# c5shen/WITCH

Measured on AMD Instinct MI355X. Metric: query-seqs aligned/sec (100k queries x 200-HMM eHMM), higher is better.
Workload: dtype f32; 1 GPU; dna_100k_x200; n_queries=100000, n_hmms=200, query_len=150, model_len_min=898, model_len_max=993, k=10, pairs_reported_rank0=20000000, pairs_multidomain_rank0=968, pairs_long_list_rank0=0, pairs_dense_redo_rank0=3, topk_crc32=3263627139

## Files before the change

witch_amd/csrc/wh_device.h:

```cpp
#pragma once
#include <hip/hip_runtime.h>

#include "wh_common.h"

namespace wh {

template <int CTRL, int ROW_MASK = 0xF, int BANK_MASK = 0xF, bool BOUND = false>
__device__ __forceinline__ float dppf(float old, float src) {
  return __builtin_bit_cast(
      float, __builtin_amdgcn_update_dpp(__builtin_bit_cast(int, old), __builtin_bit_cast(int, src), CTRL,
                                         ROW_MASK, BANK_MASK, BOUND));
}

typedef float v4f_t __attribute__((ext_vector_type(4)));
template <int Q, bool BLK = true>
__device__ __forceinline__ constexpr int fs_piece(int lane, int q4) { return (BLK && Q >= 8) ? lane * (2 * (Q / 4)) + q4 : q4 * kWave + lane; }
__device__ __forceinline__ float4 nt_load4(const float4 *p) {
  v4f_t v = __builtin_nontemporal_load(reinterpret_cast<const v4f_t *>(p));
  return make_float4(v.x, v.y, v.z, v.w);
}
__device__ __forceinline__ void nt_store4(float4 *p, float a, float b, float c, float d) {
  v4f_t v = {a, b, c, d};
  __builtin_nontemporal_store(v, reinterpret_cast<v4f_t *>(p));
}

__device__ __forceinline__ float wave_shr1(float x) { return dppf<0x138, 0xF, 0xF, true>(0.f, x); }

__device__ __forceinline__ float readlane_f(float x, int lane) {
  return __builtin_bit_cast(float, __builtin_amdgcn_readlane(__builtin_bit_cast(int, x), lane));
}

__device__ __forceinline__ float wave_sum(float x) {
  x += dppf<0xB1>(0.f, x);
  x += dppf<0x4E>(0.f, x);
  x += dppf<0x141>(0.f, x);
  x += dppf<0x140>(0.f, x);
  return (readlane_f(x, 0) + readlane_f(x, 16)) + (readlane_f(x, 32) + readlane_f(x, 48));
}

__device__ __forceinline__ float wave_max(float x) {
  x = fmaxf(x, dppf<0xB1>(x, x));
  x = fmaxf(x, dppf<0x4E>(x, x));
  x = fmaxf(x, dppf<0x141>(x, x));
  x = fmaxf(x, dppf<0x140>(x, x));
  return fmaxf(fmaxf(readlane_f(x, 0), readlane_f(x, 16)), fmaxf(readlane_f(x, 32), readlane_f(x, 48)));
}

template <int N>
struct RowsDown {
  unsigned v[N];
  int top;
  __device__ __forceinline__ void load(const float *spec, const int (&off)[N], const int (&shift)[N], int i, int lane) {
    top = i;
#pragma unroll
    for (int n = 0; n < N; n++) {
      const int r = i - lane + shift[n];
      v[n] = r >= 0 ? __builtin_nontemporal_load(reinterpret_cast<const unsigned *>(spec) + off[n] + r) : 0u;
    }
  }
  __device__ __forceinline__ bool spent(int i) const { return top - i >= kWave; }
  __device__ __forceinline__ unsigned u(int n, int i) const { return (unsigned)__builtin_amdgcn_readlane((int)v[n], top - i); }
  __device__ __forceinline__ int s(int n, int i) const { return __builtin_amdgcn_readlane((int)v[n], top - i); }
  __device__ __forceinline__ float f(int n, int i) const { return __builtin_bit_cast(float, __builtin_amdgcn_readlane((int)v[n], top - i)); }
};

struct ScanC { float s[6]; };

__device__ __forceinline__ ScanC scan_prepare(float A) {
  ScanC c;
  c.s[0] = A; A *= dppf<0x111>(1.f, A);
  c.s[1] = A; A *= dppf<0x112>(1.f, A);
  c.s[2] = A; A *= dppf<0x114>(1.f, A);
  c.s[3] = A; A *= dppf<0x118>(1.f, A);
  c.s[4] = A; A *= dppf<0x142, 0xA>(1.f, A);
  c.s[5] = A;
  return c;
}

__device__ __forceinline__ float scan_apply(const ScanC &c, float B) {
#ifndef WH_PLAIN_DPP_SCAN
  asm("s_nop 1\n\tv_fmac_f32_dpp %0, %0, %1 row_shr:1 row_mask:0xf bank_mask:0xf" : "+v"(B) : "v"(c.s[0]));
  asm("s_nop 1\n\tv_fmac_f32_dpp %0, %0, %1 row_shr:2 row_mask:0xf bank_mask:0xf" : "+v"(B) : "v"(c.s[1]));
  asm("s_nop 1\n\tv_fmac_f32_dpp %0, %0, %1 row_shr:4 row_mask:0xf bank_mask:0xf" : "+v"(B) : "v"(c.s[2]));
  asm("s_nop 1\n\tv_fmac_f32_dpp %0, %0, %1 row_shr:8 row_mask:0xf bank_mask:0xf" : "+v"(B) : "v"(c.s[3]));
  asm("s_nop 1\n\tv_fmac_f32_dpp %0, %0, %1 row_bcast:15 row_mask:0xa bank_mask:0xf" : "+v"(B) : "v"(c.s[4]));
  asm("s_nop 1\n\tv_fmac_f32_dpp %0, %0, %1 row_bcast:31 row_mask:0xc bank_mask:0xf" : "+v"(B) : "v"(c.s[5]));
  asm("s_nop 1" : "+v"(B));
  return B;
#else
  B = fmaf(c.s[0], dppf<0x111>(0.f, B), B);
  B = fmaf(c.s[1], dppf<0x112>(0.f, B), B);
  B = fmaf(c.s[2], dppf<0x114>(0.f, B), B);
  B = fmaf(c.s[3], dppf<0x118>(0.f, B), B);
  B = fmaf(c.s[4], dppf<0x142, 0xA>(0.f, B), B);
  B = fmaf(c.s[5], dppf<0x143, 0xC>(0.f, B), B);
  return B;
#endif
}

template <class T>
__device__ __forceinline__ T *uniform_ptr(T *p) {
  const unsigned long long v = (unsigned long long)p;
  const unsigned lo = (unsigned)__builtin_amdgcn_readfirstlane((int)(unsigned)v), hi = (unsigned)__builtin_amdgcn_readfirstlane((int)(unsigned)(v >> 32));
  return (T *)(((unsigned long long)hi << 32) | lo);
}

__device__ __forceinline__ float row_shr1(float x) { return dppf<0x111, 0xF, 0xF, true>(0.f, x); }
__device__ __forceinline__ float row_sum(float x) {
  x += dppf<0xB1>(0.f, x);
  x += dppf<0x4E>(0.f, x);
  x += dppf<0x141>(0.f, x);
  x += dppf<0x140>(0.f, x);
  return x;
}
struct ScanR { float s[4]; };
__device__ __forceinline__ ScanR scan_prepare_row(float A) {
  ScanR c;
  c.s[0] = A; A *= dppf<0x111>(1.f, A);
  c.s[1] = A; A *= dppf<0x112>(1.f, A);
  c.s[2] = A; A *= dppf<0x114>(1.f, A);
  c.s[3] = A;
  return c;
}
__device__ __forceinline__ float scan_apply_row(const ScanR &c, float B) {
  asm("s_nop 1\n\tv_fmac_f32_dpp %0, %0, %1 row_shr:1 row_mask:0xf bank_mask:0xf" : "+v"(B) : "v"(c.s[0]));
  asm("s_nop 1\n\tv_fmac_f32_dpp %0, %0, %1 row_shr:2 row_mask:0xf bank_mask:0xf" : "+v"(B) : "v"(c.s[1]));
  asm("s_nop 1\n\tv_fmac_f32_dpp %0, %0, %1 row_shr:4 row_mask:0xf bank_mask:0xf" : "+v"(B) : "v"(c.s[2]));
  asm("s_nop 1\n\tv_fmac_f32_dpp %0, %0, %1 row_shr:8 row_mask:0xf bank_mask:0xf" : "+v"(B) : "v"(c.s[3]));
  asm("s_nop 1" : "+v"(B));
  return B;
}

template <int Q, bool TREG>
struct TransTab;

template <int Q>
struct TransTab<Q, true> {
  float4 v[FW_NARR][Q / 4];
  __device__ __forceinline__ void load(const float *g, const float * , int lane) {
    const float4 *p = reinterpret_cast<const float4 *>(g);
#pragma unroll
    for (int a = 0; a < FW_NARR; a++)
#pragma unroll
      for (int q4 = 0; q4 < Q / 4; q4++) v[a][q4] = p[(a * (Q / 4) + q4) * kWave + lane];
  }
  __device__ __forceinline__ float4 ld(int a, int q4) const { return v[a][q4]; }
};

template <int Q>
struct TransTab<Q, false> {
  const float4 *p;
  __device__ __forceinline__ void load(const float * , const float *lds, int lane) {
    p = reinterpret_cast<const float4 *>(lds) + lane;
  }
  __device__ __forceinline__ float4 ld(int a, int q4) const { return p[(a * (Q / 4) + q4) * kWave]; }
};

__device__ __forceinline__ float f4get(const float4 &v, int j) {
  return j == 0 ? v.x : j == 1 ? v.y : j == 2 ? v.z : v.w;
}

template <int Q, bool TREG>
__device__ __forceinline__ float lane_product(const TransTab<Q, TREG> &T, int arr) {
  float A = 1.f;
#pragma unroll
  for (int q4 = 0; q4 < Q / 4; q4++) {
    float4 d = T.ld(arr, q4);
    A *= d.x; A *= d.y; A *= d.z; A *= d.w;
  }
  return A;
}

typedef float v4f_t __attribute__((ext_vector_type(4)));
typedef const __attribute__((address_space(3))) v4f_t lds_cv4_t;
struct LdsF4 {
  lds_cv4_t *p;
  __device__ __forceinline__ LdsF4(const float *base) : p((lds_cv4_t *)base) {}
  __device__ __forceinline__ float4 operator[](int i) const { const v4f_t v = p[i]; return make_float4(v.x, v.y, v.z, v.w); }
};

template <int Q>
__device__ __forceinline__ void load_em_fwd(float (&od)[Q], const float *emL, const float *emG, int x, int K,
                                            int lane) {
  if (x < K) {
    const LdsF4 p(emL + (size_t)x * Q * kWave + 4 * lane);
#pragma unroll
    for (int q4 = 0; q4 < Q / 4; q4++) {
      float4 v = p[q4 * kWave];
      od[4 * q4] = v.x; od[4 * q4 + 1] = v.y; od[4 * q4 + 2] = v.z; od[4 * q4 + 3] = v.w;
    }
  } else {
    const float4 *p = reinterpret_cast<const float4 *>(emG + (size_t)x * Q * kWave) + lane;
#pragma unroll
    for (int q4 = 0; q4 < Q / 4; q4++) {
      float4 v = p[q4 * kWave];
      od[4 * q4] = v.x; od[4 * q4 + 1] = v.y; od[4 * q4 + 2] = v.z; od[4 * q4 + 3] = v.w;
    }
  }
}

template <int Q>
__device__ __forceinline__ void load_em_rev(float (&od)[Q], const float *emL, const float *emG, int x, int K,
                                            int lane) {
  if (x < K) {
    const LdsF4 p(emL + (size_t)x * Q * kWave + 4 * (kWave - 1 - lane));
#pragma unroll
    for (int p4 = 0; p4 < Q / 4; p4++) {
      float4 v = p[(Q / 4 - 1 - p4) * kWave];
      od[4 * p4] = v.w; od[4 * p4 + 1] = v.z; od[4 * p4 + 2] = v.y; od[4 * p4 + 3] = v.x;
    }
  } else {
    const float4 *p = reinterpret_cast<const float4 *>(emG + (size_t)x * Q * kWave) + (kWave - 1 - lane);
#pragma unroll
    for (int p4 = 0; p4 < Q / 4; p4++) {
      float4 v = p[(Q / 4 - 1 - p4) * kWave];
      od[4 * p4] = v.w; od[4 * p4 + 1] = v.z; od[4 * p4 + 2] = v.y; od[4 * p4 + 3] = v.x;
    }
  }
}

__device__ __forceinline__ int f32_exponent(float x) { return ((__builtin_bit_cast(int, x) >> 23) & 0xFF) - 127; }
__device__ __forceinline__ float pow2f_int(int e) { return __builtin_bit_cast(float, (e + 127) << 23); }

struct LenCfg { float loop, move, EJ, EC; };

__device__ __forceinline__ LenCfg len_config(int Lcfg, bool multihit) {
  LenCfg c;
  float nj = multihit ? 1.0f : 0.0f;
  c.move = (2.0f + nj) / ((float)Lcfg + 2.0f + nj);
  c.loop = 1.0f - c.move;
  c.EJ = multihit ? 0.5f : 0.0f;
  c.EC = multihit ? 0.5f : 1.0f;
  return c;
}

enum { SP_N = 0, SP_B, SP_E, SP_J, SP_C, SP_S, SP_ML, SP_MH, SP_NARR };

constexpr float kRescaleHi = 1048576.0f;

__device__ __forceinline__ void region_scan_global(float *spec, int SP, int L, int *regs, int lane, int &nenv,
                                                   int &nreg, int &flags) {
  const float rt1 = 0.25f, rt2 = 0.10f;
  float btot = 0.f, etot = 0.f;
  int i0 = -1;
  bool trig = false;
  if (lane == 0) { spec[SP_J * SP] = 0.f; spec[SP_C * SP] = 0.f; }
  for (int j0 = 1; j0 <= L; j0 += kWave) {
    const int jj = j0 + lane;
    const bool valid = jj <= L;
    const float nv = valid ? __builtin_nontemporal_load(spec + SP_N * SP + jj) : 0.f;
    const float bv = valid ? __builtin_nontemporal_load(spec + SP_B * SP + jj - 1) : 0.f;
    const float ev = valid ? __builtin_nontemporal_load(spec + SP_E * SP + jj) : 0.f;
    float jout = 0.f, cout = 0.f;
    const int cnt = L - j0 + 1 < kWave ? L - j0 + 1 : kWave;
    for (int t = 0; t < cnt; t++) {
      const int j = j0 + t;
      const float mocc = 1.0f - readlane_f(nv, t);
      const float bold = btot, eold = etot;
      btot += readlane_f(bv, t);
      etot += readlane_f(ev, t);
      if (lane == t) { jout = btot; cout = etot; }
      if (!trig) {
        if (mocc - (btot - bold) < rt2) i0 = j;
        else if (i0 == -1) i0 = j;
        if (mocc >= rt1) trig = true;
      } else if (mocc - (etot - eold) < rt2) {
        if (nenv < WH_MAX_ENVELOPES) {
          if (lane == 0) { regs[2 * nenv] = i0; regs[2 * nenv + 1] = j; }
          nenv++;
        } else flags |= WH_FLAG_TRUNC;
        nreg++;
        i0 = -1;
        trig = false;
      }
    }
    if (valid) { spec[SP_J * SP + jj] = jout; spec[SP_C * SP + jj] = cout; }
  }
}

template <int Q, bool TREG, bool STORE, bool USEP = false, bool SLIM = false, bool UM = false, bool COUNT = false, bool BLK = false>
__device__ __forceinline__ void forward_sweep(const TransTab<Q, TREG> &T, const ScanC &sc, const float *emL,
                                              const float *emG, int K, const uint8_t *seq, int L, LenCfg cfg,
                                              float *spec, int SP, float *Fs, float keep_scale, int lane,
                                              float &xC_out, int &ef_out, unsigned *um_out = nullptr, int *nstored_out = nullptr, int keep_lanes = 63 << 8) {
  float Mp[Q], Ip[Q], Dp[Q];
#pragma unroll
  for (int q = 0; q < Q; q++) { Mp[q] = 0.f; Ip[q] = 0.f; Dp[q] = 0.f; }
  float xN = 1.0f, xB = cfg.move, xJ = 0.f, xC = 0.f, xE = 0.f;
  int ef = 0;
  unsigned long long um_prev = 0, um_steady = 0;
  int nstored = 0;
  unsigned long long umask = 0;
  if (lane == 0) {
    spec[SP_N * SP] = xN; spec[SP_B * SP] = xB; spec[SP_E * SP] = 0.f; spec[SP_J * SP] = 0.f;
    spec[SP_C * SP] = 0.f; reinterpret_cast<int *>(spec)[SP_S * SP] = 0;
  }
#pragma unroll 1
  for (int i = 1; i <= L; i++) {
    asm volatile("" ::: "memory");
    const int x = seq[i - 1];
    float od[Q];
    load_em_fwd<Q>(od, emL, emG, x, K, lane);
    const float mm1 = wave_shr1(Mp[Q - 1]), im1 = wave_shr1(Ip[Q - 1]), dm1 = wave_shr1(Dp[Q - 1]);
#pragma unroll
    for (int q4 = Q / 4 - 1; q4 >= 0; q4--) {
      const float4 A = T.ld(FW_A, q4), B = T.ld(FW_B, q4), C = T.ld(FW_C, q4), E = T.ld(FW_E, q4);
      const float4 MI = T.ld(FW_MI, q4), II = T.ld(FW_II, q4);
#pragma unroll
      for (int j = 3; j >= 0; j--) {
        const int q = 4 * q4 + j;
        const float pm = q > 0 ? Mp[q > 0 ? q - 1 : 0] : mm1;
        const float pi = q > 0 ? Ip[q > 0 ? q - 1 : 0] : im1;
        const float pd = q > 0 ? Dp[q > 0 ? q - 1 : 0] : dm1;
        const float ni = fmaf(f4get(MI, j), Mp[q], f4get(II, j) * Ip[q]);
        float acc = xB * f4get(E, j);
        acc = fmaf(f4get(A, j), pm, acc);
        acc = fmaf(f4get(B, j), pi, acc);
        acc = fmaf(f4get(C, j), pd, acc);
        Mp[q] = od[q] * acc;
        Ip[q] = ni;
      }
    }
    const float mn1 = wave_shr1(Mp[Q - 1]);
    float dprev = 0.f;
#pragma unroll
    for (int q4 = 0; q4 < Q / 4; q4++) {
      const float4 D1 = T.ld(FW_D1, q4), D2 = T.ld(FW_D2, q4);
#pragma unroll
      for (int j = 0; j < 4; j++) {
        const int q = 4 * q4 + j;
        const float src = q > 0 ? Mp[q > 0 ? q - 1 : 0] : mn1;
        dprev = fmaf(f4get(D2, j), dprev, f4get(D1, j) * src);
        Dp[q] = dprev;
      }
    }
    float carry = wave_shr1(scan_apply(sc, dprev));
    float es = 0.f;
#pragma unroll
    for (int q4 = 0; q4 < Q / 4; q4++) {
      const float4 D2 = T.ld(USEP ? FW_P : FW_D2, q4);
#pragma unroll
      for (int j = 0; j < 4; j++) {
        const int q = 4 * q4 + j;
        if (USEP) {
          Dp[q] = fmaf(f4get(D2, j), carry, Dp[q]);
        } else {
          carry *= f4get(D2, j);
          Dp[q] += carry;
        }
        es += Mp[q] + Dp[q];
      }
    }
    xE = wave_sum(es);
    xN = xN * cfg.loop;
    xC = fmaf(xC, cfg.loop, xE * cfg.EC);
    xJ = fmaf(xJ, cfg.loop, xE * cfg.EJ);
    if (xE > kRescaleHi) {
      const int e = f32_exponent(xE);
      const float r = pow2f_int(-e);
#pragma unroll
      for (int q = 0; q < Q; q++) { Mp[q] *= r; Ip[q] *= r; Dp[q] *= r; }
      xN *= r; xC *= r; xJ *= r; xE *= r;
      ef += e;
    }
    xB = (xJ + xN) * cfg.move;
    if (lane == 0) {
      spec[SP_N * SP + i] = xN;
      if (!(STORE && SLIM)) { spec[SP_B * SP + i] = xB; spec[SP_E * SP + i] = xE; }
      spec[SP_J * SP + i] = xJ; spec[SP_C * SP + i] = xC;
      reinterpret_cast<int *>(spec)[SP_S * SP + i] = ef;
    }
    if (UM && !STORE) {
      if ((i & 7) == 0) {
        float lmax = 0.f;
#pragma unroll
        for (int q = 0; q < Q; q += 2) lmax = fmaxf(fmaxf(fmaxf(fmaxf(lmax, Mp[q]), Mp[q + 1]), Ip[q]), Ip[q + 1]);
        const unsigned long long dom = __ballot(lmax > 0.5f * xE);
        umask |= dom;
        const unsigned long long link = dom & (um_prev | (um_prev << 1));
        if (link) um_steady |= link | (um_prev & (link | (link >> 1)));
        um_prev = dom;
      }
    }
    if (STORE) {
      constexpr int ML = SLIM ? SP_B : SP_ML, MH = SLIM ? SP_E : SP_MH;
      float lmax = 0.f;
#pragma unroll
      for (int q = 0; q < Q; q += 2) lmax = fmaxf(fmaxf(fmaxf(fmaxf(lmax, Mp[q]), Mp[q + 1]), Ip[q]), Ip[q + 1]);
      const unsigned long long dom = __ballot(lmax > 0.5f * xE);
      umask |= dom;
      const int blo = keep_lanes & 255;
      int bhi = (keep_lanes >> 8) & 255;
      if (keep_lanes >> 16) bhi = min(bhi, (keep_lanes >> 16) - 1 + i / Q);
      const bool keep = keep_scale < 0.f || (lmax > keep_scale * xE && lane >= blo && lane <= bhi);
      const unsigned long long mask = __ballot(keep);
      if (COUNT) nstored += __builtin_popcountll(mask);
      if (lane == 0) {
        reinterpret_cast<unsigned *>(spec)[ML * SP + i] = (unsigned)(mask & 0xFFFFFFFFull);
        reinterpret_cast<unsigned *>(spec)[MH * SP + i] = (unsigned)(mask >> 32);
      }
      if (keep) {
        float4 *row = reinterpret_cast<float4 *>(Fs) + (size_t)i * (2 * (Q / 4) * kWave);
#pragma unroll
        for (int q4 = 0; q4 < Q / 4; q4++) {
          nt_store4(row + (BLK ? fs_piece<Q>(lane, q4) : q4 * kWave + lane), Mp[4 * q4], Mp[4 * q4 + 1], Mp[4 * q4 + 2], Mp[4 * q4 + 3]);
          nt_store4(row + (BLK ? fs_piece<Q>(lane, Q / 4 + q4) : (Q / 4 + q4) * kWave + lane), Ip[4 * q4], Ip[4 * q4 + 1], Ip[4 * q4 + 2], Ip[4 * q4 + 3]);
        }
      }
    }
  }
  if (STORE && lane == 0) {
    reinterpret_cast<unsigned *>(spec)[(SLIM ? SP_B : SP_ML) * SP] = (unsigned)(umask & 0xFFFFFFFFull);
    reinterpret_cast<unsigned *>(spec)[(SLIM ? SP_E : SP_MH) * SP] = (unsigned)(umask >> 32);
  }
  if (UM && !STORE && lane == 0) {
    um_out[0] = (unsigned)(umask & 0xFFFFFFFFull); um_out[1] = (unsigned)(umask >> 32);
    um_out[-1] = um_steady ? (unsigned)(__builtin_ctzll(um_steady) | ((63 - __builtin_clzll(um_steady)) << 8) | (1 << 16)) : 0u;
  }
  if (COUNT && nstored_out) *nstored_out = nstored;
  xC_out = xC;
  ef_out = ef;
}

constexpr float kClampHi = 1.1529215e18f;

template <int Q>
__device__ __forceinline__ void mirror_scale(int dn, float (&Mb)[Q], float (&Ib)[Q], float &xJ, float &xC, float &xN) {
  if (dn != 0) {
    const float r = __builtin_bit_cast(float, (127 - dn) << 23);
#pragma unroll
    for (int p = 0; p < Q; p++) { Mb[p] *= r; Ib[p] *= r; }
    xJ *= r; xC *= r; xN *= r;
  }
}

template <int Q>
__device__ __forceinline__ bool clamp_backward(float (&Mb)[Q], float (&Ib)[Q], float &xB, float &xJ, float &xC, float &xN) {
  if (fmaxf(xB, fmaxf(xN, xC)) > kClampHi) {
#pragma unroll
    for (int p = 0; p < Q; p++) { Mb[p] = fminf(Mb[p], kClampHi); Ib[p] = fminf(Ib[p], kClampHi); }
    xB = fminf(xB, kClampHi); xN = fminf(xN, kClampHi); xC = fminf(xC, kClampHi); xJ = fminf(xJ, kClampHi);
    return true;
  }
  return false;
}

template <int Q, bool TREG>
__device__ __forceinline__ float backward_emit(const TransTab<Q, TREG> &T, const float *emL, const float *emG, int x,
                                               int K, int lane, float (&Mb)[Q]) {
  float part = 0.f;
  auto groups = [&](auto em_ld) {
#pragma unroll
    for (int p4 = 0; p4 < Q / 4; p4++) {
      const float4 E = T.ld(BW_E, p4);
      const float4 O = em_ld(Q / 4 - 1 - p4);
      Mb[4 * p4 + 0] *= O.w; part = fmaf(E.x, Mb[4 * p4 + 0], part);
      Mb[4 * p4 + 1] *= O.z; part = fmaf(E.y, Mb[4 * p4 + 1], part);
      Mb[4 * p4 + 2] *= O.y; part = fmaf(E.z, Mb[4 * p4 + 2], part);
      Mb[4 * p4 + 3] *= O.x; part = fmaf(E.w, Mb[4 * p4 + 3], part);
    }
  };
  x = __builtin_amdgcn_readfirstlane(x);
  if (x < K) {
    const LdsF4 ep(emL + (size_t)x * Q * kWave + 4 * (kWave - 1 - lane));
    groups([&](int q4) { return ep[q4 * kWave]; });
  } else {
    const float4 *ep = reinterpret_cast<const float4 *>(emG + (size_t)x * Q * kWave) + (kWave - 1 - lane);
    groups([&](int q4) { return ep[q4 * kWave]; });
  }
  return part;
}

template <int Q>
struct TransTabAt {
  LdsF4 base;
  int slot[4];
  __device__ __forceinline__ TransTabAt(const float *lds) : base(lds) {}
  __device__ __forceinline__ float4 ld(int a, int p4) const { return base[a * (Q / 4) * kWave + slot[p4]]; }
};

template <int Q, bool TREG, bool USEP = false>
__device__ __forceinline__ void backward_cells(const TransTab<Q, TREG> &T, const ScanC &sc, float (&Mb)[Q],
                                               float (&Ib)[Q], float xE) {
  float Dn[Q];
  const float gm1 = wave_shr1(Mb[Q - 1]);
  float dprev = 0.f;
#pragma unroll
  for (int p4 = 0; p4 < Q / 4; p4++) {
    const float4 DM = T.ld(BW_DM, p4), DD = T.ld(BW_DD, p4);
#pragma unroll
    for (int j = 0; j < 4; j++) {
      const int p = 4 * p4 + j;
      const float g = p > 0 ? Mb[p > 0 ? p - 1 : 0] : gm1;
      dprev = fmaf(f4get(DD, j), dprev, fmaf(f4get(DM, j), g, xE));
      Dn[p] = dprev;
    }
  }
  float carry = wave_shr1(scan_apply(sc, dprev));
#pragma unroll
  for (int p4 = 0; p4 < Q / 4; p4++) {
    const float4 DD = T.ld(USEP ? BW_P : BW_DD, p4);
#pragma unroll
    for (int j = 0; j < 4; j++) {
      const int p = 4 * p4 + j;
      if (USEP) {
        Dn[p] = fmaf(f4get(DD, j), carry, Dn[p]);
      } else {
        carry *= f4get(DD, j);
        Dn[p] += carry;
      }
    }
  }
  const float dm1 = wave_shr1(Dn[Q - 1]);
#pragma unroll
  for (int p4 = Q / 4 - 1; p4 >= 0; p4--) {
    const float4 MM = T.ld(BW_MM, p4), IM = T.ld(BW_IM, p4), MI = T.ld(BW_MI, p4), II = T.ld(BW_II, p4);
    const float4 MD = T.ld(BW_MD, p4);
#pragma unroll
    for (int j = 3; j >= 0; j--) {
      const int p = 4 * p4 + j;
      const float g = p > 0 ? Mb[p > 0 ? p - 1 : 0] : gm1;
      const float dn = p > 0 ? Dn[p > 0 ? p - 1 : 0] : dm1;
      float nm = fmaf(f4get(MM, j), g, xE);
      nm = fmaf(f4get(MI, j), Ib[p], nm);
      nm = fmaf(f4get(MD, j), dn, nm);
      const float ni = fmaf(f4get(IM, j), g, f4get(II, j) * Ib[p]);
      Mb[p] = nm;
      Ib[p] = ni;
    }
  }
}

template <class TT>
__device__ __forceinline__ void backward_cells_row(const TT &T, const ScanR &sc, float (&Mb)[16], float (&Ib)[16], float xE) {
  float Dn[16];
  const float gm1 = row_shr1(Mb[15]);
  float dprev = 0.f;
#pragma unroll
  for (int p4 = 0; p4 < 4; p4++) {
    const float4 DM = T.ld(BW_DM, p4), DD = T.ld(BW_DD, p4);
#pragma unroll
    for (int j = 0; j < 4; j++) {
      const int p = 4 * p4 + j;
      const float g = p > 0 ? Mb[p > 0 ? p - 1 : 0] : gm1;
      dprev = fmaf(f4get(DD, j), dprev, fmaf(f4get(DM, j), g, xE));
      Dn[p] = dprev;
    }
  }
  float carry = row_shr1(scan_apply_row(sc, dprev));
#pragma unroll
  for (int p4 = 0; p4 < 4; p4++) {
    const float4 DD = T.ld(BW_DD, p4);
#pragma unroll
    for (int j = 0; j < 4; j++) {
      const int p = 4 * p4 + j;
      carry *= f4get(DD, j);
      Dn[p] += carry;
    }
  }
  const float dm1 = row_shr1(Dn[15]);
#pragma unroll
  for (int p4 = 3; p4 >= 0; p4--) {
    const float4 MM = T.ld(BW_MM, p4), IM = T.ld(BW_IM, p4), MI = T.ld(BW_MI, p4), II = T.ld(BW_II, p4);
    const float4 MD = T.ld(BW_MD, p4);
#pragma unroll
    for (int j = 3; j >= 0; j--) {
      const int p = 4 * p4 + j;
      const float g = p > 0 ? Mb[p > 0 ? p - 1 : 0] : gm1;
      const float dn = p > 0 ? Dn[p > 0 ? p - 1 : 0] : dm1;
      float nm = fmaf(f4get(MM, j), g, xE);
      nm = fmaf(f4get(MI, j), Ib[p], nm);
      nm = fmaf(f4get(MD, j), dn, nm);
      const float ni = fmaf(f4get(IM, j), g, f4get(II, j) * Ib[p]);
      Mb[p] = nm;
      Ib[p] = ni;
    }
  }
}

}
```

witch_amd/csrc/wh_host_score.hip:

```cpp
#include "wh_host.h"

static const int kStagedMaxBatches = 1 << 15;
static const int kStagedQB = 48;

static int resolve_main_cap(int max_M) {
  const size_t per_wave = (kLdsBudget - resolve_lds_header_bytes(0)) / (size_t)resolve_waves_per_cu();
  int lo = 1, hi = 1 << 20;
  while (lo < hi) {
    const int mid = lo + (hi - lo + 1) / 2;
    if (resolve_lds_bytes(mid, max_M) <= per_wave) lo = mid; else hi = mid - 1;
  }
  return lo;
}

static ScoreCall score_call(wh_ehmm *e, const uint8_t *d_residues, const int64_t *d_offsets, int64_t nq, int64_t total_residues, int32_t max_len,
                            int32_t *d_decibits, uint8_t *d_flags, float *d_fwd_bits, wh_pair_detail *d_detail, void *stream) {
  ScoreCall c = {e, (hipStream_t)stream, d_residues, d_offsets, nq, total_residues, max_len, d_decibits, d_flags, d_fwd_bits, d_detail};
  c.Lc = std::max(max_len, 1);
  c.H = (int)e->hmms.size();
  c.npairs_all = nq * (int64_t)c.H;
  const bool fits = resolve_lds_bytes(c.Lc, e->max_M) <= kLdsBudget;
  c.Lmain = fits || e->knobs.no_long_query ? c.Lc : resolve_main_cap(e->max_M);
  c.resolve = !e->knobs.no_resolve && (fits || !e->knobs.no_long_query) && c.npairs_all < 0x7FFFFFFF;
  c.mixed = nq > 0 && total_residues > 0 && (double)max_len > 1.25 * (double)total_residues / (double)nq;
  c.wide_dense = getenv("WH_WIDE_DENSE"); c.wide_no_em_lds = getenv("WH_WIDE_NO_EM_LDS"); c.p2win_force = getenv("WH_P2WIN_FORCE");
  c.res_null2_gather = getenv("WH_RES_NULL2_GATHER"); c.res_no_lds_tables = getenv("WH_RES_NO_LDS_TABLES");
  if (const char *wv = getenv("WH_RES_WAVES")) c.res_waves = std::max(1, atoi(wv));
  c.Ls = main_length_cap(e, c.Lc, false, c.resolve, c.p2win_force);
  return c;
}

struct StagedWaves { int wl, one, both, p2, p4; };
enum class ScoreFamily { PhaseCall, PhaseCallB, TwoQuery, FourEnvelope, PassSync, Staged };
static const char *const kFamilyName[] = {"phase-call", "phase-call(B)", "two-queries-per-wave", "phase-call", "pass-synchronous", "staged"};

struct ScoreClassPlan {
  int Q, list_off, n_list;
  ScoreFamily family;
  LdsPlan b;
  int Klds;
  bool specg;
  int p2win;
  bool use_qorder;
  int QB, n_qblocks, n_items;
  size_t scratch_stride, spec_stride;
  int blocks;
  StagedWaves st;
};

static int cap_waves(const Knobs &kn, int w) { return cap_waves(kn.max_waves, w); }
static size_t score_table_bytes(const wh_ehmm *e, int Q) { return score_table_bytes(e->K, Q); }

static const int G_all = 1, G_most = 4, G_few = 8, G_rare = 32;
static int staged_cand_cap(int G, int per_pair) { return std::min(G * kStagedQB * per_pair, 2048); }
static size_t staged_lds(int Q, int wl, int arrays, int waves, int cand) {
  return lds_bytes(kLdsHeader + (size_t)cand * sizeof(int), (size_t)arrays * Q * kWave * sizeof(float), waves, wl);
}
static bool plan_staged(const wh_ehmm *e, int Q, int Lc, StagedWaves *w) {
  const int K = e->K;
  const size_t tbl = (size_t)Q * kWave * sizeof(float);
  auto fit = [&](int arrays, int from, int cand, int per_cu) { return fit_waves(kLdsHeader + (size_t)cand * sizeof(int), arrays * tbl, from, w->wl, per_cu); };
  w->wl = kScoreSpecArrays * row_stride(Lc) + 32 + kRegsInts + residue_words(Lc);
  w->one = fit(K + FW_NARR, 12, staged_cand_cap(G_few, WH_MAX_ENVELOPES), 1);
  w->both = fit(K + 2 * FW_NARR, 12, staged_cand_cap(G_rare, WH_MAX_ENVELOPES), 1);
  w->p2 = fit(K, 12, staged_cand_cap(G_most, 1), 2);
  w->p4 = fit(K, 10, staged_cand_cap(G_most, WH_MAX_ENVELOPES), 2);
  return w->one >= 4 && w->both >= 4 && w->p2 >= 4 && w->p4 >= 4;
}

static int plan_score_class(const ScoreCall &c, int Q, int list_off, int n_list, ScoreClassPlan *out) {
  const wh_ehmm *e = c.e;
  const Knobs &kn = e->knobs;
  const int Lc = c.Ls;
  const int64_t nq = c.nq;
  const size_t table = score_table_bytes(e, Q);
  ScoreClassPlan p = {};
  p.Q = Q; p.list_off = list_off; p.n_list = n_list;
  ScoreLds l;
  if (!plan_score_lds(plan_knobs(e, c.p2win_force), e->K, Q, Lc, true, &l)) { set_error("query length %d with model class Q=%d does not fit in LDS", c.max_len, Q); return WH_ERANGE; }
  p.b = l.b; p.Klds = l.Klds;
  LdsPlan &b = p.b;
  const bool big = l.big, specg = l.specg, pairk = l.pairk, p2win = l.p2win, p2inpl = l.p2inpl;
  bool quadk = false;
  if ((kn.kernel == 10 || kn.kernel == 11) && !e->st_off && !big && !pairk && !specg && !kn.dbg && (Q == 8 || Q == 12 || Q == 16 || Q == 20 || Q == 24) &&
      plan_staged(e, Q, Lc, &p.st)) {
    p.family = ScoreFamily::Staged;
    b.SP = row_stride(Lc); b.wave_lds = p.st.wl;
    p.QB = kStagedQB; p.n_qblocks = (int)((nq + p.QB - 1) / p.QB); p.n_items = n_list * p.n_qblocks;
    p.scratch_stride = (size_t)(Lc + 1) * 2 * Q * kWave;
    *out = p;
    return WH_OK;
  }
  if (kn.kernel == 12 && !big && !pairk && !specg && Q == 16) {
    const int wlq = kScoreSpecArrays * row_stride(Lc) + 128 + kRegsInts + 4 * 16 + 4 * 16 + 4 * residue_words(Lc);
    const int wq = fit_waves(kLdsHeader, table, cap_waves(kn, 12), wlq);
    if (wq >= 8) { quadk = true; b = {wq, row_stride(Lc), wlq, lds_bytes(kLdsHeader, table, wq, wlq)}; }
  }
  p.family = big ? ScoreFamily::PassSync : pairk ? ScoreFamily::TwoQuery : quadk ? ScoreFamily::FourEnvelope : kn.kernel == 8 ? ScoreFamily::PhaseCallB : ScoreFamily::PhaseCall;
  p.p2win = (specg || big || pairk || quadk) ? 0 : p2win ? 1 : p2inpl ? 2 : 0;
  p.use_qorder = big || c.mixed;
  const int waves = b.waves;
  p.QB = big ? waves * 2 : pairk ? waves * 4 : waves * (kn.item_g > 0 ? kn.item_g : 32);
  const int per_turn = pairk ? 2 : 1;
  const int max_blocks = big ? e->cu_count : e->cu_count * std::max(1, 8 / waves);
  if ((int64_t)n_list * ((nq + p.QB - 1) / p.QB) < 4 * (int64_t)max_blocks) {
    p.QB = waves * per_turn;
    if (!big && !pairk) for (int g_ = 16; g_ > 1; g_ /= 2)
      if ((int64_t)n_list * ((nq + waves * g_ - 1) / (waves * g_)) >= 4 * (int64_t)max_blocks) { p.QB = waves * g_; break; }
  }
  if (quadk) p.QB = std::max(p.QB, waves * 8);
  p.n_qblocks = (int)((nq + p.QB - 1) / p.QB);
  p.n_items = n_list * p.n_qblocks;
  p.scratch_stride = (size_t)(quadk ? 5 : per_turn) * (size_t)(Lc + 1) * 2 * Q * kWave;
  p.spec_stride = specg ? (size_t)8 * b.SP : quadk ? (size_t)(5 * kScoreSpecArrays + 1) * b.SP : 0;
  p.specg = specg || quadk;
  p.blocks = clamp_blocks(std::min(p.n_items, max_blocks), (size_t)waves * (p.scratch_stride + p.spec_stride) * sizeof(float), e->d_scratch, e->max_M, Lc, "scoring");
  if (p.blocks < 0) return WH_ENOMEM;
  *out = p;
  return WH_OK;
}

static ScoreArgs class_args(const ScoreCall &c, const ScoreClassPlan &p, int launches) {
  const wh_ehmm *e = c.e;
  const Knobs &kn = e->knobs;
  ScoreArgs a;
  fill_common(a, c);
  a.tables = (const float *)e->d_tables.p;
  a.hmm_list = (const int32_t *)e->d_lists.p + p.list_off; a.n_list = p.n_list;
  a.counter = e->counter(kSlotLaunch0 + launches);
  a.dbg = kn.dbg;
  a.no_window = kn.no_window ? 1 : 0;
  a.keep_scale = kn.keep_scale;
  a.spill_band = kn.kernel != 9 ? kn.spill_band : 0;
  a.Klds = p.Klds; a.SP = p.b.SP; a.wave_lds = p.b.wave_lds; a.spec_arrays = kScoreSpecArrays;
  a.paths = reinterpret_cast<unsigned long long *>(e->counter(kSlotScorePath));
  a.p2win = p.p2win;
  a.qorder = p.use_qorder ? c.d_qorder : nullptr;
  a.QB = p.QB; a.n_qblocks = p.n_qblocks; a.n_items = p.n_items;
  a.scratch_stride = p.scratch_stride; a.spec_stride = p.spec_stride;
  a.scratch = (float *)e->d_scratch.p;
  if (p.specg) a.spec_scratch = (float *)e->d_spec.p;
  return a;
}

static int print_class_stats(const ScoreCall &c, int Q, const unsigned long long *stats) {
  unsigned long long st[40];
  if (int rc = stats_read(c, stats, st)) return rc;
  const double tot = (double)(st[4] + st[5] + st[6] + st[7] + st[8] + st[9] + st[10] + st[11]);
  fprintf(stderr, "[wh] Q=%d wave cycles: P1 %.1f%%  P2 %.1f%%  regions %.1f%%  P3 %.1f%%  P4 %.1f%%  null2 %.1f%%  swaps+barriers %.1f%%  other %.1f%%  (total %.3g ticks)\n", Q, 100.0 * st[4] / tot,
          100.0 * st[5] / tot, 100.0 * st[6] / tot, 100.0 * st[7] / tot, 100.0 * st[8] / tot, 100.0 * st[9] / tot, 100.0 * st[10] / tot, 100.0 * st[11] / tot, tot);
  if (st[38]) fprintf(stderr, "[wh] Q=%d wave lifetimes %.3g cycles: %.1f%% in the phases above, %.1f%% fetching an item (two barriers)\n", Q, (double)st[38], 100.0 * tot / (double)st[38], 100.0 * (double)st[39] / (double)st[38]);
  if (st[37]) fprintf(stderr, "[wh] Q=%d four-envelope sweeps: %llu envelopes, %.0f wave cycles per envelope (slot 'null2' above)\n", Q, st[37], (double)st[9] / (double)st[37]);
  fprintf(stderr, "[wh] Q=%d envelope Backward sweeps: %llu on a 256-node window, %llu on a 512-node window, %llu windows failed the mass certificate, %llu full width; union of the stored lane blocks: span %.1f blocks (with margin), %.1f blocks set, of %llu envelopes\n", Q, st[0], st[1], st[2], st[3], (double)st[12] / (double)std::max(1ull, st[14]), (double)st[15] / (double)std::max(1ull, st[14]), st[14]);
  fprintf(stderr, "[wh] Q=%d multihit Backward on a window: %llu scans, of them in doubt at a threshold %llu, at the multidomain bound %llu; window loss out of range %llu; mean eps %.3g\n", Q,
          st[35], st[32], st[33], st[36], st[35] ? 1e-9 * (double)st[34] / (double)st[35] : 0.0);
  fprintf(stderr, "[wh] Q=%d |Ld - mass| / Ld  (<3e-7, <1e-6, <3e-6, <1e-5, <2e-5, more): window sweeps %llu %llu %llu %llu %llu %llu; full-width sweeps %llu %llu %llu %llu %llu %llu\n", Q,
          st[16], st[17], st[18], st[19], st[20], st[21], st[22], st[23], st[24], st[25], st[26], st[27]);
  return WH_OK;
}

static int launch_score_class(const ScoreCall &c, const ScoreClassPlan &p, int *launches) {
  wh_ehmm *e = c.e;
  hipStream_t s = c.s;
  const int Q = p.Q, waves = p.b.waves, threads = waves * kWave;
  const bool big = p.family == ScoreFamily::PassSync;
  ScoreArgs a = class_args(c, p, *launches);
  if (a.p2win == 2) {
    a.p2_backup_stride = (size_t)kScoreSpecArrays * a.SP;
    if (e->d_p2bak.ensure((size_t)p.blocks * waves * a.p2_backup_stride * sizeof(float))) return WH_ENOMEM;
    a.p2_backup = (float *)e->d_p2bak.p;
  }
  if (int rc = stats_begin(c, 320, 13, &a.stats)) return rc;
  if (e->knobs.trace) fprintf(stderr, "[wh] score Q=%d kernel=%s specg=%d waves=%d blocks=%d lds=%zu SP=%d wave_lds=%d items=%d Lcap=%d\n", Q,
                              kFamilyName[(int)p.family], (int)p.specg, waves, p.blocks, p.b.lds, a.SP, a.wave_lds, a.n_items, a.Lcap);
  HIPCHK(hipMemsetAsync(a.counter, 0, sizeof(int), s));
  if (class_mark(e, s, Q, big ? 1 : 0)) return WH_EHIP;
  hipError_t err = big ? launch_score_big(Q, a, p.blocks, threads, p.b.lds, s)
                   : p.family == ScoreFamily::TwoQuery ? launch_score9(Q, a, p.blocks, threads, p.b.lds, s)
                   : p.family == ScoreFamily::FourEnvelope ? launch_score7q(Q, a, p.blocks, threads, p.b.lds, s)
                   : p.family == ScoreFamily::PhaseCallB ? launch_score7b(Q, a, p.blocks, threads, p.b.lds, s)
                                                         : launch_score7(Q, a, p.blocks, threads, p.b.lds, s);
  if (err != hipSuccess) { set_error("score kernel launch (Q=%d) failed: %s", Q, hipGetErrorString(err)); return WH_EHIP; }
  (*launches)++;
  return a.stats ? print_class_stats(c, Q, a.stats) : WH_OK;
}

static int print_staged_stats(const ScoreCall &c, int Q, const unsigned long long *stats) {
  unsigned long long st[64];
  if (int rc = stats_read(c, stats, st)) return rc;
  static const char *kind[9] = {"p1", "p2win 256", "p2win 512", "p2full", "p3", "p4win 256", "p4win 512", "p4full", "dense"};
  for (int k = 0; k < 9; k++)
    fprintf(stderr, "[wh] staged Q=%d %-10s sweeps %9llu  shader cycles per sweep %10.0f  real time per sweep %8.1f us  (clock %.2f GHz)  wave lifetimes %.3g cycles, in sweeps %.1f%%\n", Q, kind[k], st[4 * k + 3],
            st[4 * k + 3] ? (double)st[4 * k] / (double)st[4 * k + 3] : 0.0, st[4 * k + 3] ? 0.01 * (double)st[4 * k + 1] / (double)st[4 * k + 3] : 0.0,
            st[4 * k + 1] ? 0.1 * (double)st[4 * k] / (double)st[4 * k + 1] : 0.0, (double)st[4 * k + 2], st[4 * k + 2] ? 100.0 * (double)st[4 * k] / (double)st[4 * k + 2] : 0.0);
  return WH_OK;
}

static int launch_staged_class(const ScoreCall &c, const ScoreClassPlan &p, int *launches) {
  wh_ehmm *e = c.e;
  hipStream_t s = c.s;
  const Knobs &kn = e->knobs;
  const bool split = kn.kernel == 11;
  const int Q = p.Q, Lc = c.Ls, K = e->K, w_one = p.st.one, w_both = p.st.both, w_p2 = p.st.p2, w_p4 = p.st.p4;
  auto lds_of = [&](int arrays, int waves, int cand) { return staged_lds(Q, p.st.wl, arrays, waves, cand); };
  ScoreArgs a = class_args(c, p, *launches);
  StagedArgs g;
  memset(&g, 0, sizeof g);
  g.slab_stride = (size_t)(Lc + 1) * 2 * Q * kWave;
  g.p1stride = (size_t)kScoreSpecArrays * a.SP;
  g.p3stride = g.p1stride;
  int64_t NS = split ? (int64_t)e->cu_count * w_one * 16 : (int64_t)1 << 20;
  size_t free_b = 0, total_b = 0;
  if (split && hipMemGetInfo(&free_b, &total_b) == hipSuccess) {
    const size_t budget = (size_t)((double)(free_b + e->d_st_slabs.cap + e->d_st_p3spec.cap) * 0.45);
    NS = std::min<int64_t>(NS, (int64_t)(budget / ((g.slab_stride + g.p3stride) * sizeof(float))));
  }
  if (kn.st_units > 0) NS = kn.st_units;
  const int64_t total_pairs = (int64_t)a.n_items * a.QB;
  NS = std::min<int64_t>(NS, (int64_t)((double)total_pairs * e->st_upp) + a.QB * WH_MAX_ENVELOPES);
  if (NS < 16) { set_error("staged launches: no HBM for the Forward slabs (Q=%d, L=%d)", Q, Lc); return WH_ENOMEM; }
  const double upp = split ? e->st_upp : 1.0;
  int items_b = (int)std::max<int64_t>(1, (int64_t)((double)NS / upp) / a.QB);
  items_b = std::min(items_b, a.n_items);
  {
    const int nb = (a.n_items + items_b - 1) / items_b;
    items_b = (a.n_items + nb - 1) / nb;
    if (items_b > 2 * e->cu_count) items_b = std::min((items_b + e->cu_count - 1) / e->cu_count * e->cu_count, (int)std::max<int64_t>(1, (int64_t)((double)NS / upp) / a.QB));
  }
  const int NB = items_b * a.QB;
  const int n_batches = (a.n_items + items_b - 1) / items_b;
  if (e->d_st_pairs.ensure(sizeof(StPair) * (size_t)NB) || e->d_st_p1spec.ensure(sizeof(float) * g.p1stride * (size_t)NB) ||
      e->d_st_cnt.ensure(sizeof(int) * 32 * (size_t)kStagedMaxBatches))
    return WH_ENOMEM;
  if (e->last_staged_batches + n_batches > kStagedMaxBatches) { set_error("staged launches: more than %d batches in one call", kStagedMaxBatches); return WH_ERANGE; }
  if (split && (e->d_st_units.ensure(sizeof(StUnit) * (size_t)NS) || e->d_st_p3spec.ensure(sizeof(float) * g.p3stride * (size_t)NS) ||
                e->d_st_slabs.ensure(sizeof(float) * g.slab_stride * (size_t)NS)))
    return WH_ENOMEM;
  g.NB = NB; g.NS = (int)NS;
  if (split) e->st_last_NB = NB;
  g.pairs = (StPair *)e->d_st_pairs.p; g.p1spec = (float *)e->d_st_p1spec.p;
  g.units = (StUnit *)e->d_st_units.p; g.p3spec = (float *)e->d_st_p3spec.p; g.slabs = (float *)e->d_st_slabs.p;
  g.pair_paths = e->path_buf; g.pair_paths16 = e->path_buf16;
  int *cnt0 = (int *)e->d_st_cnt.p + 32 * (size_t)e->last_staged_batches;
  HIPCHK(hipMemsetAsync(cnt0, 0, sizeof(int) * 32 * (size_t)n_batches, s));
  const bool w512 = Q == 16 || Q == 24;
  if (kn.trace) fprintf(stderr, "[wh] staged Q=%d: %d items of %d queries in %d batches of %d pairs, %lld units (%.1f GB of slabs), waves dense %d / both %d / p2win %d / p4win %d\n",
                        Q, a.n_items, a.QB, n_batches, NB, (long long)NS, (double)NS * g.slab_stride * 4e-9, w_one, w_both, w_p2, w_p4);
  if (class_mark(e, s, Q, 4)) return WH_EHIP;
  if (int rc = stats_begin(c, 512, -1, &a.stats)) return rc;
  const int cu = e->cu_count;
  for (int b = 0; b < n_batches; b++) {
    g.a = a;
    g.item0 = b * items_b;
    g.n_items_b = std::min(items_b, a.n_items - g.item0);
    g.cnt = cnt0 + 32 * (size_t)b;
    auto groups = [&](int G) { return (g.n_items_b + G - 1) / G; };
    hipError_t err = hipSuccess;
    auto go = [&](int G, int per_pair) { g.G = G; g.cand_cap = staged_cand_cap(G, per_pair); return err == hipSuccess; };
    if (go(G_all, 1)) err = launch_staged_p1(Q, g, std::min(groups(g.G), cu), w_one * kWave, lds_of(K + FW_NARR, w_one, g.cand_cap), s);
    if (go(G_most, 1)) err = launch_staged_p2win(Q, 4, g, std::min(groups(g.G), 2 * cu), w_p2 * kWave, lds_of(K, w_p2, g.cand_cap), s);
    if (w512 && go(G_few, 1)) err = launch_staged_p2win(Q, 8, g, std::min(groups(g.G), 2 * cu), w_p2 * kWave, lds_of(K, w_p2, g.cand_cap), s);
    if (go(G_few, 1)) err = launch_staged_p2full(Q, g, std::min(groups(g.G), cu), w_one * kWave, lds_of(K + BW_NARR, w_one, g.cand_cap), s);
    if (!split) {
      if (go(G_all, 1)) err = launch_staged_env(Q, g, std::min(groups(g.G), cu), w_both * kWave, lds_of(K + 2 * FW_NARR, w_both, g.cand_cap), s);
      if (err != hipSuccess) { set_error("staged launch (Q=%d, batch %d) failed: %s", Q, b, hipGetErrorString(err)); return WH_EHIP; }
      continue;
    }
    if (go(G_all, WH_MAX_ENVELOPES)) err = launch_staged_p3(Q, g, std::min(groups(g.G), cu), w_one * kWave, lds_of(K + FW_NARR, w_one, g.cand_cap), s);
    if (go(G_most, WH_MAX_ENVELOPES)) err = launch_staged_p4win(Q, 4, g, std::min(groups(g.G), 2 * cu), w_p4 * kWave, lds_of(K, w_p4, g.cand_cap), s);
    if (w512 && go(G_few, WH_MAX_ENVELOPES)) err = launch_staged_p4win(Q, 8, g, std::min(groups(g.G), 2 * cu), w_p4 * kWave, lds_of(K, w_p4, g.cand_cap), s);
    if (go(G_few, WH_MAX_ENVELOPES)) err = launch_staged_p4full(Q, g, std::min(groups(g.G), cu), w_one * kWave, lds_of(K + BW_NARR, w_one, g.cand_cap), s);
    if (go(G_rare, WH_MAX_ENVELOPES)) err = launch_staged_dense(Q, g, std::min(groups(g.G), cu), w_both * kWave, lds_of(K + 2 * FW_NARR, w_both, g.cand_cap), s);
    if (err == hipSuccess) err = launch_staged_assemble(g, s);
    if (err != hipSuccess) { set_error("staged launch (Q=%d, batch %d) failed: %s", Q, b, hipGetErrorString(err)); return WH_EHIP; }
  }
  e->last_staged_batches += n_batches;
  (*launches)++;
  return a.stats ? print_staged_stats(c, Q, a.stats) : WH_OK;
}

static int size_resolver_queue(const ScoreCall &c) {
  wh_ehmm *e = c.e;
  e->last_resolved = 0;
  if (!c.resolve) return WH_OK;
  int64_t cap = std::max<int64_t>(65536, std::max<int64_t>(c.npairs_all / 20, (int64_t)(1.25 * e->rq_rate * (double)c.npairs_all) + 1024)) +
                c.nq * (int64_t)e->generic_front.size();
  cap = std::max<int64_t>(cap, (int64_t)(e->d_rrecs.cap / sizeof(ResolveRec)));
  if (e->knobs.rqueue_cap > 0) cap = e->knobs.rqueue_cap;
  cap = std::min<int64_t>(std::max(cap, e->rq_floor), c.npairs_all);
  if (e->d_rrecs.ensure(sizeof(ResolveRec) * (size_t)cap)) return WH_ENOMEM;
  e->rq_cap = cap;
  HIPCHK(hipMemsetAsync(e->counter(kSlotResolveCount), 0, 2 * sizeof(int), c.s));
  return WH_OK;
}

static int order_queries(ScoreCall &c) {
  wh_ehmm *e = c.e;
  const int64_t nq = c.nq;
  bool any_long = !e->wide_by_w.empty();
  for (auto &kv : e->by_q) any_long = any_long || kv.first >= 20;
  c.d_qorder = nullptr;
  if (!(any_long || c.mixed) || nq <= 4 || nq >= 0x7FFFFFFF) return WH_OK;
  std::vector<int64_t> offs((size_t)nq + 1);
  HIPCHK(hipMemcpyAsync(offs.data(), c.d_offsets, sizeof(int64_t) * offs.size(), hipMemcpyDeviceToHost, c.s));
  HIPCHK(hipStreamSynchronize(c.s));
  std::vector<int32_t> ord((size_t)nq);
  for (int64_t q = 0; q < nq; q++) ord[(size_t)q] = (int32_t)q;
  std::stable_sort(ord.begin(), ord.end(), [&](int32_t x, int32_t y) { return offs[x + 1] - offs[x] > offs[y + 1] - offs[y]; });
  if (e->d_qorder.ensure(sizeof(int32_t) * ord.size())) return WH_ENOMEM;
  HIPCHK(hipMemcpyAsync(e->d_qorder.p, ord.data(), sizeof(int32_t) * ord.size(), hipMemcpyHostToDevice, c.s));
  HIPCHK(hipStreamSynchronize(c.s));
  c.d_qorder = (const int32_t *)e->d_qorder.p;
  return WH_OK;
}

static int score_size_classes(const ScoreCall &c, int *launches) {
  wh_ehmm *e = c.e;
  std::vector<ScoreClassPlan> plans;
  size_t need_scratch = 0, need_spec = 0;
  int list_off = 0;
  for (auto &kv : e->by_q) {
    const int n_list = (int)kv.second.size();
    list_off += n_list;
    if (e->force_wide && e->dev[(size_t)kv.second[0]].wideW > 0) continue;
    ScoreClassPlan p;
    if (int rc = plan_score_class(c, kv.first, list_off - n_list, n_list, &p)) return rc;
    const size_t waves = p.family == ScoreFamily::Staged ? (size_t)p.st.both : (size_t)p.b.waves;
    const size_t blocks = p.family == ScoreFamily::Staged ? (e->knobs.kernel == 11 ? 0 : (size_t)e->cu_count) : (size_t)p.blocks;
    need_scratch = std::max(need_scratch, blocks * waves * p.scratch_stride * sizeof(float));
    if (p.specg) need_spec = std::max(need_spec, blocks * waves * p.spec_stride * sizeof(float));
    plans.push_back(p);
  }
  if (e->d_scratch.ensure(need_scratch) || (need_spec && e->d_spec.ensure(need_spec))) return WH_ENOMEM;
  for (const ScoreClassPlan &p : plans)
    if (int rc = p.family == ScoreFamily::Staged ? launch_staged_class(c, p, launches) : launch_score_class(c, p, launches)) return rc;
  return WH_OK;
}

static int print_wide_stats(const ScoreCall &c, int W, int wq, const unsigned long long *stats) {
  unsigned long long st[24];
  if (int rc = stats_read(c, stats, st)) return rc;
  for (int wv = 0; wv < 2; wv++) {
    const unsigned long long *g = st + 8 + 8 * wv;
    double rt = 0; for (int k = 0; k < 7; k++) rt += (double)g[k];
    if (rt > 0) fprintf(stderr, "[wh] wide P1 row, %s wave: cells %.1f%%  barrier0 %.1f%%  local D %.1f%%  barrier1 %.1f%%  fix-up+sum %.1f%%  barrier2 %.1f%%  specials+tail %.1f%%\n", wv ? "last" : "first",
                        100 * g[0] / rt, 100 * g[1] / rt, 100 * g[2] / rt, 100 * g[3] / rt, 100 * g[4] / rt, 100 * g[5] / rt, 100 * g[6] / rt);
  }
  const double tot = (double)st[5] > 0 ? (double)st[5] : 1.0;
  fprintf(stderr, "[wh] wide %d x %d cells per lane, cycles of the first wave: P1 %.1f%%  P2 %.1f%%  regions %.1f%%  P3 %.1f%%  P4 %.1f%%  (of %.3g)\n", W, wq,
          100.0 * st[0] / tot, 100.0 * st[1] / tot, 100.0 * st[2] / tot, 100.0 * st[3] / tot, 100.0 * st[4] / tot, tot);
  return WH_OK;
}

static size_t wide_score_stride(int Lc, int wq, int W, bool sparse) {
  const size_t st = (size_t)(Lc + 1) * 2 * wq * W * kWave + (sparse ? (size_t)(Lc + 1) * W * 2 + 4 : 0);
  return (st + 3) & ~(size_t)3;
}

static int score_wide_classes(const ScoreCall &c, int *launches, bool *wide_done) {
  wh_ehmm *e = c.e;
  hipStream_t s = c.s;
  const int Lc = c.Ls;
  const size_t wlds0 = wide_lds_bytes(Lc);
  *wide_done = wlds0 <= kLdsBudget;
  if (!*wide_done && e->force_wide) { set_error("WH_FORCE_WIDE: query length %d does not fit the wide kernel's LDS block", c.max_len); return WH_ERANGE; }
  if (!*wide_done) return WH_OK;
  size_t woff = e->generic_front.size();
  for (auto &kv : e->by_q) woff += kv.second.size();
  int wclass = 0;
  for (auto &kv : e->wide_by_w) {
    const int W = kv.first & 15, wq = kv.first >> 4;
    const size_t em_floats = (size_t)e->K * wq * W * kWave;
    const bool em_lds = (wq == kWideQReg || wq == kWideQReg2) && !c.wide_no_em_lds && wide_lds_bytes(Lc, em_floats) <= kLdsBudget;
    const size_t wlds = em_lds ? wide_lds_bytes(Lc, em_floats) : wlds0;
    WideArgs a;
    fill_common(a, c);
    a.tables = (const float *)e->d_tables.p;
    a.hmm_list = (const int32_t *)e->d_lists.p + woff; a.n_list = (int)kv.second.size();
    woff += kv.second.size();
    if (wclass >= kWideScoreClasses) { set_error("too many classes of long models"); return WH_ERANGE; }
    a.counter = e->counter(kSlotWideScore + wclass++);
    a.em_lds = em_lds ? 1 : 0;
    a.SP = row_stride(Lc);
    a.qorder = c.d_qorder;
    a.sparse = c.wide_dense ? 0 : 1;
    a.paths16 = e->path_buf16;
    a.scratch_stride = wide_score_stride(Lc, wq, W, a.sparse != 0);
    const int64_t n_items = c.nq * (int64_t)a.n_list;
    const int per_cu = (W <= 4 && 2 * wlds <= kLdsBudget) ? 2 : 1;
    int blocks = (int)std::min<int64_t>(n_items, (int64_t)e->cu_count * per_cu);
    blocks = clamp_blocks(blocks, a.scratch_stride * sizeof(float), e->d_wscratch, e->max_M, Lc, "wide scoring");
    if (blocks < 0) return WH_ENOMEM;
    if (e->d_wscratch.ensure((size_t)blocks * a.scratch_stride * sizeof(float))) return WH_ENOMEM;
    a.scratch = (float *)e->d_wscratch.p;
    HIPCHK(hipMemsetAsync(a.counter, 0, sizeof(int), s));
    if (e->knobs.trace) fprintf(stderr, "[wh] wide scoring: %lld pairs on %d models, %d waves per pair x %d cells per lane, %d workgroups, lds %zu, slab %zu MB per workgroup\n",
                                (long long)n_items, a.n_list, W, wq, blocks, wlds, a.scratch_stride * 4 >> 20);
    if (class_mark(e, s, wq * W, 3)) return WH_EHIP;
    if (int rc = stats_begin(c, 320, -1, &a.stats)) return rc;
    hipError_t werr = launch_score_wide(wq, a, blocks, W, wlds, s);
    if (werr != hipSuccess) { set_error("wide score kernel launch failed: %s", hipGetErrorString(werr)); return WH_EHIP; }
    if (a.stats) if (int rc = print_wide_stats(c, W, wq, a.stats)) return rc;
    (*launches)++;
  }
  return WH_OK;
}

static int score_front_end(const ScoreCall &c, bool wide_done, int *launches) {
  wh_ehmm *e = c.e;
  if (!c.resolve || c.nq * (int64_t)e->generic.size() >= 0x7FFFFFFF) {
    set_error("models of more than %d nodes need the resolver stage (query length %d, %lld pairs)", kMaxQ * kWave, c.max_len, (long long)c.npairs_all);
    return WH_ERANGE;
  }
  GenericArgs g = front_args(c, c.Ls);
  size_t goff = 0;
  for (auto &kv : e->by_q) goff += kv.second.size();
  const size_t n_gen = wide_done ? e->generic_front.size() : e->generic.size();
  g.hmm_list = (const int32_t *)e->d_lists.p + goff; g.n_list = (int)n_gen;
  const size_t glds = generic_lds_bytes(c.Ls);
  if (glds > kLdsBudget) { set_error("query length %d does not fit the any-size kernel's LDS", c.max_len); return WH_ERANGE; }
  const int64_t n_items = c.nq * (int64_t)n_gen;
  int blocks = 0;
  if (int rc = front_blocks(c, g, n_items, "any-size front end", &blocks)) return rc;
  HIPCHK(hipMemsetAsync(g.counter, 0, sizeof(int), c.s));
  if (e->knobs.trace) fprintf(stderr, "[wh] any-size front end: %lld pairs on %zu models (up to %d nodes), %d wavefronts, slab %zu MB per wave\n",
                              (long long)n_items, n_gen, e->max_M, blocks, g.slab_stride * 8 >> 20);
  if (class_mark(e, c.s, e->max_Q, 2)) return WH_EHIP;
  hipError_t gerr = launch_generic_front(g, blocks, glds, c.s);
  if (gerr != hipSuccess) { set_error("any-size front kernel launch failed: %s", hipGetErrorString(gerr)); return WH_EHIP; }
  (*launches)++;
  return WH_OK;
}

static int read_staged_counters(const ScoreCall &c, bool *over) {
  wh_ehmm *e = c.e;
  e->st_cnt_host.resize((size_t)32 * e->last_staged_batches);
  HIPCHK(hipMemcpyAsync(e->st_cnt_host.data(), e->d_st_cnt.p, sizeof(int) * e->st_cnt_host.size(), hipMemcpyDeviceToHost, c.s));
  HIPCHK(hipStreamSynchronize(c.s));
  int most_units = 0;
  for (int b = 0; b < e->last_staged_batches; b++) {
    *over = *over || e->st_cnt_host[(size_t)32 * b + ST_OVERFLOW] != 0;
    most_units = std::max(most_units, e->st_cnt_host[(size_t)32 * b + ST_N_UNITS]);
  }
  if (!*over && most_units > 0 && e->st_last_NB > 0) e->st_upp = std::max(1.05, 1.25 * (double)most_units / (double)e->st_last_NB);
  if (!*over) return WH_OK;
  if (e->knobs.trace) fprintf(stderr, "[wh] staged launches: a batch ran out of envelope units, the scoring pass is repeated with the fused kernel\n");
  e->st_upp = std::min<double>(WH_MAX_ENVELOPES, e->st_upp * 2.0);
  e->st_off = true;
  return WH_OK;
}

static void prefetch_align_workspace(const ScoreCall &c) {
  wh_ehmm *e = c.e;
  const size_t need = (size_t)8 * (size_t)e->cu_count * (size_t)(c.Ls + 1) * 5 * (size_t)e->by_q.rbegin()->first * kWave * sizeof(float);
  size_t free_b = 0, total_b = 0;
  if (need > e->d_ascratch.cap && hipMemGetInfo(&free_b, &total_b) == hipSuccess && need < free_b / 10) (void)e->d_ascratch.ensure(need);
}

static int score_dev_pass(ScoreCall &c, bool *overflow) {
  wh_ehmm *e = c.e;
  hipStream_t s = c.s;
  HIPCHK(hipSetDevice(e->device));
  if (timer_begin(e, 0, s)) return WH_EHIP;
  e->cls_n = 0;
  e->last_staged_batches = 0;
  int launches = 0;
  bool wide_done = false;
  if (c.nq > 0) {
    if ((int)e->by_q.size() > kMaxLaunches) { set_error("too many model size classes (%zu)", e->by_q.size()); return WH_ERANGE; }
    if (int rc = size_resolver_queue(c)) return rc;
    HIPCHK(hipMemsetAsync(e->counter(kSlotScorePath), 0, kScorePathInts * sizeof(int), s));
    static_assert(2 * kPathRecSlot + 2 == kScorePathInts, "the record's address takes the last of the eight path counters");
    if (e->path_buf16) HIPCHK(hipMemcpyAsync(e->counter(kSlotScorePath) + 2 * kPathRecSlot, &e->path_buf16, sizeof e->path_buf16, hipMemcpyHostToDevice, s));
    if (int rc = order_queries(c)) return rc;
    if (int rc = score_size_classes(c, &launches)) return rc;
    if (!e->wide_by_w.empty()) if (int rc = score_wide_classes(c, &launches, &wide_done)) return rc;
    if (!e->generic_front.empty() || (!wide_done && !e->wide_by_w.empty() && !e->force_wide))
      if (int rc = score_front_end(c, wide_done, &launches)) return rc;
  }
  if (class_mark(e, s, 0, -1)) return WH_EHIP;
  if (timer_end(e, 0, s, launches)) return WH_EHIP;
  if (e->last_staged_batches > 0) {
    bool over = false;
    if (int rc = read_staged_counters(c, &over)) return rc;
    if (over) {
      *overflow = true;
      if (timer_begin(e, 4, s) || timer_end(e, 4, s, 0)) return WH_EHIP;
      return WH_OK;
    }
  }
  if (c.nq > 0 && !e->by_q.empty()) prefetch_align_workspace(c);
  if (timer_begin(e, 4, s)) return WH_EHIP;
  int rlaunches = 0;
  if (c.nq > 0 && !e->knobs.no_resolve && e->d_rrecs.p) {
    if (int rc = resolver_stage(c, overflow, &rlaunches)) return rc;
  }
  if (timer_end(e, 4, s, rlaunches)) return WH_EHIP;
  return WH_OK;
}

extern "C" int wh_score_dev(wh_ehmm *e, const uint8_t *d_residues, const int64_t *d_offsets, int64_t nq,
                            int64_t total_residues, int32_t max_len, int32_t *d_decibits, uint8_t *d_flags,
                            float *d_fwd_bits, wh_pair_detail *d_detail, void *stream) {
  if (!e || !d_residues || !d_offsets || !d_decibits || !d_flags || nq < 0 || max_len < 0) {
    set_error("wh_score_dev: bad argument");
    return WH_EINVAL;
  }
  if (nq * (int64_t)e->hmms.size() >= 0x7FFFFFFF) {
    set_error("wh_score_dev: %lld queries x %zu models is 2^31 pairs or more; score the queries in chunks", (long long)nq, e->hmms.size());
    return WH_ERANGE;
  }
  ScoreCall c = score_call(e, d_residues, d_offsets, nq, total_residues, max_len, d_decibits, d_flags, d_fwd_bits, d_detail, stream);
  if (nq > 0 && !e->generic.empty() &&
      !one_block_fits(((generic_front_doubles(c.Ls, e->max_Q) + 1) & ~(size_t)1) * sizeof(double), e->d_rmx, e->max_M, c.Ls, "any-size front end"))
    return WH_ENOMEM;
  if (nq > 0 && !e->wide_by_w.empty()) {
    if ((int)e->wide_by_w.size() > kWideScoreClasses) { set_error("too many classes of long models (%zu)", e->wide_by_w.size()); return WH_ERANGE; }
    for (auto &kv : e->wide_by_w)
      if (wide_lds_bytes(c.Ls) <= kLdsBudget &&
          !one_block_fits(wide_score_stride(c.Ls, kv.first >> 4, kv.first & 15, !c.wide_dense) * sizeof(float), e->d_wscratch, e->max_M, c.Ls, "wide scoring"))
        return WH_ENOMEM;
  }
  if (c.Ls < c.Lc && !one_block_fits(front_args(c, c.Lc, front_longq(e, c.Lc)).slab_stride * sizeof(double), e->d_rmx, e->max_M, c.Lc, "long-query scoring pass"))
    return WH_ENOMEM;
  e->last_queue_reruns = 0;
  reset_resolver_counts(e);
  e->rq_floor = 0;
  e->st_off = false;
  if (d_detail && nq > 0) HIPCHK(hipMemsetAsync(d_detail, 0, sizeof(wh_pair_detail) * (size_t)nq * e->hmms.size(), c.s));
  bool overflow = false;
  int rc = score_dev_pass(c, &overflow);
  for (int again = 0; rc == WH_OK && overflow; again++) {
    if (again == 2) { set_error("wh_score_dev: the resolver's queue overflowed twice"); rc = WH_ERANGE; break; }
    e->last_queue_reruns++;
    overflow = false;
    rc = score_dev_pass(c, &overflow);
  }
  e->rq_floor = 0;
  e->st_off = false;
  return rc;
}
```

witch_amd/csrc/wh_plan.h:

```cpp
#pragma once
#include <algorithm>
#include <cstddef>
#include <vector>

#include "wh_common.h"

namespace wh {

size_t wide_lds_bytes(int Lcap, size_t em_floats);
size_t generic_lds_bytes(int Lcap);
int score9_block_floats(int SP, int Lcap);

constexpr size_t kLdsBudget = 160 * 1024 - 512;
constexpr size_t kLdsHeader = 16;
constexpr int kScoreSpecArrays = 6;
constexpr int kAlignSpecRows = 14;
constexpr int kMaxPlanLength = 1 << 24;

inline int row_stride(int Lc) { return (Lc + 1 + 3) / 4 * 4; }
inline int residue_words(int Lc) { return (Lc + 3) / 4 + 4; }
inline size_t lds_bytes(size_t header, size_t table, int w, int wave_words) { return header + table + (size_t)w * (size_t)wave_words * sizeof(float); }
inline int fit_waves(size_t header, size_t table, int w, int wave_words, int per_cu = 1) {
  while (w >= 1 && per_cu * lds_bytes(header, table, w, wave_words) > kLdsBudget) w--;
  return w;
}
inline bool plan_long_model(int Q, int K, int wave_words, int *Klds, size_t *lds) {
  *Klds = K;
  size_t table = (size_t)(K + 8) * Q * kWave * sizeof(float);
  if (lds_bytes(kLdsHeader, table, 4, wave_words) > kLdsBudget) { *Klds = 0; table = (size_t)8 * Q * kWave * sizeof(float); }
  *lds = lds_bytes(kLdsHeader, table, 4, wave_words);
  return *lds <= kLdsBudget;
}

struct PlanKnobs { int kernel = 7, max_waves = 0; bool force_specg = false, no_window = false, no_p2win = false, p2win_force = false; };
struct LdsPlan { int waves, SP, wave_lds; size_t lds; };
inline int cap_waves(int max_waves, int w) { return max_waves > 0 ? std::max(1, std::min(w, max_waves)) : w; }
inline size_t score_table_bytes(int K, int Q) { return (size_t)(K + 2 * FW_NARR) * Q * kWave * sizeof(float); }

inline bool plan_block1(int max_waves, int K, int Q, int Lcap, int extra_arrays, LdsPlan *b) {
  const int sp = row_stride(Lcap);
  const int wl = (kScoreSpecArrays + extra_arrays) * sp + 32 + kRegsInts + residue_words(Lcap);
  const int w = fit_waves(kLdsHeader, score_table_bytes(K, Q), cap_waves(max_waves, 12), wl);
  if (w < 1) return false;
  *b = {w, sp, wl, lds_bytes(kLdsHeader, score_table_bytes(K, Q), w, wl)};
  return true;
}

struct ScoreLds { LdsPlan b; bool big, specg, pairk, p2win, p2inpl; int Klds; };
inline bool plan_score_lds(const PlanKnobs &kn, int K, int Q, int Lc, bool with9, ScoreLds *out) {
  const size_t table = score_table_bytes(K, Q);
  ScoreLds r = {};
  LdsPlan &b = r.b;
  r.big = Q > kMaxQFast;
  if (with9 && !r.big && kn.kernel == 9 && !kn.force_specg && (Q == 8 || Q == 12 || Q == 16)) {
    const int wl9 = 2 * score9_block_floats(row_stride(Lc), Lc), w9 = cap_waves(kn.max_waves, 8);
    if (lds_bytes(kLdsHeader, table, w9, wl9) <= kLdsBudget) { r.pairk = true; b = {w9, row_stride(Lc), wl9, lds_bytes(kLdsHeader, table, w9, wl9)}; }
  }
  if (!r.big && !r.pairk) {
    bool ok = plan_block1(kn.max_waves, K, Q, Lc, 0, &b);
    if (ok && b.waves >= 4 && !kn.force_specg && !kn.no_window && !kn.no_p2win && Q >= 8) {
      LdsPlan b2 = {};
      if (plan_block1(kn.max_waves, K, Q, Lc, 3, &b2) && (b2.waves >= b.waves || (kn.p2win_force && b2.waves >= 8))) { r.p2win = true; b = b2; }
      else if (Q >= 20 && kn.kernel != 9) r.p2inpl = true;
    }
    if (!ok || b.waves < 4 || kn.force_specg) {
      r.specg = true;
      b.SP = row_stride(Lc);
      b.wave_lds = 32 + kRegsInts + residue_words(Lc);
      b.waves = fit_waves(kLdsHeader, table, cap_waves(kn.max_waves, Q <= 16 ? 12 : 8), b.wave_lds);
      ok = b.waves >= 1;
      b.lds = lds_bytes(kLdsHeader, table, b.waves, b.wave_lds);
      if (Q >= 20 && (!ok || b.waves < 4)) r.big = true;
      if (Q == 16 && !ok) r.big = true;
    }
    if (!r.big && !ok) return false;
  }
  if (r.big) {
    b.waves = 4; b.SP = row_stride(Lc); b.wave_lds = 32 + kRegsInts + residue_words(Lc);
    if (!plan_long_model(Q, K, b.wave_lds, &r.Klds, &b.lds)) return false;
    r.specg = true;
  }
  *out = r;
  return true;
}

struct AlignLds { int waves, SP, wave_lds, Klds; size_t lds; bool spec_in_hbm, swap; };
inline int plan_align_lds(bool force_specg, int K, int Q, int Lc, AlignLds *out) {
  const size_t table = (size_t)(K + 2 * FW_NARR) * Q * kWave * sizeof(float);
  AlignLds p = {};
  p.Klds = K; p.SP = row_stride(Lc);
  if (Q <= kMaxQFast) {
    p.wave_lds = kAlignSpecRows * p.SP + residue_words(Lc);
    p.waves = std::max(0, fit_waves(0, table, 8, p.wave_lds));
    p.lds = lds_bytes(kLdsHeader, table, p.waves, p.wave_lds);
  }
  p.swap = Q > kMaxQFast;
  if (!p.swap && Q >= 20 && (p.waves < 4 || force_specg) && lds_bytes(kLdsHeader, table, 4, residue_words(Lc)) > kLdsBudget) p.swap = true;
  if (!p.swap && Q == 16 && fit_waves(kLdsHeader, table, 8, residue_words(Lc)) < 1) p.swap = true;
  if (p.swap) {
    p.spec_in_hbm = true; p.wave_lds = residue_words(Lc); p.waves = 4;
    if (!plan_long_model(Q, K, p.wave_lds, &p.Klds, &p.lds)) return 1;
  } else if (p.waves < 4 || force_specg) {
    p.spec_in_hbm = true; p.wave_lds = residue_words(Lc);
    p.waves = fit_waves(kLdsHeader, table, 8, p.wave_lds);
    if (p.waves < 1) return lds_bytes(kLdsHeader, table, 1, residue_words(1)) > kLdsBudget ? 2 : 1;
    p.lds = lds_bytes(kLdsHeader, table, p.waves, p.wave_lds);
  }
  *out = p;
  return 0;
}

struct PlanClasses {
  int K = 4;
  std::vector<int> score_q, align_q;
  bool wide = false;
  bool force_wide = false;
  bool front = false;
};
inline bool score_fits(const PlanKnobs &kn, const PlanClasses &cl, int L, bool as_today) {
  ScoreLds s;
  for (int Q : cl.score_q) if (!plan_score_lds(kn, cl.K, Q, L, false, &s)) return false;
  const bool wide_ok = !cl.wide || wide_lds_bytes(L, 0) <= kLdsBudget;
  if (!wide_ok && (cl.force_wide || !as_today)) return false;
  if ((cl.front || (cl.wide && !wide_ok)) && generic_lds_bytes(L) > kLdsBudget) return false;
  return true;
}
inline bool align_fits(const PlanKnobs &kn, const PlanClasses &cl, int L) {
  AlignLds a;
  for (int Q : cl.align_q) if (plan_align_lds(kn.force_specg, cl.K, Q, L, &a) != 0) return false;
  return true;
}
template <class Fits> int largest_length(Fits fits) {
  if (!fits(1)) return 0;
  int lo = 1, hi = kMaxPlanLength;
  while (lo < hi) {
    const int mid = lo + (hi - lo + 1) / 2;
    if (fits(mid)) lo = mid; else hi = mid - 1;
  }
  return lo;
}
inline int score_main_cap(const PlanKnobs &kn, const PlanClasses &cl, int Lc) {
  if (score_fits(kn, cl, Lc, true)) return Lc;
  const int cap = largest_length([&](int L) { return score_fits(kn, cl, L, false); });
  return cap > 0 ? std::min(cap, Lc) : Lc;
}
inline int align_main_cap(const PlanKnobs &kn, const PlanClasses &cl, int Lc) {
  if (align_fits(kn, cl, Lc)) return Lc;
  const int cap = largest_length([&](int L) { return align_fits(kn, cl, L); });
  return cap > 0 ? std::min(cap, Lc) : Lc;
}
inline int query_len_cap(const PlanKnobs &kn, const PlanClasses &cl) {
  const int s = largest_length([&](int L) { return score_fits(kn, cl, L, false); });
  const int a = largest_length([&](int L) { return align_fits(kn, cl, L); });
  return std::min(s, a);
}

}
```

witch_amd/csrc/wh_score7.hip:

```cpp
#include <hip/hip_runtime.h>

#include "wh_device.h"
#include "wh_launch.h"

#ifndef WH_K7NS
#define WH_K7NS k7
#define WH_K7LAUNCH launch_score7
#endif

namespace wh {
namespace WH_K7NS {


constexpr float kKeepScale7 = 5.9604645e-08f;
constexpr float kMassTol7 = 2e-5f;
constexpr float kWinTol7 = 3e-6f;
__device__ __forceinline__ float spill_tol(bool banded) { return banded ? kWinTol7 : kMassTol7; }
#ifndef WH_K7_MAXQP
#define WH_K7_MAXQP 0
#endif
constexpr int kMaxQP = WH_K7_MAXQP;
#ifdef WH_SLIM_SPEC
constexpr bool kSlim = true;
constexpr int kSpML = SP_B, kSpMH = SP_E, kSpArr = 6;
#else
constexpr bool kSlim = false;
constexpr int kSpML = SP_ML, kSpMH = SP_MH, kSpArr = SP_NARR;
#endif
constexpr bool kMaskedAcc = true;

__device__ __noinline__ static double dlog(double x) { return log(x); }
__device__ __noinline__ static double dexp(double x) { return exp(x); }
__device__ __forceinline__ float flogsum0_v7(float b) {
  const float mx = b > 0.f ? b : 0.f, mn = b > 0.f ? 0.f : b;
  if (mn == -INFINITY || (mx - mn) >= 15.7f) return mx;
  const int idx = (int)((mx - mn) * 1000.0f);
  return mx + (float)dlog(1.0 + dexp((double)-idx / 1000.0));
}

typedef __attribute__((address_space(3))) float lds_f;
typedef __attribute__((address_space(3))) uint8_t lds_u8;
typedef __attribute__((address_space(3))) int lds_i;
typedef __attribute__((address_space(1))) float glb_f;

struct WaveCtx {
  lds_f *emL;
  const glb_f *emG;
  lds_f *fwL, *bwL;
  lds_f *spec;
  glb_f *specg;
  lds_f *n2tab;
  glb_f *Fs;
  int SP, lane;
  int alpha;
  uint32_t degen;
};
#if defined(__HIP_DEVICE_COMPILE__)
static_assert(sizeof(WaveCtx) <= 80, "WaveCtx must stay register-passed (see comment)");
#endif
__device__ __forceinline__ int ctxK(const WaveCtx &c) { return c.alpha & 255; }
__device__ __forceinline__ int ctxKp(const WaveCtx &c) { return (c.alpha >> 8) & 255; }
__device__ __forceinline__ int ctxKlds(const WaveCtx &c) { return (c.alpha >> 16) & 255; }
__device__ __forceinline__ float uniform_f(float x) { return __builtin_bit_cast(float, __builtin_amdgcn_readfirstlane(__builtin_bit_cast(int, x))); }
__device__ __forceinline__ int64_t uniform_i64(int64_t v) {
  const unsigned lo = (unsigned)__builtin_amdgcn_readfirstlane((int)(unsigned)(unsigned long long)v), hi = (unsigned)__builtin_amdgcn_readfirstlane((int)(unsigned)((unsigned long long)v >> 32));
  return (int64_t)(((unsigned long long)hi << 32) | lo);
}
struct P4Out { float mass, domcorr; };
struct RegOut { int nenv, nreg, flags; };

struct FwdOut { float xC; int ef; int nst; };
__device__ __forceinline__ FwdOut uniform_fwd(FwdOut o) { return FwdOut{uniform_f(o.xC), __builtin_amdgcn_readfirstlane(o.ef), __builtin_amdgcn_readfirstlane(o.nst)}; }

constexpr int kUmSlot = 30;
template <int Q, bool STORE, int TH, bool SG>
__device__ __noinline__ FwdOut sweep_forward(const WaveCtx c, lds_u8 *seq3, int L, LenCfg cfg, float keep_scale, int keep_lanes = 63 << 8) {
  const uint8_t *seq = (const uint8_t *)seq3;
  TransTab<Q, false> T;
  T.load(nullptr, (const float *)c.fwL, c.lane);
  const ScanC sc = scan_prepare(lane_product<Q, false>(T, FW_D2));
  FwdOut o;
  constexpr bool UM = !STORE && !SG && Q >= 8;
  o.nst = 0;
  forward_sweep<Q, false, STORE, (Q <= kMaxQP), kSlim, UM, STORE, !SG>(T, sc, (const float *)c.emL, (const float *)c.emG, ctxKlds(c), seq, L, cfg, SG ? (float *)c.specg : (float *)c.spec, c.SP, (float *)c.Fs, keep_scale, c.lane, o.xC, o.ef,
                                                                  reinterpret_cast<unsigned *>((float *)c.n2tab) + kUmSlot, &o.nst, keep_lanes);
  if (SG) __builtin_amdgcn_fence(__ATOMIC_SEQ_CST, "workgroup");
  return o;
}

template <int Q, int TH, bool SG>
__device__ __noinline__ void sweep_backward_decode(const WaveCtx c, lds_u8 *seq3, int L, LenCfg cm, float invZ, int ef_L) {
  const uint8_t *seq = (const uint8_t *)seq3;
  const float *emL = (const float *)c.emL;
  TransTab<Q, false> T;
  T.load(nullptr, (const float *)c.bwL, c.lane);
  const ScanC sc = scan_prepare(lane_product<Q, false>(T, BW_DD));
  const int lane = c.lane, SP = c.SP;
  float *spec = SG ? (float *)c.specg : (float *)c.spec;
  auto ldf = [&](int idx) -> float { return SG ? __builtin_nontemporal_load(spec + idx) : spec[idx]; };
  auto ldi = [&](int idx) -> int { return SG ? __builtin_nontemporal_load(reinterpret_cast<const int *>(spec) + idx) : reinterpret_cast<const int *>(spec)[idx]; };
  float Mb[Q], Ib[Q];
#pragma unroll
  for (int p = 0; p < Q; p++) { Mb[p] = 0.f; Ib[p] = 0.f; }
  float xC = cm.move, xJ = 0.f, xN = 0.f, xB = 0.f;
  int eb = 0;
  RowsDown<7> R;
  const int r_off[7] = {SP_S * SP, SP_S * SP, SP_E * SP, SP_B * SP, SP_N * SP, SP_J * SP, SP_C * SP};
  const int r_sh[7] = {0, -1, 0, 0, -1, -1, -1};
  float wE = 0.f, wB = 0.f, wN = 0.f;
  auto flush = [&](int lo) {
    const int r = R.top - lane;
    if (r >= lo) {
      __builtin_nontemporal_store(wE, spec + SP_E * SP + r);
      __builtin_nontemporal_store(wB, spec + SP_B * SP + r);
      __builtin_nontemporal_store(wN, spec + SP_N * SP + r);
    }
  };
  if (SG) R.load(spec, r_off, r_sh, L, lane);
#pragma unroll 1
  for (int i = L; i >= 0; i--) {
    asm volatile("" ::: "memory");
    if (SG && R.spent(i)) { flush(i + 1); R.load(spec, r_off, r_sh, i, lane); }
    if (i < L) {
      xB = wave_sum(backward_emit<Q, false>(T, emL, (const float *)c.emG, seq[i], ctxKlds(c), lane, Mb));
      xJ = fmaf(xJ, cm.loop, xB * cm.move);
      xC = xC * cm.loop;
      xN = fmaf(xN, cm.loop, xB * cm.move);
    }
    float xE = fmaf(xC, cm.EC, xJ * cm.EJ);
    if (i >= 1) backward_cells<Q, false, (Q <= kMaxQP)>(T, sc, Mb, Ib, xE);
    const float big = fmaxf(xB, xN);
    if (big > kRescaleHi) {
      const int e = f32_exponent(big);
      const float r = pow2f_int(-e);
#pragma unroll
      for (int p = 0; p < Q; p++) { Mb[p] *= r; Ib[p] *= r; }
      xB *= r; xJ *= r; xC *= r; xN *= r; xE *= r;
      eb += e;
    }
    const float s_i = ldexpf(invZ, (SG ? R.s(0, i) : ldi(SP_S * SP + i)) + eb - ef_L);
    const float pe = (SG ? R.f(2, i) : ldf(SP_E * SP + i)) * xE * s_i;
    const float pb = (SG ? R.f(3, i) : ldf(SP_B * SP + i)) * xB * s_i;
    float njc = 0.f;
    if (i >= 1) {
      const float s_p = ldexpf(invZ, (SG ? R.s(1, i) : ldi(SP_S * SP + i - 1)) + eb - ef_L);
      njc = (SG ? R.f(4, i) : ldf(SP_N * SP + i - 1)) * xN;
      njc = fmaf(SG ? R.f(5, i) : ldf(SP_J * SP + i - 1), xJ, njc);
      njc = fmaf(SG ? R.f(6, i) : ldf(SP_C * SP + i - 1), xC, njc);
      njc = njc * cm.loop * s_p;
    }
    if (SG) {
      if (lane == R.top - i) { wE = pe; wB = pb; wN = njc; }
    } else {
      __builtin_amdgcn_wave_barrier();
      if (lane == 0) { spec[SP_E * SP + i] = pe; spec[SP_B * SP + i] = pb; spec[SP_N * SP + i] = njc; }
      __builtin_amdgcn_wave_barrier();
    }
  }
  if (SG) { flush(0); __builtin_amdgcn_fence(__ATOMIC_SEQ_CST, "workgroup"); }
}

template <int Q, int TH, bool SG>
__device__ __noinline__ P4Out sweep_backward_null2(const WaveCtx c, lds_u8 *eseq3, int Ld, LenCfg cu, float invZe, int ef_e, float mass_tol) {
  const uint8_t *eseq = (const uint8_t *)eseq3;
  const float *emL = (const float *)c.emL;
  TransTab<Q, false> T;
  T.load(nullptr, (const float *)c.bwL, c.lane);
  const ScanC sc = scan_prepare(lane_product<Q, false>(T, BW_DD));
  const int lane = c.lane, SP = c.SP;
  const float *spec = SG ? (const float *)c.specg : (const float *)c.spec;
  auto ldf = [&](int idx) -> float { return SG ? __builtin_nontemporal_load(spec + idx) : spec[idx]; };
  auto ldi = [&](int idx) -> int { return SG ? __builtin_nontemporal_load(reinterpret_cast<const int *>(spec) + idx) : reinterpret_cast<const int *>(spec)[idx]; };
  auto ldu = [&](int idx) -> unsigned { return SG ? __builtin_nontemporal_load(reinterpret_cast<const unsigned *>(spec) + idx) : reinterpret_cast<const unsigned *>(spec)[idx]; };
  float Mb[Q], Ib[Q], fM[Q];
#pragma unroll
  for (int p = 0; p < Q; p++) { Mb[p] = 0.f; Ib[p] = 0.f; fM[p] = 0.f; }
  float xC = cu.move, xJ = 0.f, xN = 0.f, xB = 0.f, xfac = 0.f, fIs = 0.f;
  const int src = kWave - 1 - lane;
  int S_next = 0;
  RowsDown<7> R;
  const int r_off[7] = {kSpML * SP, kSpMH * SP, SP_S * SP, SP_S * SP, SP_N * SP, SP_J * SP, SP_C * SP};
  const int r_sh[7] = {0, 0, 0, -1, -1, -1, -1};
  if (SG) R.load(spec, r_off, r_sh, Ld, lane);
#pragma unroll 1
  for (int i = Ld; i >= 1; i--) {
    asm volatile("" ::: "memory");
    if (SG && R.spent(i)) R.load(spec, r_off, r_sh, i, lane);
    auto mask_word = [&]() -> unsigned { return SG ? (src < 32 ? R.u(0, i) : R.u(1, i)) : (src < 32 ? ldu(kSpML * SP + i) : ldu(kSpMH * SP + i)); };
    float4 fm4[Q / 4], fi4[Q / 4];
    auto request_row = [&]() {
      const unsigned mword = mask_word();
      const bool have = (mword >> (src & 31)) & 1u;
      const float4 *row = reinterpret_cast<const float4 *>((const float *)c.Fs) + (size_t)i * (2 * (Q / 4) * kWave);
      if (have) {
#pragma unroll
        for (int p4 = 0; p4 < Q / 4; p4++) {
          fm4[p4] = nt_load4(row + fs_piece<Q, !SG>(src, Q / 4 - 1 - p4));
          fi4[p4] = nt_load4(row + fs_piece<Q, !SG>(src, Q / 4 + Q / 4 - 1 - p4));
        }
      } else {
#pragma unroll
        for (int p4 = 0; p4 < Q / 4; p4++) { fm4[p4] = make_float4(0.f, 0.f, 0.f, 0.f); fi4[p4] = fm4[p4]; }
      }
    };
    if (TH < 768) request_row();
    const int S_i = SG ? R.s(2, i) : ldi(SP_S * SP + i);
    const int dS = S_i - (SG ? R.s(3, i) : ldi(SP_S * SP + i - 1));
    if (i < Ld) {
      mirror_scale<Q>(S_next - S_i, Mb, Ib, xJ, xC, xN);
      xB = wave_sum(backward_emit<Q, false>(T, emL, (const float *)c.emG, eseq[i], ctxKlds(c), lane, Mb));
      xJ = fmaf(xJ, cu.loop, xB * cu.move);
      xC = xC * cu.loop;
      xN = fmaf(xN, cu.loop, xB * cu.move);
    }
    float xE = fmaf(xC, cu.EC, xJ * cu.EJ);
    backward_cells<Q, false, (Q <= kMaxQP)>(T, sc, Mb, Ib, xE);
    clamp_backward<Q>(Mb, Ib, xB, xJ, xC, xN);
    const float s_i = invZe;
    const float s_p = ldexpf(invZe, -dS);
    if (TH >= 768 && kMaskedAcc) {
      asm volatile("" ::: "memory");
      const unsigned mword = mask_word();
      if ((mword >> (src & 31)) & 1u) {
        const float4 *row = reinterpret_cast<const float4 *>((const float *)c.Fs) + (size_t)i * (2 * (Q / 4) * kWave);
        float idot = 0.f;
#pragma unroll
        for (int p4 = 0; p4 < Q / 4; p4++) {
          const float4 fm = nt_load4(row + fs_piece<Q, !SG>(src, Q / 4 - 1 - p4));
          const float4 fi = nt_load4(row + fs_piece<Q, !SG>(src, Q / 4 + Q / 4 - 1 - p4));
          fM[4 * p4 + 0] = fmaf(fm.w * Mb[4 * p4 + 0], s_i, fM[4 * p4 + 0]);
          fM[4 * p4 + 1] = fmaf(fm.z * Mb[4 * p4 + 1], s_i, fM[4 * p4 + 1]);
          fM[4 * p4 + 2] = fmaf(fm.y * Mb[4 * p4 + 2], s_i, fM[4 * p4 + 2]);
          fM[4 * p4 + 3] = fmaf(fm.x * Mb[4 * p4 + 3], s_i, fM[4 * p4 + 3]);
          idot = fmaf(fi.w, Ib[4 * p4 + 0], idot); idot = fmaf(fi.z, Ib[4 * p4 + 1], idot);
          idot = fmaf(fi.y, Ib[4 * p4 + 2], idot); idot = fmaf(fi.x, Ib[4 * p4 + 3], idot);
        }
        fIs = fmaf(idot, s_i, fIs);
      }
    } else {
      if (TH >= 768) { asm volatile("" ::: "memory"); request_row(); }
      float idot = 0.f;
#pragma unroll
      for (int p4 = 0; p4 < Q / 4; p4++) {
        fM[4 * p4 + 0] = fmaf(fm4[p4].w * Mb[4 * p4 + 0], s_i, fM[4 * p4 + 0]);
        fM[4 * p4 + 1] = fmaf(fm4[p4].z * Mb[4 * p4 + 1], s_i, fM[4 * p4 + 1]);
        fM[4 * p4 + 2] = fmaf(fm4[p4].y * Mb[4 * p4 + 2], s_i, fM[4 * p4 + 2]);
        fM[4 * p4 + 3] = fmaf(fm4[p4].x * Mb[4 * p4 + 3], s_i, fM[4 * p4 + 3]);
        idot = fmaf(fi4[p4].w, Ib[4 * p4 + 0], idot); idot = fmaf(fi4[p4].z, Ib[4 * p4 + 1], idot);
        idot = fmaf(fi4[p4].y, Ib[4 * p4 + 2], idot); idot = fmaf(fi4[p4].x, Ib[4 * p4 + 3], idot);
      }
      fIs = fmaf(idot, s_i, fIs);
    }
    float nj = (SG ? R.f(4, i) : ldf(SP_N * SP + i - 1)) * xN;
    nj = fmaf(SG ? R.f(5, i) : ldf(SP_J * SP + i - 1), xJ, nj);
    nj = fmaf(SG ? R.f(6, i) : ldf(SP_C * SP + i - 1), xC, nj);
    S_next = S_i;
    xfac = fmaf(nj * cu.loop, s_p, xfac);
  }
  float sm = 0.f;
#pragma unroll
  for (int p = 0; p < Q; p++) sm += fM[p];
  sm = wave_sum(sm);
  const float si = wave_sum(fIs);
  const float mass = sm + si + xfac;
  P4Out o;
  o.mass = mass; o.domcorr = 0.f;
  if (!(fabsf((float)Ld - mass) <= mass_tol * (float)Ld)) return o;
  const float norm = 1.0f / (float)Ld;
  float mine = 1.0f;
  for (int x = 0; x < ctxK(c); x++) {
    float od[Q];
    load_em_rev<Q>(od, emL, (const float *)c.emG, x, ctxKlds(c), lane);
    float s = 0.f;
#pragma unroll
    for (int p = 0; p < Q; p++) s = fmaf(fM[p], od[p], s);
    s = wave_sum(s);
    if (lane == x) mine = (s + si) * norm + xfac * norm;
  }
  float *n2tab = (float *)c.n2tab;
  __builtin_amdgcn_wave_barrier();
  if (lane < ctxK(c)) n2tab[lane] = mine;
  __builtin_amdgcn_wave_barrier();
  if (lane >= ctxK(c) && lane < ctxKp(c)) {
    const uint32_t m = c.degen;
    float s = 0.f; int n = 0;
    for (int x = 0; x < ctxK(c); x++) if (m & (1u << x)) { s += n2tab[x]; n++; }
    mine = n > 0 ? s / (float)n : 1.0f;
  }
  __builtin_amdgcn_wave_barrier();
  if (lane < ctxKp(c)) n2tab[lane] = logf(mine);
  __builtin_amdgcn_wave_barrier();
  float dc = 0.f;
  for (int t = lane; t < Ld; t += kWave) dc += n2tab[eseq[t]];
  o.domcorr = wave_sum(dc);
  return o;
}

template <int QB, int Q, int TH, bool SG, bool BWG = false>
__device__ __noinline__ P4Out sweep_backward_null2_win(const WaveCtx c, lds_u8 *eseq3, int Ld, LenCfg cu, float invZe, float mass_tol, int m0) {
  static_assert(Q % QB == 0 && QB % 4 == 0, "a window lane must stay inside one forward lane block");
  static_assert(!(SG && BWG), "c.specg cannot be both");
  constexpr int Q4 = Q / 4, B4 = QB / 4;
  const uint8_t *eseq = (const uint8_t *)eseq3;
  const int lane = c.lane, SP = c.SP, Klds = ctxKlds(c);
  const float *spec = SG ? (const float *)c.specg : (const float *)c.spec;
  auto ldf = [&](int idx) -> float { return SG ? __builtin_nontemporal_load(spec + idx) : spec[idx]; };
  auto ldi = [&](int idx) -> int { return SG ? __builtin_nontemporal_load(reinterpret_cast<const int *>(spec) + idx) : reinterpret_cast<const int *>(spec)[idx]; };
  auto ldu = [&](int idx) -> unsigned { return SG ? __builtin_nontemporal_load(reinterpret_cast<const unsigned *>(spec) + idx) : reinterpret_cast<const unsigned *>(spec)[idx]; };
  int fwd[B4], frow[B4];
  TransTab<QB, true> T;
  {
    const float4 *bw4 = BWG ? reinterpret_cast<const float4 *>((const float *)c.specg) : reinterpret_cast<const float4 *>((const float *)c.bwL);
#pragma unroll
    for (int p4 = 0; p4 < B4; p4++) {
      const int m4 = (m0 >> 2) + lane * B4 + p4;
      const int rev = (m4 % Q4) * kWave + m4 / Q4;
      const int jf = 16 * Q - 1 - m4;
      fwd[p4] = (jf % Q4) * kWave + jf / Q4;
      frow[p4] = fs_piece<Q, !SG>(jf / Q4, jf % Q4);
#pragma unroll
      for (int a = 0; a < BW_NARR; a++) T.v[a][p4] = bw4[a * Q4 * kWave + rev];
    }
  }
  const int lanef = (16 * Q - 1 - ((m0 >> 2) + lane * B4)) / Q4;
  const ScanC sc = scan_prepare(lane_product<QB, true>(T, BW_DD));
  const LdsF4 em4L((const float *)c.emL);
  const float4 *em4G = reinterpret_cast<const float4 *>((const float *)c.emG);
  float Mb[QB], Ib[QB], fM[QB];
#pragma unroll
  for (int p = 0; p < QB; p++) { Mb[p] = 0.f; Ib[p] = 0.f; fM[p] = 0.f; }
  float xC = cu.move, xJ = 0.f, xN = 0.f, xB = 0.f, xfac = 0.f, fIs = 0.f;
  int S_next = 0;
  float4 fm_n[B4], fi_n[B4];
  bool have_n = false;
  RowsDown<7> R;
  const int r_off[7] = {kSpML * SP, kSpMH * SP, SP_S * SP, SP_S * SP, SP_N * SP, SP_J * SP, SP_C * SP};
  const int r_sh[7] = {-1, -1, 0, -1, -1, -1, -1};
  if (SG) R.load(spec, r_off, r_sh, Ld, lane);
  auto request_row = [&](int r, bool first) {
    const unsigned mword = SG ? (first ? (lanef < 32 ? ldu(kSpML * SP + r) : ldu(kSpMH * SP + r)) : (lanef < 32 ? R.u(0, r + 1) : R.u(1, r + 1)))
                              : (lanef < 32 ? ldu(kSpML * SP + r) : ldu(kSpMH * SP + r));
    have_n = (mword >> (lanef & 31)) & 1u;
    if (have_n) {
      const float4 *row = reinterpret_cast<const float4 *>((const float *)c.Fs) + (size_t)r * (2 * Q4 * kWave);
#pragma unroll
      for (int p4 = 0; p4 < B4; p4++) { fm_n[p4] = nt_load4(row + frow[p4]); fi_n[p4] = nt_load4(row + (SG ? Q4 * kWave : Q4) + frow[p4]); }
    }
  };
  request_row(Ld, true);
#pragma unroll 1
  for (int i = Ld; i >= 1; i--) {
    asm volatile("" ::: "memory");
    if (SG && R.spent(i)) R.load(spec, r_off, r_sh, i, lane);
    float4 fm_c[B4], fi_c[B4];
#pragma unroll
    for (int p4 = 0; p4 < B4; p4++) { fm_c[p4] = fm_n[p4]; fi_c[p4] = fi_n[p4]; }
    const bool have = have_n;
    if (i > 1) request_row(i - 1, false);
    const int S_i = SG ? R.s(2, i) : ldi(SP_S * SP + i);
    const int dS = S_i - (SG ? R.s(3, i) : ldi(SP_S * SP + i - 1));
    if (i < Ld) {
      mirror_scale<QB>(S_next - S_i, Mb, Ib, xJ, xC, xN);
      const int x = __builtin_amdgcn_readfirstlane((int)eseq[i]);
      float part = 0.f;
      auto emit = [&](auto em_ld) {
#pragma unroll
        for (int p4 = 0; p4 < B4; p4++) {
          const float4 E = T.v[BW_E][p4];
          const float4 O = em_ld(p4);
          Mb[4 * p4 + 0] *= O.w; part = fmaf(E.x, Mb[4 * p4 + 0], part);
          Mb[4 * p4 + 1] *= O.z; part = fmaf(E.y, Mb[4 * p4 + 1], part);
          Mb[4 * p4 + 2] *= O.y; part = fmaf(E.z, Mb[4 * p4 + 2], part);
          Mb[4 * p4 + 3] *= O.x; part = fmaf(E.w, Mb[4 * p4 + 3], part);
        }
      };
      if (x < Klds) emit([&](int p4) { return em4L[x * (Q * 16) + fwd[p4]]; });
      else emit([&](int p4) { return em4G[(size_t)x * (Q * 16) + fwd[p4]]; });
      xB = wave_sum(part);
      xJ = fmaf(xJ, cu.loop, xB * cu.move);
      xC = xC * cu.loop;
      xN = fmaf(xN, cu.loop, xB * cu.move);
    }
    const float xE = fmaf(xC, cu.EC, xJ * cu.EJ);
    backward_cells<QB, true, false>(T, sc, Mb, Ib, xE);
    clamp_backward<QB>(Mb, Ib, xB, xJ, xC, xN);
    const float s_i = invZe;
    const float s_p = ldexpf(invZe, -dS);
    if (have) {
      float idot = 0.f;
#pragma unroll
      for (int p4 = 0; p4 < B4; p4++) {
        const float4 fm = fm_c[p4];
        const float4 fi = fi_c[p4];
        fM[4 * p4 + 0] = fmaf(fm.w * Mb[4 * p4 + 0], s_i, fM[4 * p4 + 0]);
        fM[4 * p4 + 1] = fmaf(fm.z * Mb[4 * p4 + 1], s_i, fM[4 * p4 + 1]);
        fM[4 * p4 + 2] = fmaf(fm.y * Mb[4 * p4 + 2], s_i, fM[4 * p4 + 2]);
        fM[4 * p4 + 3] = fmaf(fm.x * Mb[4 * p4 + 3], s_i, fM[4 * p4 + 3]);
        idot = fmaf(fi.w, Ib[4 * p4 + 0], idot); idot = fmaf(fi.z, Ib[4 * p4 + 1], idot);
        idot = fmaf(fi.y, Ib[4 * p4 + 2], idot); idot = fmaf(fi.x, Ib[4 * p4 + 3], idot);
      }
      fIs = fmaf(idot, s_i, fIs);
    }
    float nj = (SG ? R.f(4, i) : ldf(SP_N * SP + i - 1)) * xN;
    nj = fmaf(SG ? R.f(5, i) : ldf(SP_J * SP + i - 1), xJ, nj);
    nj = fmaf(SG ? R.f(6, i) : ldf(SP_C * SP + i - 1), xC, nj);
    S_next = S_i;
    xfac = fmaf(nj * cu.loop, s_p, xfac);
  }
  float sm = 0.f;
#pragma unroll
  for (int p = 0; p < QB; p++) sm += fM[p];
  sm = wave_sum(sm);
  const float si = wave_sum(fIs);
  const float mass = sm + si + xfac;
  P4Out o;
  o.mass = mass; o.domcorr = 0.f;
  if (!(fabsf((float)Ld - mass) <= mass_tol * (float)Ld)) return o;
  const float norm = 1.0f / (float)Ld;
  float mine = 1.0f;
  for (int x = 0; x < ctxK(c); x++) {
    float s = 0.f;
    auto dot = [&](auto em_ld) {
#pragma unroll
      for (int p4 = 0; p4 < B4; p4++) {
        const float4 O = em_ld(p4);
        s = fmaf(fM[4 * p4 + 0], O.w, s); s = fmaf(fM[4 * p4 + 1], O.z, s);
        s = fmaf(fM[4 * p4 + 2], O.y, s); s = fmaf(fM[4 * p4 + 3], O.x, s);
      }
    };
    if (x < Klds) dot([&](int p4) { return em4L[x * (Q * 16) + fwd[p4]]; });
    else dot([&](int p4) { return em4G[(size_t)x * (Q * 16) + fwd[p4]]; });
    s = wave_sum(s);
    if (lane == x) mine = (s + si) * norm + xfac * norm;
  }
  float *n2tab = (float *)c.n2tab;
  __builtin_amdgcn_wave_barrier();
  if (lane < ctxK(c)) n2tab[lane] = mine;
  __builtin_amdgcn_wave_barrier();
  if (lane >= ctxK(c) && lane < ctxKp(c)) {
    const uint32_t m = c.degen;
    float s = 0.f; int n = 0;
    for (int x = 0; x < ctxK(c); x++) if (m & (1u << x)) { s += n2tab[x]; n++; }
    mine = n > 0 ? s / (float)n : 1.0f;
  }
  __builtin_amdgcn_wave_barrier();
  if (lane < ctxKp(c)) n2tab[lane] = logf(mine);
  __builtin_amdgcn_wave_barrier();
  float dc = 0.f;
  for (int t = lane; t < Ld; t += kWave) dc += n2tab[eseq[t]];
  o.domcorr = wave_sum(dc);
  return o;
}

enum { QS_ACTIVE = 0, QS_LD, QS_M0, QS_INVZ, QS_LOOP, QS_MOVE, QS_SEQ, QS_PAD, QS_MASS, QS_DOMCORR, QS_INTS = 16 };
template <int Q, int TH>
__device__ __noinline__ void sweep_backward_null2_quad(const WaveCtx c, lds_i *slots3, lds_u8 *seqs3, lds_f *n2, int slab_stride, int spec_stride, float mass_tol) {
  static_assert(Q % 4 == 0, "float4 pieces");
  constexpr int Q4 = Q / 4;
  const int lane = c.lane, SP = c.SP, Klds = ctxKlds(c);
  const int t = lane >> 4, r = lane & 15;
  lds_i *slot = slots3 + t * QS_INTS;
  const bool active = slot[QS_ACTIVE] != 0;
  const int Ld = active ? min(max(slot[QS_LD], 0), SP - 1) : 0;
  const int m0 = active ? min(max(slot[QS_M0], 0), 16 * (Q - 4) * 4) & ~15 : 0;
  const float invZe = __builtin_bit_cast(float, slot[QS_INVZ]);
  LenCfg cu;
  cu.loop = __builtin_bit_cast(float, slot[QS_LOOP]); cu.move = __builtin_bit_cast(float, slot[QS_MOVE]); cu.EJ = 0.0f; cu.EC = 1.0f;
  lds_u8 *eseq = seqs3 + (active ? slot[QS_SEQ] : 0);
  typedef __attribute__((address_space(1))) unsigned glb_u;
  typedef __attribute__((address_space(1))) v4f_t glb_v4;
  typedef __attribute__((address_space(1))) char glb_c;
  const glb_c *FsU = (const glb_c *)uniform_ptr((const glb_f *)c.Fs);
  const glb_c *specU = (const glb_c *)uniform_ptr((const glb_f *)c.specg);
  constexpr int kRowBytes = 32 * Q4 * kWave;
  const unsigned qspec = 4u * (unsigned)(t * __builtin_amdgcn_readfirstlane(spec_stride) + Ld);
  const unsigned qslab = 4u * (unsigned)(t * __builtin_amdgcn_readfirstlane(slab_stride)) + (unsigned)Ld * kRowBytes;
  auto ldu = [&](int arr_word, int back) -> unsigned {
    return __builtin_nontemporal_load((const glb_u *)(uniform_ptr(specU + 4 * ((long)__builtin_amdgcn_readfirstlane(arr_word) - (long)__builtin_amdgcn_readfirstlane(back))) + qspec));
  };
  auto ldf_ = [&](int arr_word, int back) -> float { return __builtin_bit_cast(float, ldu(arr_word, back)); };
  const unsigned qmask = qspec + 4u * (unsigned)(((kWave - 1 - ((m0 >> 4) + r)) < 32 ? kSpML : kSpMH) * SP);
  static_assert(Q == 16, "the quarter-wave sweep is written for 16 cells per lane");
  const int lr = (m0 >> 4) + r, lanef = kWave - 1 - lr;
  struct TabRow {
    LdsF4 base; int lr;
    __device__ __forceinline__ TabRow(const float *lds, int lr_) : base(lds), lr(lr_) {}
    __device__ __forceinline__ float4 ld(int a, int p4) const { return base[(a * 4 + p4) * kWave + lr]; }
  } T((const float *)c.bwL, lr);
  float A = 1.f;
#pragma unroll
  for (int p4 = 0; p4 < 4; p4++) { const float4 d = T.ld(BW_DD, p4); A *= d.x; A *= d.y; A *= d.z; A *= d.w; }
  const ScanR sc = scan_prepare_row(A);
  const LdsF4 em4L((const float *)c.emL);
  const float4 *em4G = reinterpret_cast<const float4 *>((const float *)c.emG);
  float Mb[16], Ib[16], fM[16];
#pragma unroll
  for (int p = 0; p < 16; p++) { Mb[p] = 0.f; Ib[p] = 0.f; fM[p] = 0.f; }
  float xC = cu.move, xJ = 0.f, xN = 0.f, xB = 0.f, xfac = 0.f, fIs = 0.f;
  auto mask_word = [&](int back) -> unsigned {
    return __builtin_nontemporal_load((const glb_u *)(uniform_ptr(specU - 4 * (long)__builtin_amdgcn_readfirstlane(back)) + qmask));
  };
  float4 fm[4], fi[4];
  const unsigned foff = qslab + 128u * (unsigned)lanef;
  auto ld4 = [&](const glb_c *rowp, unsigned off) -> float4 {
    const v4f_t v = __builtin_nontemporal_load((const glb_v4 *)(rowp + off));
    return make_float4(v.x, v.y, v.z, v.w);
  };
  auto request_row = [&](int back) {
#pragma unroll
    for (int p4 = 0; p4 < 4; p4++) {
      const glb_c *rowp = uniform_ptr(FsU - (long)__builtin_amdgcn_readfirstlane(back) * kRowBytes + 16 * (3 - p4));
      fm[p4] = ld4(rowp, foff);
      fi[p4] = ld4(uniform_ptr(rowp + 64), foff);
    }
  };
  int Lmax = Ld;
  Lmax = max(Lmax, __shfl_xor(Lmax, 16));
  Lmax = max(Lmax, __shfl_xor(Lmax, 32));
  int S_i, S_p;
  float n_p, j_p, c_p;
  unsigned w_i;
  request_row(0);
  w_i = mask_word(0);
  S_i = (int)ldu(SP_S * SP, 0);
  S_p = (int)ldu(SP_S * SP, 1);
  n_p = ldf_(SP_N * SP, 1);
  j_p = ldf_(SP_J * SP, 1);
  c_p = ldf_(SP_C * SP, 1);
#pragma unroll 1
  for (int j = 0; j < Lmax; j++) {
    asm volatile("" ::: "memory");
    const int i = Ld - j;
    if (i >= 1) {
      if (j > 0) {
        const int x = eseq[i];
        float part = 0.f;
        auto emit = [&](auto em_ld) {
#pragma unroll
          for (int p4 = 0; p4 < 4; p4++) {
            const float4 E = T.ld(BW_E, p4);
            const float4 O = em_ld(p4);
            Mb[4 * p4 + 0] *= O.w; part = fmaf(E.x, Mb[4 * p4 + 0], part);
            Mb[4 * p4 + 1] *= O.z; part = fmaf(E.y, Mb[4 * p4 + 1], part);
            Mb[4 * p4 + 2] *= O.y; part = fmaf(E.z, Mb[4 * p4 + 2], part);
            Mb[4 * p4 + 3] *= O.x; part = fmaf(E.w, Mb[4 * p4 + 3], part);
          }
        };
        if (x < Klds) emit([&](int p4) { return em4L[x * (Q * 16) + (3 - p4) * kWave + lanef]; });
        else emit([&](int p4) { return em4G[(size_t)x * (Q * 16) + (3 - p4) * kWave + lanef]; });
        xB = row_sum(part);
        xJ = fmaf(xJ, cu.loop, xB * cu.move);
        xC = xC * cu.loop;
        xN = fmaf(xN, cu.loop, xB * cu.move);
      }
      const float xE = fmaf(xC, cu.EC, xJ * cu.EJ);
      backward_cells_row(T, sc, Mb, Ib, xE);
      clamp_backward<16>(Mb, Ib, xB, xJ, xC, xN);
      const float s_i = invZe;
      const float s_p = ldexpf(invZe, S_p - S_i);
      if ((w_i >> (lanef & 31)) & 1u) {
        float idot = 0.f;
#pragma unroll
        for (int p4 = 0; p4 < 4; p4++) {
          const float4 fm_ = fm[p4], fi_ = fi[p4];
          fM[4 * p4 + 0] = fmaf(fm_.w * Mb[4 * p4 + 0], s_i, fM[4 * p4 + 0]);
          fM[4 * p4 + 1] = fmaf(fm_.z * Mb[4 * p4 + 1], s_i, fM[4 * p4 + 1]);
          fM[4 * p4 + 2] = fmaf(fm_.y * Mb[4 * p4 + 2], s_i, fM[4 * p4 + 2]);
          fM[4 * p4 + 3] = fmaf(fm_.x * Mb[4 * p4 + 3], s_i, fM[4 * p4 + 3]);
          idot = fmaf(fi_.w, Ib[4 * p4 + 0], idot); idot = fmaf(fi_.z, Ib[4 * p4 + 1], idot);
          idot = fmaf(fi_.y, Ib[4 * p4 + 2], idot); idot = fmaf(fi_.x, Ib[4 * p4 + 3], idot);
        }
        fIs = fmaf(idot, s_i, fIs);
      }
      float nj = n_p * xN;
      nj = fmaf(j_p, xJ, nj);
      nj = fmaf(c_p, xC, nj);
      xfac = fmaf(nj * cu.loop, s_p, xfac);
      mirror_scale<16>(S_i - S_p, Mb, Ib, xJ, xC, xN);
    }
    if (j + 1 < Lmax) {
      request_row(j + 1);
      w_i = mask_word(j + 1);
      S_i = (int)ldu(SP_S * SP, j + 1);
      S_p = (int)ldu(SP_S * SP, j + 2);
      n_p = ldf_(SP_N * SP, j + 2);
      j_p = ldf_(SP_J * SP, j + 2);
      c_p = ldf_(SP_C * SP, j + 2);
    }
  }
  float sm = 0.f;
#pragma unroll
  for (int p = 0; p < 16; p++) sm += fM[p];
  sm = row_sum(sm);
  const float si = row_sum(fIs);
  const float mass = sm + si + xfac;
  const bool ok = active && fabsf((float)Ld - mass) <= mass_tol * (float)Ld;
  lds_f *n2tab = n2 + 32 * t;
  const int K = ctxK(c), Kp = ctxKp(c);
  const float norm = 1.0f / (float)(Ld > 0 ? Ld : 1);
  for (int x = 0; x < K; x++) {
    float s_ = 0.f;
    auto dot = [&](auto em_ld) {
#pragma unroll
      for (int p4 = 0; p4 < 4; p4++) {
        const float4 O = em_ld(p4);
        s_ = fmaf(fM[4 * p4 + 0], O.w, s_); s_ = fmaf(fM[4 * p4 + 1], O.z, s_);
        s_ = fmaf(fM[4 * p4 + 2], O.y, s_); s_ = fmaf(fM[4 * p4 + 3], O.x, s_);
      }
    };
    if (x < Klds) dot([&](int p4) { return em4L[x * (Q * 16) + (3 - p4) * kWave + lanef]; });
    else dot([&](int p4) { return em4G[(size_t)x * (Q * 16) + (3 - p4) * kWave + lanef]; });
    s_ = row_sum(s_);
    if (r == 0) n2tab[x] = (s_ + si) * norm + xfac * norm;
  }
  __builtin_amdgcn_wave_barrier();
  const uint32_t mdeg = (uint32_t)__shfl((int)c.degen, min(K + r, kWave - 1));
  if (K + r < Kp) {
    float s_ = 0.f; int n = 0;
    for (int x = 0; x < K; x++) if (mdeg & (1u << x)) { s_ += n2tab[x]; n++; }
    n2tab[K + r] = n > 0 ? s_ / (float)n : 1.0f;
  }
  __builtin_amdgcn_wave_barrier();
  for (int d = r; d < Kp; d += 16) n2tab[d] = logf(n2tab[d]);
  __builtin_amdgcn_wave_barrier();
  float dc = 0.f;
  for (int u = r; u < Ld; u += 16) dc += n2tab[eseq[u]];
  const float domcorr = row_sum(dc);
  if (r == 0) {
    slot[QS_MASS] = __builtin_bit_cast(int, mass);
    slot[QS_DOMCORR] = __builtin_bit_cast(int, ok ? domcorr : 0.f);
  }
  __builtin_amdgcn_wave_barrier();
}

struct WinDec { float eps; };
template <int QB, int Q, int TH, bool INPL = false, bool BWG = false, bool TMPG = false>
__device__ __noinline__ WinDec sweep_backward_decode_win(const WaveCtx c, lds_u8 *seq3, int L, LenCfg cm, float invZ, int ef_L, int m0) {
  static_assert(Q % QB == 0 && QB % 4 == 0, "a window lane must stay inside one forward lane block");
  static_assert(!(BWG && TMPG) && !(INPL && TMPG), "c.specg serves one purpose per call");
  constexpr int Q4 = Q / 4, B4 = QB / 4;
  const uint8_t *seq = (const uint8_t *)seq3;
  const int lane = c.lane, SP = c.SP, Klds = ctxKlds(c);
  const float *spec = (const float *)c.spec;
  float *tmp = (float *)c.spec + kSpArr * SP;
  float *tE = INPL ? (float *)c.spec + SP_E * SP : tmp, *tB = INPL ? (float *)c.spec + SP_B * SP : tmp + SP, *tN = INPL ? (float *)c.spec + SP_N * SP : tmp + 2 * SP;
  glb_f *gE = c.specg, *gB = c.specg + SP, *gN = c.specg + 2 * SP;
  const int *speci = reinterpret_cast<const int *>(spec);
  int fwd[B4];
  TransTab<QB, true> T;
  {
    const float4 *bw4 = BWG ? reinterpret_cast<const float4 *>((const float *)c.specg) : reinterpret_cast<const float4 *>((const float *)c.bwL);
#pragma unroll
    for (int p4 = 0; p4 < B4; p4++) {
      const int m4 = (m0 >> 2) + lane * B4 + p4;
      const int rev = (m4 % Q4) * kWave + m4 / Q4;
      const int jf = 16 * Q - 1 - m4;
      fwd[p4] = (jf % Q4) * kWave + jf / Q4;
#pragma unroll
      for (int a = 0; a < BW_NARR; a++) T.v[a][p4] = bw4[a * Q4 * kWave + rev];
    }
  }
  const ScanC sc = scan_prepare(lane_product<QB, true>(T, BW_DD));
  const LdsF4 em4L((const float *)c.emL);
  const float4 *em4G = reinterpret_cast<const float4 *>((const float *)c.emG);
  float Mb[QB], Ib[QB];
#pragma unroll
  for (int p = 0; p < QB; p++) { Mb[p] = 0.f; Ib[p] = 0.f; }
  float xC = cm.move, xJ = 0.f, xN = 0.f, xB = 0.f;
  int eb = 0;
  float ratio = 0.f;
#pragma unroll 1
  for (int i = L; i >= 0; i--) {
    asm volatile("" ::: "memory");
    if (i < L) {
      const int x = __builtin_amdgcn_readfirstlane((int)seq[i]);
      float part = 0.f;
      auto emit = [&](auto em_ld) {
#pragma unroll
        for (int p4 = 0; p4 < B4; p4++) {
          const float4 E = T.v[BW_E][p4];
          const float4 O = em_ld(p4);
          Mb[4 * p4 + 0] *= O.w; part = fmaf(E.x, Mb[4 * p4 + 0], part);
          Mb[4 * p4 + 1] *= O.z; part = fmaf(E.y, Mb[4 * p4 + 1], part);
          Mb[4 * p4 + 2] *= O.y; part = fmaf(E.z, Mb[4 * p4 + 2], part);
          Mb[4 * p4 + 3] *= O.x; part = fmaf(E.w, Mb[4 * p4 + 3], part);
        }
      };
      if (x < Klds) emit([&](int p4) { return em4L[x * (Q * 16) + fwd[p4]]; });
      else emit([&](int p4) { return em4G[(size_t)x * (Q * 16) + fwd[p4]]; });
      xB = wave_sum(part);
      xJ = fmaf(xJ, cm.loop, xB * cm.move);
      xC = xC * cm.loop;
      xN = fmaf(xN, cm.loop, xB * cm.move);
    }
    float xE = fmaf(xC, cm.EC, xJ * cm.EJ);
    if (i >= 1) backward_cells<QB, true, false>(T, sc, Mb, Ib, xE);
    const float big = fmaxf(xB, xN);
    if (big > kRescaleHi) {
      const int e = f32_exponent(big);
      const float r = pow2f_int(-e);
#pragma unroll
      for (int p = 0; p < QB; p++) { Mb[p] *= r; Ib[p] *= r; }
      xB *= r; xJ *= r; xC *= r; xN *= r; xE *= r;
      eb += e;
    }
    const float s_i = ldexpf(invZ, speci[SP_S * SP + i] + eb - ef_L);
    const float pe = spec[SP_E * SP + i] * xE * s_i;
    const float pb = spec[SP_B * SP + i] * xB * s_i;
    float njc = 0.f;
    if (i >= 1) {
      const float s_p = ldexpf(invZ, speci[SP_S * SP + i - 1] + eb - ef_L);
      njc = spec[SP_N * SP + i - 1] * xN;
      njc = fmaf(spec[SP_J * SP + i - 1], xJ, njc);
      njc = fmaf(spec[SP_C * SP + i - 1], xC, njc);
      njc = njc * cm.loop * s_p;
    } else {
      ratio = spec[SP_N * SP] * xN * s_i;
    }
    __builtin_amdgcn_wave_barrier();
    if (TMPG) { if (lane == 0) { gE[i] = pe; gB[i] = pb; gN[i] = njc; } }
    else if (lane == 0) { tE[i] = pe; tB[i] = pb; tN[i] = njc; }
    __builtin_amdgcn_wave_barrier();
  }
  WinDec o;
  o.eps = 1.0f - ratio;
  return o;
}

template <int TH, bool INPL = false, bool TMPG = false>
__device__ __noinline__ RegOut region_scan_cert(lds_f *spec3, int SP, int L, lds_i *regs3, int lane, float eps, glb_f *tmpg = nullptr) {
  float *tmp = TMPG ? (float *)tmpg : (float *)spec3 + kSpArr * SP;
  float *tE = INPL ? (float *)spec3 + SP_E * SP : tmp, *tB = INPL ? (float *)spec3 + SP_B * SP : tmp + SP, *tN = INPL ? (float *)spec3 + SP_N * SP : tmp + 2 * SP;
  if (TMPG) __builtin_amdgcn_fence(__ATOMIC_SEQ_CST, "workgroup");
  int *regs = (int *)regs3;
  const float rt1 = 0.25f, rt2 = 0.10f, rt3 = 0.20f;
  const float slack = 2e-5f;
  const float e1 = eps + slack, e2 = 2.0f * eps + slack;
  int nenv = 0, nreg = 0, flags = 0, doubt = 0, doubt_md = 0;
  float btot = 0.f, etot = 0.f;
  int i0 = -1;
  bool trig = false;
  auto ldt = [&](const float *p_) -> float { return TMPG ? __builtin_nontemporal_load(p_) : *p_; };
  auto stt = [&](float *p_, float v_) { if (TMPG) __builtin_nontemporal_store(v_, p_); else *p_ = v_; };
  const float pb0 = ldt(tB);
  __builtin_amdgcn_wave_barrier();
  if (lane == 0) { stt(tE, 0.f); stt(tN, 0.f); }
  for (int j0 = 1; j0 <= L; j0 += kWave) {
    const int jj = j0 + lane;
    const bool valid = jj <= L;
    const float nv = valid ? ldt(tN + jj) : 0.f;
    const float bv = valid ? (jj - 1 == 0 ? pb0 : ldt(tB + jj - 1)) : 0.f;
    const float ev = valid ? ldt(tE + jj) : 0.f;
    float jout = 0.f, cout = 0.f;
    const int cnt = L - j0 + 1 < kWave ? L - j0 + 1 : kWave;
    for (int t = 0; t < cnt; t++) {
      const int j = j0 + t;
      const float mocc = 1.0f - readlane_f(nv, t);
      const float bold = btot, eold = etot;
      btot += readlane_f(bv, t);
      etot += readlane_f(ev, t);
      if (lane == t) { jout = btot; cout = etot; }
      if (!trig) {
        const float d = mocc - (btot - bold);
        if (d >= rt2 - slack && d < rt2 + e2) doubt = 1;
        if (d < rt2) i0 = j;
        else if (i0 == -1) i0 = j;
        if (mocc >= rt1 - slack && mocc < rt1 + e1) doubt = 1;
        if (mocc >= rt1) trig = true;
      } else {
        const float d = mocc - (etot - eold);
        if (d >= rt2 - slack && d < rt2 + e2) doubt = 1;
        if (d < rt2) {
          if (nenv < WH_MAX_ENVELOPES) {
            if (lane == 0) { regs[2 * nenv] = i0; regs[2 * nenv + 1] = j; }
            nenv++;
          } else flags |= WH_FLAG_TRUNC;
          nreg++;
          i0 = -1;
          trig = false;
        }
      }
    }
    if (valid) { stt(tN + jj, jout); stt(tE + jj, cout); }
  }
  __builtin_amdgcn_wave_barrier();
  if (TMPG) __builtin_amdgcn_fence(__ATOMIC_SEQ_CST, "workgroup");
  int multi_mask = 0;
  for (int e = 0; e < nenv; e++) {
    const int ri = regs[2 * e], rj = regs[2 * e + 1];
    float mx = -1.0f;
    const float e0 = ldt(tE + ri - 1), bj = ldt(tN + rj);
    for (int z = ri + lane; z <= rj; z += kWave) {
      const float u = ldt(tE + z) - e0, v = bj - ldt(tN + z - 1);
      mx = fmaxf(mx, fminf(u, v));
    }
    mx = wave_max(mx);
    const float up = mx + (float)(rj - ri + 1) * eps + slack;
    if (mx >= rt3) { flags |= WH_FLAG_MULTI; multi_mask |= 1 << e; if (mx < rt3 + slack) doubt_md = 1; }
    else if (up >= rt3) doubt_md = 1;
  }
  RegOut o;
  o.nenv = nenv; o.nreg = nreg; o.flags = flags | (multi_mask << 8) | (doubt << 24) | (doubt_md << 25);
  return o;
}

template <int TH, bool SG>
__device__ __noinline__ RegOut region_scan(lds_f *spec3, glb_f *specg, int SP, int L, lds_i *regs3, int lane) {
  float *spec = SG ? (float *)specg : (float *)spec3;
  auto ldf = [&](int idx) -> float { return SG ? __builtin_nontemporal_load(spec + idx) : spec[idx]; };
  int *regs = (int *)regs3;
  const float rt3 = 0.20f;
  int nenv = 0, nreg = 0, flags = 0;
  region_scan_global(spec, SP, L, regs, lane, nenv, nreg, flags);
  __builtin_amdgcn_wave_barrier();
  if (SG) __builtin_amdgcn_fence(__ATOMIC_SEQ_CST, "workgroup");
  int multi_mask = 0;
  for (int e = 0; e < nenv; e++) {
    const int ri = regs[2 * e], rj = regs[2 * e + 1];
    float mx = -1.0f;
    const float e0 = ldf(SP_C * SP + ri - 1), bj = ldf(SP_J * SP + rj);
    for (int z = ri + lane; z <= rj; z += kWave) {
      const float u = ldf(SP_C * SP + z) - e0, v = bj - ldf(SP_J * SP + z - 1);
      mx = fmaxf(mx, fminf(u, v));
    }
    mx = wave_max(mx);
    if (mx >= rt3) { flags |= WH_FLAG_MULTI; multi_mask |= 1 << e; }
  }
  RegOut o;
  o.nenv = nenv; o.nreg = nreg; o.flags = flags | (multi_mask << 8);
  return o;
}

struct EnvCounters { unsigned n_w256, n_w512, n_wfail, n_full; unsigned long long spill; };
constexpr int kBandEvShift = 48;
__device__ __forceinline__ unsigned take_band_events(EnvCounters &ec) {
  const unsigned ev = (unsigned)(ec.spill >> kBandEvShift);
  ec.spill &= (1ull << kBandEvShift) - 1;
  return ev;
}
__device__ __forceinline__ int band_path_bits(unsigned ev) {
  const unsigned n0 = ev & 0xFF, nfail = ev >> 8;
  return (nfail ? WH_PATH_BAND_FAIL : 0) | (n0 > nfail ? WH_PATH_BAND_KEPT : 0);
}
__device__ __forceinline__ unsigned long long mask_in_band(unsigned long long um, int band) {
  const int blo = band & 255, bhi = (band >> 8) & 255;
  const unsigned long long bm = (bhi >= 63 ? ~0ull : ((1ull << (bhi + 1)) - 1)) & ~((1ull << blo) - 1);
  return (um & bm) ? (um & bm) : um;
}
template <int Q, int TH, bool SG>
__device__ __forceinline__ P4Out envelope_backward(const ScoreArgs &a, const WaveCtx &c, const uint8_t *eseq, int Ld, LenCfg cu, const FwdOut &f3,
                                                   bool dense, bool skip_window, EnvCounters &ec, int lane, int band) {
  const int SP = c.SP;
  const bool banded = band != (63 << 8);
  const float tol = dense ? INFINITY : spill_tol(banded);
  P4Out p4;
  bool have4 = false;
  if constexpr (Q >= 8) {
    if (!dense && !a.no_window && !skip_window) {
      const unsigned *su = reinterpret_cast<const unsigned *>(SG ? (const float *)c.specg : (const float *)c.spec);
      unsigned long long um = ((unsigned long long)su[kSpMH * SP] << 32) | su[kSpML * SP];
      um = mask_in_band(um, band);
      if (um != 0) {
        int lo = __builtin_ctzll(um), hi = 63 - __builtin_clzll(um);
        lo = lo > 1 ? lo - 2 : 0; hi = hi < 63 ? hi + 1 : 63;
        const int nodes = (hi - lo + 1) * Q;
        if (a.stats && lane == 0) { atomicAdd(a.stats + 12, (unsigned long long)(hi - lo + 1)); atomicAdd(a.stats + 14, 1ull); atomicAdd(a.stats + 15, (unsigned long long)__builtin_popcountll(um)); }
        if (nodes <= 4 * kWave) {
          const int m0 = min((63 - hi) * Q, kWave * (Q - 4));
          p4 = sweep_backward_null2_win<4, Q, TH, SG>(c, (lds_u8 *)eseq, Ld, cu, 1.0f / (f3.xC * cu.move), kWinTol7, m0);
          have4 = fabsf((float)Ld - p4.mass) <= kWinTol7 * (float)Ld;
          if (have4) ec.n_w256++; else ec.n_wfail++;
          if (a.stats && lane == 0) {
            atomicAdd(a.stats + (have4 ? 0 : 2), 1ull);
            const float dev = fabsf((float)Ld - p4.mass) / (float)Ld;
            atomicAdd(a.stats + (dev < 3e-7f ? 16 : dev < 1e-6f ? 17 : dev < 3e-6f ? 18 : dev < 1e-5f ? 19 : dev < 2e-5f ? 20 : 21), 1ull);
          }
        } else if (Q % 8 == 0 && Q > 8 && nodes <= 8 * kWave) {
          const int m0 = min((63 - hi) * Q, kWave * (Q - 8));
          p4 = sweep_backward_null2_win<(Q % 8 == 0 ? 8 : 4), Q, TH, SG>(c, (lds_u8 *)eseq, Ld, cu, 1.0f / (f3.xC * cu.move), kWinTol7, m0);
          have4 = fabsf((float)Ld - p4.mass) <= kWinTol7 * (float)Ld;
          if (have4) ec.n_w512++; else ec.n_wfail++;
          if (a.stats && lane == 0) atomicAdd(a.stats + (have4 ? 1 : 2), 1ull);
        }
      }
    }
  }
  if (!have4) {
    p4 = sweep_backward_null2<Q, TH, SG>(c, (lds_u8 *)eseq, Ld, cu, 1.0f / (f3.xC * cu.move), f3.ef, tol);
    ec.n_full++;
    if (a.stats && lane == 0) {
      atomicAdd(a.stats + 3, 1ull);
      const float dev = fabsf((float)Ld - p4.mass) / (float)Ld;
      atomicAdd(a.stats + (dev < 3e-7f ? 22 : dev < 1e-6f ? 23 : dev < 3e-6f ? 24 : dev < 1e-5f ? 25 : dev < 2e-5f ? 26 : 27), 1ull);
    }
  }
  return p4;
}

__device__ __forceinline__ void assemble_score(int L, int Ld_tot, float seqbias_sum, float sum_score, float sb2, float fwdsc, float nullsc,
                                               wh_pair_detail *dp, int &flags, int &decibits) {
  const double LOG2 = 0.69314718055994529;
  const float lomega = (float)log(1.0 / 256.0);
  const float seqbias = flogsum0_v7(lomega + seqbias_sum);
  float pre_score = (float)(((double)fwdsc - (double)nullsc) / LOG2);
  float seq_score = (float)(((double)fwdsc - (double)(nullsc + seqbias)) / LOG2);
  sb2 = flogsum0_v7(lomega + sb2);
  sum_score += (float)((double)(L - Ld_tot) * dlog((double)((float)L / (float)(L + 3))));
  const float pre2 = (float)(((double)sum_score - (double)nullsc) / LOG2);
  sum_score = (float)(((double)sum_score - (double)(nullsc + sb2)) / LOG2);
  if (Ld_tot > 0 && sum_score > seq_score) { seq_score = sum_score; pre_score = pre2; flags |= WH_FLAG_OVERRIDE; }
  decibits = (int)rint((double)seq_score * 10.0);
  flags |= WH_FLAG_REPORTED;
  if (dp) { dp->seq_score = seq_score; dp->pre_score = pre_score; dp->seqbias_nats = seqbias; }
}

#define WH_TICK7(slot) do { if (a.stats) { const long long t_now = __builtin_readcyclecounter(); if (lane == 0) atomicAdd(a.stats + (slot), (unsigned long long)(t_now - t_last)); t_last = t_now; } } while (0)
constexpr int kAllLanes = 63 << 8;
struct P1Mask { unsigned long long um; unsigned steady; };
template <int Q>
__device__ __forceinline__ int spill_band(const ScoreArgs &a, P1Mask pm) {
  unsigned long long um1 = pm.um;
  const bool steady = pm.steady && !(a.spill_band & 2);
  if (steady) um1 = (1ull << (pm.steady & 255)) | (1ull << ((pm.steady >> 8) & 255));
  if (Q < 8 || um1 == 0 || !a.spill_band) return kAllLanes;
  int below = (80 + Q - 1) / Q, above = (48 + Q - 1) / Q;
  if (a.spill_band >= 1000) { below = (a.spill_band / 1000 + Q - 1) / Q; above = (a.spill_band % 1000 + Q - 1) / Q; }
  const int lo = __builtin_ctzll(um1) - below, hi = 63 - __builtin_clzll(um1) + above;
  int band = (lo > 0 ? lo : 0) | ((hi < 63 ? hi : 63) << 8);
  if (steady && !(a.spill_band & 4)) band |= (__builtin_ctzll(um1) + 1 + (32 + Q - 1) / Q) << 16;
  return band;
}
__device__ __forceinline__ P1Mask p1_mask(const WaveCtx &c) {
  const unsigned *su = reinterpret_cast<const unsigned *>((const float *)c.n2tab) + kUmSlot;
  return P1Mask{((unsigned long long)su[1] << 32) | su[0], su[-1]};
}
template <int Q, int TH, bool SG>
__device__ __forceinline__ float envelope_attempts(const ScoreArgs &a, WaveCtx &c, const uint8_t *eseq, int Ld, LenCfg cu, int band, int first,
                                                   EnvCounters &ec, int lane, int &flags, long long &t_last, float &envsc) {
  const double LOG2 = 0.69314718055994529;
  float domcorr = 0.f;
#pragma unroll 1
  for (int attempt = first; attempt < 3; attempt++) {
    const float keep_scale = attempt < 2 ? (a.keep_scale > 0.f ? a.keep_scale : kKeepScale7) : -1.0f;
    const FwdOut f3 = uniform_fwd(sweep_forward<Q, true, TH, SG>(c, (lds_u8 *)eseq, Ld, cu, keep_scale, attempt == 0 ? band : kAllLanes));
    ec.spill += (unsigned long long)f3.nst * (8 * Q) + (attempt == 0 ? (f3.xC > 0.f ? 1ull << kBandEvShift : 0ull) : attempt == 1 && band != kAllLanes ? 1ull << (kBandEvShift + 8) : 0ull);
    __builtin_amdgcn_fence(__ATOMIC_SEQ_CST, "workgroup");
    envsc = uniform_f((float)((double)f3.ef * LOG2 + dlog((double)(f3.xC * cu.move))));
    domcorr = 0.f;
    if (!(f3.xC > 0.f)) break;
    WH_TICK7(7);
    const P4Out p4 = envelope_backward<Q, TH, SG>(a, c, eseq, Ld, cu, f3, attempt == 2, false, ec, lane, attempt == 0 ? band : kAllLanes);
    domcorr = uniform_f(p4.domcorr);
    WH_TICK7(8);
    if (attempt < 2 && !(fabsf((float)Ld - p4.mass) <= spill_tol(attempt == 0) * (float)Ld)) continue;
    if (attempt == 2) flags |= WH_FLAG_EXACT;
    break;
  }
  return domcorr;
}

template <int Q, int TH, bool SG>
__device__ __forceinline__ void score_envelopes(const ScoreArgs &a, WaveCtx &c, uint8_t *seq, int *regs, int L, int lane, int h, int64_t qi, int nenv, int nreg,
                                                int multi_mask, float fwdsc, float nullsc, float fwd_bits_out, wh_pair_detail *dp, int &flags, int &decibits,
                                                EnvCounters &ec, long long &t_last, P1Mask um1) {
  const int band = spill_band<Q>(a, SG ? P1Mask{0ull, 0u} : um1);
  {
  const LenCfg cu = len_config(L, false);
  float seqbias_sum = 0.f, sum_score = 0.f, sb2 = 0.f;
  int Ld_tot = 0;
  const bool queue_pair = multi_mask != 0 && a.rrecs != nullptr;
  float *envres = reinterpret_cast<float *>(regs + 3 * WH_MAX_ENVELOPES);
  for (int e = 0; e < nenv; e++) {
    if (queue_pair && ((multi_mask >> e) & 1)) { if (lane == 0) { envres[e] = 0.f; envres[WH_MAX_ENVELOPES + e] = 0.f; } continue; }
    const int ri = regs[2 * e], rj = regs[2 * e + 1];
    const int Ld = rj - ri + 1;
    const uint8_t *eseq = seq + (ri - 1);
    float envsc = -INFINITY;
    const float domcorr = envelope_attempts<Q, TH, SG>(a, c, eseq, Ld, cu, band, band != kAllLanes ? 0 : 1, ec, lane, flags, t_last, envsc);
    seqbias_sum += domcorr;
    if (envsc - domcorr > 0.0f) { sum_score += envsc; Ld_tot += Ld; sb2 += domcorr; }
    if (dp) { dp->env_i[e] = ri; dp->env_j[e] = rj; dp->envsc[e] = envsc; dp->domcorr[e] = domcorr; }
    if (queue_pair && lane == 0) { envres[e] = envsc; envres[WH_MAX_ENVELOPES + e] = domcorr; }
  }
  if (queue_pair) {
    __builtin_amdgcn_wave_barrier();
    int slot = 0;
    if (lane == 0) slot = atomicAdd(a.rcount, 1);
    slot = __shfl(slot, 0);
    if (slot < a.rcap && lane == 0) {
      ResolveRec *rr = a.rrecs + slot;
      rr->q = qi; rr->h = h; rr->fwdsc = fwdsc; rr->fwd_bits = fwd_bits_out; rr->nreg = nreg; rr->nenv = nenv;
      rr->multi_mask = multi_mask; rr->flags = flags;
      for (int e = 0; e < nenv; e++) { rr->ri[e] = regs[2 * e]; rr->rj[e] = regs[2 * e + 1]; rr->envsc[e] = envres[e]; rr->domcorr[e] = envres[WH_MAX_ENVELOPES + e]; }
    }
  } else assemble_score(L, Ld_tot, seqbias_sum, sum_score, sb2, fwdsc, nullsc, dp, flags, decibits);
  }
}

struct FrontState {
  float eps_prev, eps_prev2;
  unsigned n_pairs_h;
  unsigned n_p2w, n_p2rej;
};
template <int Q, int TH, bool SG, bool TMPG>
__device__ __forceinline__ RegOut score_regions(const ScoreArgs &a, const WaveCtx &c, uint8_t *seq, int *regs, int L, int lane, LenCfg cm, const FwdOut &f1,
                                                FrontState &fs, long long &t_last, glb_f *tmpg = nullptr) {
  const int SP = c.SP;
  bool saved = false;
  RegOut ro;
  bool have_ro = false;
  if constexpr (Q >= 8 && !SG) {
    const bool try_win = fminf(fs.eps_prev, fs.eps_prev2) * (float)L < 0.17f || (fs.n_pairs_h & 15) == 0;
    fs.n_pairs_h++;
    if ((a.p2win == 1 || TMPG) && !a.no_window && try_win) {
      const unsigned *su = reinterpret_cast<const unsigned *>((const float *)c.n2tab) + kUmSlot;
      const unsigned long long um = ((unsigned long long)su[1] << 32) | su[0];
      if (um != 0) {
        int lo = __builtin_ctzll(um), hi = 63 - __builtin_clzll(um);
        lo = lo > 1 ? lo - 2 : 0; hi = hi < 63 ? hi + 1 : 63;
        const int nodes = (hi - lo + 1) * Q;
        WinDec wd;
        wd.eps = 1.0f;
        if (TMPG && nodes <= (Q % 8 == 0 && Q > 8 ? 8 : 4) * kWave) {
          const float *spec = (const float *)c.spec;
          for (int arr = 0; arr < kSpArr; arr++)
            for (int u = lane; u <= L; u += kWave) __builtin_nontemporal_store(spec[arr * SP + u], tmpg + arr * SP + u);
          saved = true;
        }
        if (nodes <= 4 * kWave) wd = sweep_backward_decode_win<4, Q, TH, TMPG, false, false>(c, (lds_u8 *)seq, L, cm, 1.0f / (f1.xC * cm.move), f1.ef, min((63 - hi) * Q, kWave * (Q - 4)));
        else if (Q % 8 == 0 && Q > 8 && nodes <= 8 * kWave) wd = sweep_backward_decode_win<(Q % 8 == 0 ? 8 : 4), Q, TH, TMPG, false, false>(c, (lds_u8 *)seq, L, cm, 1.0f / (f1.xC * cm.move), f1.ef, min((63 - hi) * Q, kWave * (Q - 8)));
        if (nodes <= (Q % 8 == 0 && Q > 8 ? 8 : 4) * kWave) { fs.eps_prev2 = fs.eps_prev; fs.eps_prev = fabsf(wd.eps); }
        if (wd.eps > -1e-4f && wd.eps < 0.01f) {
          ro = region_scan_cert<TH, TMPG, false>(c.spec, SP, L, (lds_i *)regs, lane, fmaxf(wd.eps, 0.f));
          have_ro = ((ro.flags >> 24) & 3) == 0;
          if (a.stats && lane == 0) {
            if ((ro.flags >> 24) & 1) atomicAdd(a.stats + 32, 1ull);
            if ((ro.flags >> 25) & 1) atomicAdd(a.stats + 33, 1ull);
            atomicAdd(a.stats + 34, (unsigned long long)(wd.eps * 1e9f));
            atomicAdd(a.stats + 35, 1ull);
          }
          ro.flags &= 0xFFFFFF;
        } else if (a.stats && lane == 0) atomicAdd(a.stats + 36, 1ull);
        if (have_ro) fs.n_p2w++; else fs.n_p2rej++;
      }
    }
  }
  if (!have_ro) {
    if (TMPG && saved) {
      __builtin_amdgcn_fence(__ATOMIC_SEQ_CST, "workgroup");
      float *spec = (float *)c.spec;
      __builtin_amdgcn_wave_barrier();
      for (int arr = 0; arr < kSpArr; arr++)
        for (int u = lane; u <= L; u += kWave) spec[arr * SP + u] = __builtin_nontemporal_load(tmpg + arr * SP + u);
      __builtin_amdgcn_wave_barrier();
    }
    sweep_backward_decode<Q, TH, SG>(c, (lds_u8 *)seq, L, cm, 1.0f / (f1.xC * cm.move), f1.ef);
    WH_TICK7(5);
    ro = region_scan<TH, SG>(c.spec, c.specg, SP, L, (lds_i *)regs, lane);
  } else WH_TICK7(5);
  return ro;
}

__device__ __forceinline__ int *path_words(int *regs) { return regs + 2 * WH_MAX_ENVELOPES; }
__device__ __forceinline__ void path_snapshot(int *regs, const EnvCounters &ec, const FrontState &fs) {
  int *pw = path_words(regs);
  pw[0] = (int)ec.n_w256; pw[1] = (int)ec.n_w512; pw[2] = (int)ec.n_wfail; pw[3] = (int)ec.n_full; pw[4] = (int)fs.n_p2w;
}
__device__ __forceinline__ int path_bits(const int *regs, const EnvCounters &ec, const FrontState &fs, bool p2_ran, int flags, bool queued, unsigned band_ev) {
  const int *pw = regs + 2 * WH_MAX_ENVELOPES;
  int path = p2_ran ? ((int)fs.n_p2w != pw[4] ? WH_PATH_P2_WIN : WH_PATH_P2_FULL) : 0;
  if ((int)ec.n_w256 != pw[0]) path |= WH_PATH_P4_W256;
  if ((int)ec.n_w512 != pw[1]) path |= WH_PATH_P4_W512;
  if ((int)ec.n_wfail != pw[2]) path |= WH_PATH_P4_WFAIL;
  if ((int)ec.n_full != pw[3]) path |= WH_PATH_P4_FULL;
  if (flags & WH_FLAG_EXACT) path |= WH_PATH_DENSE;
  if (queued) path |= WH_PATH_MULTI;
  return path | band_path_bits(band_ev);
}

#ifndef WH_SWEEPS_ONLY

template <int Q, int TH, bool SG>
__global__ __launch_bounds__(TH) void score_kernel7(ScoreArgs a) {
  extern __shared__ __attribute__((aligned(16))) float smem_raw[];
  volatile int *s_item_p = reinterpret_cast<volatile int *>(smem_raw);
  float *smem = smem_raw + 4;
  const int lane = threadIdx.x & 63, wave = __builtin_amdgcn_readfirstlane((int)(threadIdx.x >> 6)), nwaves = blockDim.x >> 6;
  constexpr int TBL = Q * kWave;
  float *emL = smem;
  float *trL = smem + (size_t)a.K * TBL;
  constexpr int NARR = FW_NARR + (Q <= kMaxQP ? 1 : 0);
  float *wbase = trL + 2 * NARR * TBL + (size_t)wave * a.wave_lds;
  const int SP = a.SP;
  WaveCtx c;
  c.emL = (lds_f *)emL; c.fwL = (lds_f *)trL; c.bwL = (lds_f *)(trL + NARR * TBL);
  const int spArrAll = kSpArr + (a.p2win == 1 ? 3 : 0);
  c.spec = (lds_f *)wbase; c.n2tab = (lds_f *)(wbase + (SG ? 0 : spArrAll * SP));
  c.specg = SG ? (glb_f *)(a.spec_scratch + ((size_t)blockIdx.x * nwaves + wave) * a.spec_stride) : nullptr;
  c.degen = 0;
  for (int t = 0; t < 32; t++) if (t == lane) c.degen = a.degen[t];
  c.Fs = (glb_f *)(a.scratch + ((size_t)blockIdx.x * nwaves + wave) * a.scratch_stride);
  c.SP = SP; c.alpha = a.K | (a.Kp << 8) | (a.K << 16); c.lane = lane;
  int *regs = reinterpret_cast<int *>(wbase + (SG ? 0 : spArrAll * SP) + 32);
  uint8_t *seq = reinterpret_cast<uint8_t *>(regs + kRegsInts);
  const double LOG2 = 0.69314718055994529;
  int cur_h = -1;
  const DevHMM *hm = nullptr;
  EnvCounters ec = {0, 0, 0, 0, 0};
  FrontState fs = {0.f, 0.f, 0u, 0u, 0u};

  for (;;) {
    __syncthreads();
    if (threadIdx.x == 0) { *s_item_p = atomicAdd(a.counter, 1); s_item_p[1] = 0; }
    __syncthreads();
    const int item = __builtin_amdgcn_readfirstlane(*s_item_p);
    if (item >= a.n_items) break;
    const int h = __builtin_amdgcn_readfirstlane(a.hmm_list[item / a.n_qblocks]);
    const int64_t q_lo = (int64_t)(item % a.n_qblocks) * a.QB;
    const int64_t q_hi = q_lo + a.QB < a.nq ? q_lo + a.QB : a.nq;
    if (h != cur_h) {
      hm = a.hmms + h;
      const float4 *src = reinterpret_cast<const float4 *>(a.tables + hm->em_off);
      float4 *dst = reinterpret_cast<float4 *>(emL);
      for (int t = threadIdx.x; t < a.K * TBL / 4; t += blockDim.x) dst[t] = src[t];
      const float4 *s1 = reinterpret_cast<const float4 *>(a.tables + hm->fw_off);
      const float4 *s2 = reinterpret_cast<const float4 *>(a.tables + hm->bw_off);
      float4 *d1 = reinterpret_cast<float4 *>(trL);
      for (int t = threadIdx.x; t < NARR * TBL / 4; t += blockDim.x) { d1[t] = s1[t]; d1[NARR * TBL / 4 + t] = s2[t]; }
      cur_h = h;
      fs.eps_prev = 0.f; fs.eps_prev2 = 0.f; fs.n_pairs_h = 0;
      __syncthreads();
    }
    c.emG = (const glb_f *)(a.tables + hm->em_off);

    for (;;) {
      int k_ = 0;
      if (lane == 0) k_ = atomicAdd(const_cast<int *>(s_item_p) + 1, 1);
      const int64_t qpos = q_lo + __builtin_amdgcn_readfirstlane(k_);
      if (qpos >= q_hi) break;
      const int64_t qi = a.qorder ? uniform_i64(a.qorder[qpos]) : qpos;
      const int64_t off = uniform_i64(a.offsets[qi]);
      const int L = __builtin_amdgcn_readfirstlane((int)(a.offsets[qi + 1] - off));
      const size_t out = (size_t)qi * a.H + h;
      int flags = 0, decibits = 0;
      float fwd_bits_out = -INFINITY;
      if (lane == 0) path_snapshot(regs, ec, fs);
      wh_pair_detail *dp = (a.detail && lane == 0) ? a.detail + out : nullptr;
      if (dp) {
        dp->fwd_bits = -INFINITY; dp->seq_score = 0.f; dp->pre_score = 0.f; dp->seqbias_nats = 0.f;
        dp->nregions = 0; dp->nenv = 0;
      }
      if (L > 0 && L <= a.Lcap) {
        for (int t = lane; t < L; t += kWave) {
          int r = a.residues[off + t];
          seq[t] = (uint8_t)(r < a.Kp ? r : a.Kp - 1);
        }
        __builtin_amdgcn_wave_barrier();
        long long t_last = a.stats ? __builtin_readcyclecounter() : 0;
        const LenCfg cm = len_config(L, true);
        const FwdOut f1 = uniform_fwd(sweep_forward<Q, false, TH, SG>(c, (lds_u8 *)seq, L, cm, 0.f));
        const double fwd_nats = (double)f1.ef * LOG2 + dlog((double)(f1.xC * cm.move));
        const float fwdsc = uniform_f((float)fwd_nats);
        const float p1 = (float)L / (float)(L + 1);
        const float nullsc = uniform_f((float)((double)(float)L * dlog((double)p1) + dlog(1.0 - (double)p1)));
        fwd_bits_out = uniform_f((float)((fwd_nats - (double)nullsc) / LOG2));
        if (dp) dp->fwd_bits = fwd_bits_out;
        if (f1.xC > 0.f && isfinite(fwdsc)) {
          WH_TICK7(4);
          RegOut ro;
          if constexpr (!SG && Q >= 20) {
            if (a.p2win == 2) ro = score_regions<Q, TH, false, true>(a, c, seq, regs, L, lane, cm, f1, fs, t_last, (glb_f *)(a.p2_backup + ((size_t)blockIdx.x * nwaves + wave) * a.p2_backup_stride));
            else ro = score_regions<Q, TH, SG, false>(a, c, seq, regs, L, lane, cm, f1, fs, t_last);
          } else ro = score_regions<Q, TH, SG, false>(a, c, seq, regs, L, lane, cm, f1, fs, t_last);
          const int nenv = ro.nenv, nreg = ro.nreg, multi_mask = ro.flags >> 8;
          flags |= ro.flags & 0xFF;
          if (dp) { dp->nregions = nreg; dp->nenv = nenv; }
          if (nenv > 0) {
            WH_TICK7(6);
            score_envelopes<Q, TH, SG>(a, c, seq, regs, L, lane, h, qi, nenv, nreg, multi_mask, fwdsc, nullsc, fwd_bits_out, dp, flags, decibits, ec, t_last, p1_mask(c));
          }
        }
      }
      if (lane == 0) {
        a.decibits[out] = decibits;
        a.flags[out] = (uint8_t)flags;
        if (a.fwd_bits) a.fwd_bits[out] = fwd_bits_out;
      }
      const unsigned band_ev = take_band_events(ec);
      if (uint16_t *rec = path_record(a)) {
        if (lane == 0) rec[out] = (uint16_t)path_bits(regs, ec, fs, isfinite(fwd_bits_out), flags, (flags & WH_FLAG_MULTI) && a.rrecs != nullptr, band_ev);
      }
    }
  }
  if (a.paths && lane == 0) {
    if (ec.n_w256) atomicAdd(a.paths + 0, (unsigned long long)ec.n_w256);
    if (ec.n_w512) atomicAdd(a.paths + 1, (unsigned long long)ec.n_w512);
    if (ec.n_wfail) atomicAdd(a.paths + 2, (unsigned long long)ec.n_wfail);
    if (ec.n_full) atomicAdd(a.paths + 3, (unsigned long long)ec.n_full);
    if (ec.spill) atomicAdd(a.paths + 6, ec.spill);
    if (fs.n_p2w) atomicAdd(a.paths + 4, (unsigned long long)fs.n_p2w);
    if (fs.n_p2rej) atomicAdd(a.paths + 5, (unsigned long long)fs.n_p2rej);
  }
}

enum { QR_QLO = 0, QR_QHI, QR_L, QR_NREG, QR_FLAGS, QR_FWDSC, QR_NULLSC, QR_FWDBITS, QR_ENVSC, QR_RI, QR_RJ, QR_XC3, QR_EF3, QR_BAND, QR_INTS = 16 };
template <int Q, int TH>
__global__ __launch_bounds__(TH) void score_kernel7q(ScoreArgs a) {
  extern __shared__ __attribute__((aligned(16))) float smem_raw[];
  volatile int *s_item_p = reinterpret_cast<volatile int *>(smem_raw);
  float *smem = smem_raw + 4;
  const int lane = threadIdx.x & 63, wave = threadIdx.x >> 6, nwaves = blockDim.x >> 6;
  constexpr int TBL = Q * kWave;
  float *emL = smem;
  float *trL = smem + (size_t)a.K * TBL;
  float *wbase = trL + 2 * FW_NARR * TBL + (size_t)wave * a.wave_lds;
  const int SP = a.SP;
  const int seqw = (a.Lcap + 3) / 4 + 4;
  WaveCtx c;
  c.emL = (lds_f *)emL; c.fwL = (lds_f *)trL; c.bwL = (lds_f *)(trL + FW_NARR * TBL);
  c.spec = (lds_f *)wbase; c.n2tab = (lds_f *)(wbase + kSpArr * SP);
  const size_t wid = (size_t)blockIdx.x * nwaves + wave;
  glb_f *specg0 = (glb_f *)(a.spec_scratch + wid * a.spec_stride) + SP;
  const int spec_stride1 = kSpArr * SP;
  glb_f *tmpg = specg0 + 4 * spec_stride1;
  c.specg = nullptr;
  c.degen = 0;
  for (int t = 0; t < 32; t++) if (t == lane) c.degen = a.degen[t];
  const int slab1 = (int)(a.scratch_stride / 5);
  glb_f *Fs0 = (glb_f *)(a.scratch + wid * a.scratch_stride) + slab1;
  glb_f *FsW = Fs0 - slab1;
  c.Fs = FsW;
  c.SP = SP; c.alpha = a.K | (a.Kp << 8) | (a.K << 16); c.lane = lane;
  int *regs = reinterpret_cast<int *>(wbase + kSpArr * SP + 128);
  int *qslots = regs + kRegsInts;
  int *qrecs = qslots + 4 * QS_INTS;
  uint8_t *seqs = reinterpret_cast<uint8_t *>(qrecs + 4 * QR_INTS);
  const double LOG2 = 0.69314718055994529;
  int cur_h = -1;
  const DevHMM *hm = nullptr;
  EnvCounters ec = {0, 0, 0, 0, 0};
  FrontState fs = {0.f, 0.f, 0u, 0u, 0u};
  const long long t_kernel0 = a.stats ? (long long)__builtin_readcyclecounter() : 0;

  for (;;) {
    const long long t_bar0 = a.stats ? (long long)__builtin_readcyclecounter() : 0;
    __syncthreads();
    if (threadIdx.x == 0) { *s_item_p = atomicAdd(a.counter, 1); s_item_p[1] = 0; }
    __syncthreads();
    const int item = *s_item_p;
    if (a.stats && lane == 0) atomicAdd(a.stats + 39, (unsigned long long)((long long)__builtin_readcyclecounter() - t_bar0));
    if (item >= a.n_items) break;
    const int h = a.hmm_list[item / a.n_qblocks];
    const int64_t q_lo = (int64_t)(item % a.n_qblocks) * a.QB;
    const int64_t q_hi = q_lo + a.QB < a.nq ? q_lo + a.QB : a.nq;
    if (h != cur_h) {
      hm = a.hmms + h;
      const float4 *src = reinterpret_cast<const float4 *>(a.tables + hm->em_off);
      float4 *dst = reinterpret_cast<float4 *>(emL);
      for (int t = threadIdx.x; t < a.K * TBL / 4; t += blockDim.x) dst[t] = src[t];
      const float4 *s1 = reinterpret_cast<const float4 *>(a.tables + hm->fw_off);
      const float4 *s2 = reinterpret_cast<const float4 *>(a.tables + hm->bw_off);
      float4 *d1 = reinterpret_cast<float4 *>(trL);
      for (int t = threadIdx.x; t < FW_NARR * TBL / 4; t += blockDim.x) { d1[t] = s1[t]; d1[FW_NARR * TBL / 4 + t] = s2[t]; }
      cur_h = h;
      fs.eps_prev = 0.f; fs.eps_prev2 = 0.f; fs.n_pairs_h = 0;
      __syncthreads();
    }
    c.emG = (const glb_f *)(a.tables + hm->em_off);

    for (;;) {
      int k_ = 0;
      if (lane == 0) k_ = atomicAdd(const_cast<int *>(s_item_p) + 1, 4);
      const int64_t base = q_lo + __builtin_amdgcn_readfirstlane(k_);
      if (base >= q_hi) break;
      int waiting = 0;
      if (lane < 4) qslots[lane * QS_INTS + QS_ACTIVE] = 0;
      __builtin_amdgcn_wave_barrier();
      for (int t = 0; t < 4; t++) {
        const int64_t qpos = base + t;
        if (qpos >= q_hi) break;
        const int64_t qi = a.qorder ? a.qorder[qpos] : qpos;
        const int64_t off = a.offsets[qi];
        const int L = (int)(a.offsets[qi + 1] - off);
        const size_t out = (size_t)qi * a.H + h;
        uint8_t *seq = seqs + t * seqw * 4;
        int flags = 0, decibits = 0;
        float fwd_bits_out = -INFINITY;
        bool deferred = false;
        wh_pair_detail *dp = (a.detail && lane == 0) ? a.detail + out : nullptr;
        if (dp) {
          dp->fwd_bits = -INFINITY; dp->seq_score = 0.f; dp->pre_score = 0.f; dp->seqbias_nats = 0.f;
          dp->nregions = 0; dp->nenv = 0;
        }
        if (L > 0 && L <= a.Lcap) {
          for (int u = lane; u < L; u += kWave) {
            int r = a.residues[off + u];
            seq[u] = (uint8_t)(r < a.Kp ? r : a.Kp - 1);
          }
          __builtin_amdgcn_wave_barrier();
          long long t_last = a.stats ? __builtin_readcyclecounter() : 0;
          const LenCfg cm = len_config(L, true);
          const FwdOut f1 = sweep_forward<Q, false, TH, false>(c, (lds_u8 *)seq, L, cm, 0.f);
          const double fwd_nats = (double)f1.ef * LOG2 + dlog((double)(f1.xC * cm.move));
          const float fwdsc = (float)fwd_nats;
          const float p1 = (float)L / (float)(L + 1);
          const float nullsc = (float)((double)(float)L * dlog((double)p1) + dlog(1.0 - (double)p1));
          fwd_bits_out = (float)((fwd_nats - (double)nullsc) / LOG2);
          if (dp) dp->fwd_bits = fwd_bits_out;
          if (f1.xC > 0.f && isfinite(fwdsc)) {
            WH_TICK7(4);
            const RegOut ro = score_regions<Q, TH, false, true>(a, c, seq, regs, L, lane, cm, f1, fs, t_last, tmpg);
            const int nenv = ro.nenv, nreg = ro.nreg, multi_mask = ro.flags >> 8;
            flags |= ro.flags & 0xFF;
            if (dp) { dp->nregions = nreg; dp->nenv = nenv; }
            if (nenv == 1 && multi_mask == 0 && !a.no_window) {
              WH_TICK7(6);
              const int ri = regs[0], rj = regs[1];
              const int Ld = rj - ri + 1;
              const uint8_t *eseq = seq + (ri - 1);
              const LenCfg cu = len_config(L, false);
              c.Fs = Fs0 + (size_t)t * slab1;
              const float keep_scale = a.keep_scale > 0.f ? a.keep_scale : kKeepScale7;
              const int band = spill_band<Q>(a, p1_mask(c));
              const FwdOut f3 = sweep_forward<Q, true, TH, false>(c, (lds_u8 *)eseq, Ld, cu, keep_scale, band);
              ec.spill += (unsigned long long)f3.nst * (8 * Q);
              __builtin_amdgcn_fence(__ATOMIC_SEQ_CST, "workgroup");
              const float envsc = (float)((double)f3.ef * LOG2 + dlog((double)(f3.xC * cu.move)));
              WH_TICK7(7);
              float domcorr = 0.f;
              bool done = !(f3.xC > 0.f);
              if (!done) {
                const unsigned *su = reinterpret_cast<const unsigned *>((const float *)c.spec);
                const unsigned long long um = mask_in_band(((unsigned long long)su[kSpMH * SP] << 32) | su[kSpML * SP], band);
                int m0 = -1;
                if (um != 0) {
                  int lo = __builtin_ctzll(um), hi = 63 - __builtin_clzll(um);
                  lo = lo > 1 ? lo - 2 : 0; hi = hi < 63 ? hi + 1 : 63;
                  if ((hi - lo + 1) * Q <= 4 * kWave) m0 = min((63 - hi) * Q, kWave * (Q - 4));
                }
                if (m0 >= 0) {
                  glb_f *dst = specg0 + (size_t)t * spec_stride1;
                  const float *spec = (const float *)c.spec;
                  for (int arr = 0; arr < kSpArr; arr++)
                    for (int u = lane; u <= Ld; u += kWave) __builtin_nontemporal_store(spec[arr * SP + u], dst + arr * SP + u);
                  if (lane == 0) {
                    int *sl = qslots + t * QS_INTS;
                    sl[QS_ACTIVE] = 1; sl[QS_LD] = Ld; sl[QS_M0] = m0;
                    sl[QS_INVZ] = __builtin_bit_cast(int, 1.0f / (f3.xC * cu.move));
                    sl[QS_LOOP] = __builtin_bit_cast(int, cu.loop); sl[QS_MOVE] = __builtin_bit_cast(int, cu.move);
                    sl[QS_SEQ] = t * seqw * 4 + (ri - 1);
                    int *qr = qrecs + t * QR_INTS;
                    qr[QR_QLO] = (int)(unsigned)(qi & 0xFFFFFFFF); qr[QR_QHI] = (int)(qi >> 32);
                    qr[QR_L] = L; qr[QR_NREG] = nreg; qr[QR_FLAGS] = flags;
                    qr[QR_FWDSC] = __builtin_bit_cast(int, fwdsc); qr[QR_NULLSC] = __builtin_bit_cast(int, nullsc);
                    qr[QR_FWDBITS] = __builtin_bit_cast(int, fwd_bits_out); qr[QR_ENVSC] = __builtin_bit_cast(int, envsc);
                    qr[QR_RI] = ri; qr[QR_RJ] = rj; qr[QR_XC3] = __builtin_bit_cast(int, f3.xC); qr[QR_EF3] = f3.ef; qr[QR_BAND] = band;
                  }
                  waiting |= 1 << t;
                  deferred = true;
                  WH_TICK7(10);
                } else {
                  const bool banded = band != kAllLanes;
                  const P4Out p4 = envelope_backward<Q, TH, false>(a, c, eseq, Ld, cu, f3, false, false, ec, lane, band);
                  domcorr = p4.domcorr;
                  if (!(fabsf((float)Ld - p4.mass) <= spill_tol(banded) * (float)Ld)) {
                    float envsc2;
                    domcorr = envelope_attempts<Q, TH, false>(a, c, eseq, Ld, cu, band, banded ? 1 : 2, ec, lane, flags, t_last, envsc2);
                  }
                  done = true;
                }
              }
              if (done) {
                WH_TICK7(8);
                float sum_score = 0.f, sb2 = 0.f; int Ld_tot = 0;
                if (envsc - domcorr > 0.0f) { sum_score = envsc; Ld_tot = Ld; sb2 = domcorr; }
                if (dp) { dp->env_i[0] = ri; dp->env_j[0] = rj; dp->envsc[0] = envsc; dp->domcorr[0] = domcorr; }
                assemble_score(L, Ld_tot, domcorr, sum_score, sb2, fwdsc, nullsc, dp, flags, decibits);
              }
              c.Fs = FsW;
            } else if (nenv > 0) {
              WH_TICK7(6);
              score_envelopes<Q, TH, false>(a, c, seq, regs, L, lane, h, qi, nenv, nreg, multi_mask, fwdsc, nullsc, fwd_bits_out, dp, flags, decibits, ec, t_last, p1_mask(c));
            }
          }
        }
        if (lane == 0) {
          if (!deferred) { a.decibits[out] = decibits; a.flags[out] = (uint8_t)flags; }
          if (a.fwd_bits) a.fwd_bits[out] = fwd_bits_out;
        }
      }
      if (waiting) {
        long long t_last = a.stats ? __builtin_readcyclecounter() : 0;
        __builtin_amdgcn_wave_barrier();
        __builtin_amdgcn_fence(__ATOMIC_SEQ_CST, "workgroup");
        WaveCtx cq = c;
        cq.specg = specg0;
        cq.Fs = Fs0;
        WH_TICK7(10);
        sweep_backward_null2_quad<Q, TH>(cq, (lds_i *)qslots, (lds_u8 *)seqs, (lds_f *)(wbase + kSpArr * SP), slab1, spec_stride1, kWinTol7);
        WH_TICK7(9);
        if (a.stats && lane == 0) atomicAdd(a.stats + 37, (unsigned long long)__builtin_popcount(waiting));
        for (int t = 0; t < 4; t++) {
          if (!((waiting >> t) & 1)) continue;
          const int *qr = qrecs + t * QR_INTS;
          const int *sl = qslots + t * QS_INTS;
          const int64_t qi = ((int64_t)qr[QR_QHI] << 32) | (unsigned)qr[QR_QLO];
          const size_t out = (size_t)qi * a.H + h;
          const int L = qr[QR_L], Ld = sl[QS_LD], ri = qr[QR_RI], rj = qr[QR_RJ];
          int flags = qr[QR_FLAGS], decibits = 0;
          const float fwdsc = __builtin_bit_cast(float, qr[QR_FWDSC]), nullsc = __builtin_bit_cast(float, qr[QR_NULLSC]);
          const float envsc = __builtin_bit_cast(float, qr[QR_ENVSC]);
          const float mass = __builtin_bit_cast(float, sl[QS_MASS]);
          float domcorr = __builtin_bit_cast(float, sl[QS_DOMCORR]);
          wh_pair_detail *dp = (a.detail && lane == 0) ? a.detail + out : nullptr;
          if (fabsf((float)Ld - mass) <= kWinTol7 * (float)Ld) ec.n_w256++;
          else {
            ec.n_wfail++;
            uint8_t *seq = seqs + t * seqw * 4;
            const uint8_t *eseq = seq + (ri - 1);
            const LenCfg cu = len_config(L, false);
            float *spec = (float *)c.spec;
            const glb_f *src = specg0 + (size_t)t * spec_stride1;
            __builtin_amdgcn_wave_barrier();
            for (int arr = 0; arr < kSpArr; arr++)
              for (int u = lane; u <= Ld; u += kWave) spec[arr * SP + u] = __builtin_nontemporal_load(src + arr * SP + u);
            __builtin_amdgcn_wave_barrier();
            c.Fs = Fs0 + (size_t)t * slab1;
            FwdOut f3; f3.xC = __builtin_bit_cast(float, qr[QR_XC3]); f3.ef = qr[QR_EF3];
            const int band = qr[QR_BAND];
            const bool banded = band != kAllLanes;
            const P4Out p4 = envelope_backward<Q, TH, false>(a, c, eseq, Ld, cu, f3, false, true, ec, lane, band);
            domcorr = p4.domcorr;
            if (!(fabsf((float)Ld - p4.mass) <= spill_tol(banded) * (float)Ld)) {
              float envsc2;
              domcorr = envelope_attempts<Q, TH, false>(a, c, eseq, Ld, cu, band, banded ? 1 : 2, ec, lane, flags, t_last, envsc2);
            }
            c.Fs = FsW;
          }
          float sum_score = 0.f, sb2 = 0.f; int Ld_tot = 0;
          if (envsc - domcorr > 0.0f) { sum_score = envsc; Ld_tot = Ld; sb2 = domcorr; }
          if (dp) { dp->env_i[0] = ri; dp->env_j[0] = rj; dp->envsc[0] = envsc; dp->domcorr[0] = domcorr; }
          assemble_score(L, Ld_tot, domcorr, sum_score, sb2, fwdsc, nullsc, dp, flags, decibits);
          if (lane == 0) { a.decibits[out] = decibits; a.flags[out] = (uint8_t)flags; }
        }
        WH_TICK7(11);
      }
    }
  }
  (void)take_band_events(ec);
  if (a.paths && lane == 0) {
    if (ec.n_w256) atomicAdd(a.paths + 0, (unsigned long long)ec.n_w256);
    if (ec.n_w512) atomicAdd(a.paths + 1, (unsigned long long)ec.n_w512);
    if (ec.n_wfail) atomicAdd(a.paths + 2, (unsigned long long)ec.n_wfail);
    if (ec.n_full) atomicAdd(a.paths + 3, (unsigned long long)ec.n_full);
    if (ec.spill) atomicAdd(a.paths + 6, ec.spill);
    if (fs.n_p2w) atomicAdd(a.paths + 4, (unsigned long long)fs.n_p2w);
    if (fs.n_p2rej) atomicAdd(a.paths + 5, (unsigned long long)fs.n_p2rej);
  }
  if (a.stats && lane == 0) atomicAdd(a.stats + 38, (unsigned long long)(__builtin_readcyclecounter() - t_kernel0));
}

template <int Q, int TH>
static hipError_t launch7q(const ScoreArgs &a, int blocks, int threads, size_t lds, hipStream_t s) {
  hipError_t err = hipFuncSetAttribute(reinterpret_cast<const void *>(&score_kernel7q<Q, TH>), hipFuncAttributeMaxDynamicSharedMemorySize, (int)lds);
  if (err != hipSuccess) return err;
  hipLaunchKernelGGL((score_kernel7q<Q, TH>), dim3(blocks), dim3(threads), lds, s, a);
  return hipGetLastError();
}

template <int Q, int TH, bool SG>
static hipError_t launch7sg(const ScoreArgs &a, int blocks, int threads, size_t lds, hipStream_t s) {
  hipError_t err = hipFuncSetAttribute(reinterpret_cast<const void *>(&score_kernel7<Q, TH, SG>),
                                       hipFuncAttributeMaxDynamicSharedMemorySize, (int)lds);
  if (err != hipSuccess) return err;
  hipLaunchKernelGGL((score_kernel7<Q, TH, SG>), dim3(blocks), dim3(threads), lds, s, a);
  return hipGetLastError();
}

template <int Q, int TH>
static hipError_t launch7(const ScoreArgs &a, int blocks, int threads, size_t lds, hipStream_t s) {
  if (a.spec_scratch) return launch7sg<Q, TH, true>(a, blocks, threads, lds, s);
  return launch7sg<Q, TH, false>(a, blocks, threads, lds, s);
}

template <int TH>
static hipError_t launch7_q(int Q, const ScoreArgs &a, int blocks, int threads, size_t lds, hipStream_t s) {
  switch (Q) {
    case 4:  return launch7<4, TH>(a, blocks, threads, lds, s);
    case 8:  return launch7<8, TH>(a, blocks, threads, lds, s);
    case 12: return launch7<12, TH>(a, blocks, threads, lds, s);
    case 16: return launch7<16, TH>(a, blocks, threads, lds, s);
    case 20: return launch7<20, TH>(a, blocks, threads, lds, s);
    case 24: return launch7<24, TH>(a, blocks, threads, lds, s);
    default: return hipErrorInvalidValue;
  }
}

#endif
}

#if !defined(WH_SWEEPS_ONLY) && !defined(WH_K7B)
hipError_t launch_score7q(int Q, const ScoreArgs &a, int blocks, int threads, size_t lds, hipStream_t s) {
  using namespace WH_K7NS;
  if (a.spec_arrays != kSpArr || !a.spec_scratch || threads > 768) return hipErrorInvalidValue;
  if (Q == 16) return launch7q<16, 768>(a, blocks, threads, lds, s);
  return hipErrorInvalidValue;
}
#endif
#ifndef WH_SWEEPS_ONLY
hipError_t WH_K7LAUNCH(int Q, const ScoreArgs &a, int blocks, int threads, size_t lds, hipStream_t s) {
  using namespace WH_K7NS;
  if (!a.spec_scratch && a.spec_arrays != kSpArr) return hipErrorInvalidValue;
  if (threads <= 512) return launch7_q<512>(Q, a, blocks, threads, lds, s);
  if (threads <= 768) return launch7_q<768>(Q, a, blocks, threads, lds, s);
  return hipErrorInvalidValue;
}
#endif

}
```

Baseline: 22970 queries/s.

## Store per-row spec records interleaved and drop J state in unihit stored sweeps

Adds a row-major (array-of-structs) layout for the per-row special-state scratch, packing the six per-row words (B, E, S, N, J, C) together so the backward and decode passes touch one record per row instead of six strided arrays. It also adds a unihit specialisation for the stored forward sweep that skips the J-state update, its store and its load in the backward pass. The layout is chosen at compile time and tagged into spec_arrays so the host and kernel agree. This adds template complexity and a new layout-mismatch failure mode, and round-trips through the global spill buffer now translate between the two layouts.

```diff
diff --git a/witch_amd/csrc/wh_device.h b/witch_amd/csrc/wh_device.h
--- a/witch_amd/csrc/wh_device.h
+++ b/witch_amd/csrc/wh_device.h
@@ -238,19 +238,43 @@
 
 constexpr float kRescaleHi = 1048576.0f;
 
+enum { SPEC_SOA = 0, SPEC_ROWS = 1 };
+template <int LAYOUT>
+struct SpecAt {
+  int SP;
+  __device__ __forceinline__ int operator()(int field, int row) const {
+    if (LAYOUT == SPEC_ROWS) {
+      return 6 * row + (field == SP_B ? 0 : field == SP_E ? 1 : field == SP_S ? 2 : field == SP_N ? 3 : field == SP_J ? 4 : 5);
+    }
+    return field * SP + row;
+  }
+  __device__ __forceinline__ int row0(int field) const { return LAYOUT == SPEC_ROWS ? (*this)(field, 0) : field * SP; }
+  __device__ __forceinline__ int operator()(int field, int row, int back) const {
+    if (LAYOUT == SPEC_ROWS) return (*this)(field, row - back);
+    return field * SP + row - back;
+  }
+  template <class T>
+  __device__ __forceinline__ T *ptr(T *spec, int field, int row, int back = 0) const {
+    if (LAYOUT == SPEC_ROWS) return spec + (*this)(field, row - back);
+    return back ? spec + field * SP + row - back : spec + field * SP + row;
+  }
+};
+
+template <int LAYOUT = SPEC_SOA>
 __device__ __forceinline__ void region_scan_global(float *spec, int SP, int L, int *regs, int lane, int &nenv,
                                                    int &nreg, int &flags) {
+  const SpecAt<LAYOUT> at{SP};
   const float rt1 = 0.25f, rt2 = 0.10f;
   float btot = 0.f, etot = 0.f;
   int i0 = -1;
   bool trig = false;
-  if (lane == 0) { spec[SP_J * SP] = 0.f; spec[SP_C * SP] = 0.f; }
+  if (lane == 0) { spec[at.row0(SP_J)] = 0.f; spec[at.row0(SP_C)] = 0.f; }
   for (int j0 = 1; j0 <= L; j0 += kWave) {
     const int jj = j0 + lane;
     const bool valid = jj <= L;
-    const float nv = valid ? __builtin_nontemporal_load(spec + SP_N * SP + jj) : 0.f;
-    const float bv = valid ? __builtin_nontemporal_load(spec + SP_B * SP + jj - 1) : 0.f;
-    const float ev = valid ? __builtin_nontemporal_load(spec + SP_E * SP + jj) : 0.f;
+    const float nv = valid ? __builtin_nontemporal_load(at.ptr(spec, SP_N, jj)) : 0.f;
+    const float bv = valid ? __builtin_nontemporal_load(at.ptr(spec, SP_B, jj, 1)) : 0.f;
+    const float ev = valid ? __builtin_nontemporal_load(at.ptr(spec, SP_E, jj)) : 0.f;
     float jout = 0.f, cout = 0.f;
     const int cnt = L - j0 + 1 < kWave ? L - j0 + 1 : kWave;
     for (int t = 0; t < cnt; t++) {
@@ -274,15 +298,17 @@
         trig = false;
       }
     }
-    if (valid) { spec[SP_J * SP + jj] = jout; spec[SP_C * SP + jj] = cout; }
-  }
-}
-
-template <int Q, bool TREG, bool STORE, bool USEP = false, bool SLIM = false, bool UM = false, bool COUNT = false, bool BLK = false>
+    if (valid) { spec[at(SP_J, jj)] = jout; spec[at(SP_C, jj)] = cout; }
+  }
+}
+
+template <int Q, bool TREG, bool STORE, bool USEP = false, bool SLIM = false, bool UM = false, bool COUNT = false, bool BLK = false, bool UNI = false, int LAYOUT = SPEC_SOA>
 __device__ __forceinline__ void forward_sweep(const TransTab<Q, TREG> &T, const ScanC &sc, const float *emL,
                                               const float *emG, int K, const uint8_t *seq, int L, LenCfg cfg,
                                               float *spec, int SP, float *Fs, float keep_scale, int lane,
                                               float &xC_out, int &ef_out, unsigned *um_out = nullptr, int *nstored_out = nullptr, int keep_lanes = 63 << 8) {
+  static_assert(LAYOUT == SPEC_SOA || !STORE || SLIM, "a record has six words: the mask words of a stored sweep share the B / E slots");
+  const SpecAt<LAYOUT> at{SP};
   float Mp[Q], Ip[Q], Dp[Q];
 #pragma unroll
   for (int q = 0; q < Q; q++) { Mp[q] = 0.f; Ip[q] = 0.f; Dp[q] = 0.f; }
@@ -292,8 +318,8 @@
   int nstored = 0;
   unsigned long long umask = 0;
   if (lane == 0) {
-    spec[SP_N * SP] = xN; spec[SP_B * SP] = xB; spec[SP_E * SP] = 0.f; spec[SP_J * SP] = 0.f;
-    spec[SP_C * SP] = 0.f; reinterpret_cast<int *>(spec)[SP_S * SP] = 0;
+    spec[at.row0(SP_N)] = xN; spec[at.row0(SP_B)] = xB; spec[at.row0(SP_E)] = 0.f; spec[at.row0(SP_J)] = 0.f;
+    spec[at.row0(SP_C)] = 0.f; reinterpret_cast<int *>(spec)[at.row0(SP_S)] = 0;
   }
 #pragma unroll 1
   for (int i = 1; i <= L; i++) {
@@ -353,22 +379,29 @@
     }
     xE = wave_sum(es);
     xN = xN * cfg.loop;
-    xC = fmaf(xC, cfg.loop, xE * cfg.EC);
-    xJ = fmaf(xJ, cfg.loop, xE * cfg.EJ);
+    if (UNI) {
+      xC = fmaf(xC, cfg.loop, xE);
+    } else {
+      xC = fmaf(xC, cfg.loop, xE * cfg.EC);
+      xJ = fmaf(xJ, cfg.loop, xE * cfg.EJ);
+    }
     if (xE > kRescaleHi) {
       const int e = f32_exponent(xE);
       const float r = pow2f_int(-e);
 #pragma unroll
       for (int q = 0; q < Q; q++) { Mp[q] *= r; Ip[q] *= r; Dp[q] *= r; }
-      xN *= r; xC *= r; xJ *= r; xE *= r;
+      xN *= r; xC *= r;
+      if (!UNI) xJ *= r;
+      xE *= r;
       ef += e;
     }
-    xB = (xJ + xN) * cfg.move;
+    xB = UNI ? xN * cfg.move : (xJ + xN) * cfg.move;
     if (lane == 0) {
-      spec[SP_N * SP + i] = xN;
-      if (!(STORE && SLIM)) { spec[SP_B * SP + i] = xB; spec[SP_E * SP + i] = xE; }
-      spec[SP_J * SP + i] = xJ; spec[SP_C * SP + i] = xC;
-      reinterpret_cast<int *>(spec)[SP_S * SP + i] = ef;
+      spec[at(SP_N, i)] = xN;
+      if (!(STORE && SLIM)) { spec[at(SP_B, i)] = xB; spec[at(SP_E, i)] = xE; }
+      if (!UNI) spec[at(SP_J, i)] = xJ;
+      spec[at(SP_C, i)] = xC;
+      reinterpret_cast<int *>(spec)[at(SP_S, i)] = ef;
     }
     if (UM && !STORE) {
       if ((i & 7) == 0) {
@@ -396,8 +429,8 @@
       const unsigned long long mask = __ballot(keep);
       if (COUNT) nstored += __builtin_popcountll(mask);
       if (lane == 0) {
-        reinterpret_cast<unsigned *>(spec)[ML * SP + i] = (unsigned)(mask & 0xFFFFFFFFull);
-        reinterpret_cast<unsigned *>(spec)[MH * SP + i] = (unsigned)(mask >> 32);
+        reinterpret_cast<unsigned *>(spec)[at(ML, i)] = (unsigned)(mask & 0xFFFFFFFFull);
+        reinterpret_cast<unsigned *>(spec)[at(MH, i)] = (unsigned)(mask >> 32);
       }
       if (keep) {
         float4 *row = reinterpret_cast<float4 *>(Fs) + (size_t)i * (2 * (Q / 4) * kWave);
@@ -410,8 +443,8 @@
     }
   }
   if (STORE && lane == 0) {
-    reinterpret_cast<unsigned *>(spec)[(SLIM ? SP_B : SP_ML) * SP] = (unsigned)(umask & 0xFFFFFFFFull);
-    reinterpret_cast<unsigned *>(spec)[(SLIM ? SP_E : SP_MH) * SP] = (unsigned)(umask >> 32);
+    reinterpret_cast<unsigned *>(spec)[at.row0(SLIM ? SP_B : SP_ML)] = (unsigned)(umask & 0xFFFFFFFFull);
+    reinterpret_cast<unsigned *>(spec)[at.row0(SLIM ? SP_E : SP_MH)] = (unsigned)(umask >> 32);
   }
   if (UM && !STORE && lane == 0) {
     um_out[0] = (unsigned)(umask & 0xFFFFFFFFull); um_out[1] = (unsigned)(umask >> 32);
@@ -432,6 +465,26 @@
     for (int p = 0; p < Q; p++) { Mb[p] *= r; Ib[p] *= r; }
     xJ *= r; xC *= r; xN *= r;
   }
+}
+
+template <int Q>
+__device__ __forceinline__ void mirror_scale(int dn, float (&Mb)[Q], float (&Ib)[Q], float &xC, float &xN) {
+  if (dn != 0) {
+    const float r = __builtin_bit_cast(float, (127 - dn) << 23);
+#pragma unroll
+    for (int p = 0; p < Q; p++) { Mb[p] *= r; Ib[p] *= r; }
+    xC *= r; xN *= r;
+  }
+}
+template <int Q>
+__device__ __forceinline__ bool clamp_backward(float (&Mb)[Q], float (&Ib)[Q], float &xB, float &xC, float &xN) {
+  if (fmaxf(xB, fmaxf(xN, xC)) > kClampHi) {
+#pragma unroll
+    for (int p = 0; p < Q; p++) { Mb[p] = fminf(Mb[p], kClampHi); Ib[p] = fminf(Ib[p], kClampHi); }
+    xB = fminf(xB, kClampHi); xN = fminf(xN, kClampHi); xC = fminf(xC, kClampHi);
+    return true;
+  }
+  return false;
 }
 
 template <int Q>
diff --git a/witch_amd/csrc/wh_host_score.hip b/witch_amd/csrc/wh_host_score.hip
--- a/witch_amd/csrc/wh_host_score.hip
+++ b/witch_amd/csrc/wh_host_score.hip
@@ -133,6 +133,7 @@
   a.keep_scale = kn.keep_scale;
   a.spill_band = kn.kernel != 9 ? kn.spill_band : 0;
   a.Klds = p.Klds; a.SP = p.b.SP; a.wave_lds = p.b.wave_lds; a.spec_arrays = kScoreSpecArrays;
+  if (p.family == ScoreFamily::PhaseCall || p.family == ScoreFamily::FourEnvelope) a.spec_arrays |= kScoreSpecLayout << 8;
   a.paths = reinterpret_cast<unsigned long long *>(e->counter(kSlotScorePath));
   a.p2win = p.p2win;
   a.qorder = p.use_qorder ? c.d_qorder : nullptr;
diff --git a/witch_amd/csrc/wh_plan.h b/witch_amd/csrc/wh_plan.h
--- a/witch_amd/csrc/wh_plan.h
+++ b/witch_amd/csrc/wh_plan.h
@@ -14,6 +14,10 @@
 constexpr size_t kLdsBudget = 160 * 1024 - 512;
 constexpr size_t kLdsHeader = 16;
 constexpr int kScoreSpecArrays = 6;
+#ifndef WH_K7_LAYOUT
+#define WH_K7_LAYOUT 1
+#endif
+constexpr int kScoreSpecLayout = WH_K7_LAYOUT;
 constexpr int kAlignSpecRows = 14;
 constexpr int kMaxPlanLength = 1 << 24;
 
diff --git a/witch_amd/csrc/wh_score7.hip b/witch_amd/csrc/wh_score7.hip
--- a/witch_amd/csrc/wh_score7.hip
+++ b/witch_amd/csrc/wh_score7.hip
@@ -28,6 +28,22 @@
 constexpr int kSpML = SP_ML, kSpMH = SP_MH, kSpArr = SP_NARR;
 #endif
 constexpr bool kMaskedAcc = true;
+#if defined(WH_SWEEPS_ONLY) || !defined(WH_SLIM_SPEC)
+#define WH_K7_NEW_DEFAULT 0
+#else
+#define WH_K7_NEW_DEFAULT 1
+#endif
+#ifndef WH_SPEC_ROWS
+#define WH_SPEC_ROWS WH_K7_NEW_DEFAULT
+#endif
+#ifndef WH_UNI
+#define WH_UNI WH_K7_NEW_DEFAULT
+#endif
+constexpr int kLayout = WH_SPEC_ROWS ? SPEC_ROWS : SPEC_SOA;
+constexpr bool kUni = WH_UNI != 0;
+static_assert(kLayout == SPEC_SOA || kSlim, "a row record has six words (WH_SLIM_SPEC)");
+template <bool SG> using SpecOf = SpecAt<SG ? (int)SPEC_SOA : kLayout>;
+constexpr int kSpecTag = kSpArr | (kLayout << 8);
 
 __device__ __noinline__ static double dlog(double x) { return log(x); }
 __device__ __noinline__ static double dexp(double x) { return exp(x); }
@@ -66,6 +82,7 @@
   const unsigned lo = (unsigned)__builtin_amdgcn_readfirstlane((int)(unsigned)(unsigned long long)v), hi = (unsigned)__builtin_amdgcn_readfirstlane((int)(unsigned)((unsigned long long)v >> 32));
   return (int64_t)(((unsigned long long)hi << 32) | lo);
 }
+__device__ __forceinline__ void touch_len_config(const LenCfg &cfg) { asm volatile("" :: "v"(cfg.EJ), "v"(cfg.EC)); }
 struct P4Out { float mass, domcorr; };
 struct RegOut { int nenv, nreg, flags; };
 
@@ -81,8 +98,9 @@
   const ScanC sc = scan_prepare(lane_product<Q, false>(T, FW_D2));
   FwdOut o;
   constexpr bool UM = !STORE && !SG && Q >= 8;
+  if (STORE && kUni && !SG) touch_len_config(cfg);
   o.nst = 0;
-  forward_sweep<Q, false, STORE, (Q <= kMaxQP), kSlim, UM, STORE, !SG>(T, sc, (const float *)c.emL, (const float *)c.emG, ctxKlds(c), seq, L, cfg, SG ? (float *)c.specg : (float *)c.spec, c.SP, (float *)c.Fs, keep_scale, c.lane, o.xC, o.ef,
+  forward_sweep<Q, false, STORE, (Q <= kMaxQP), kSlim, UM, STORE, !SG, (STORE && kUni && !SG), (SG ? (int)SPEC_SOA : kLayout)>(T, sc, (const float *)c.emL, (const float *)c.emG, ctxKlds(c), seq, L, cfg, SG ? (float *)c.specg : (float *)c.spec, c.SP, (float *)c.Fs, keep_scale, c.lane, o.xC, o.ef,
                                                                   reinterpret_cast<unsigned *>((float *)c.n2tab) + kUmSlot, &o.nst, keep_lanes);
   if (SG) __builtin_amdgcn_fence(__ATOMIC_SEQ_CST, "workgroup");
   return o;
@@ -96,6 +114,7 @@
   T.load(nullptr, (const float *)c.bwL, c.lane);
   const ScanC sc = scan_prepare(lane_product<Q, false>(T, BW_DD));
   const int lane = c.lane, SP = c.SP;
+  const SpecOf<SG> at{SP};
   float *spec = SG ? (float *)c.specg : (float *)c.spec;
   auto ldf = [&](int idx) -> float { return SG ? __builtin_nontemporal_load(spec + idx) : spec[idx]; };
   auto ldi = [&](int idx) -> int { return SG ? __builtin_nontemporal_load(reinterpret_cast<const int *>(spec) + idx) : reinterpret_cast<const int *>(spec)[idx]; };
@@ -138,22 +157,22 @@
       xB *= r; xJ *= r; xC *= r; xN *= r; xE *= r;
       eb += e;
     }
-    const float s_i = ldexpf(invZ, (SG ? R.s(0, i) : ldi(SP_S * SP + i)) + eb - ef_L);
-    const float pe = (SG ? R.f(2, i) : ldf(SP_E * SP + i)) * xE * s_i;
-    const float pb = (SG ? R.f(3, i) : ldf(SP_B * SP + i)) * xB * s_i;
+    const float s_i = ldexpf(invZ, (SG ? R.s(0, i) : ldi(at(SP_S, i))) + eb - ef_L);
+    const float pe = (SG ? R.f(2, i) : ldf(at(SP_E, i))) * xE * s_i;
+    const float pb = (SG ? R.f(3, i) : ldf(at(SP_B, i))) * xB * s_i;
     float njc = 0.f;
     if (i >= 1) {
-      const float s_p = ldexpf(invZ, (SG ? R.s(1, i) : ldi(SP_S * SP + i - 1)) + eb - ef_L);
-      njc = (SG ? R.f(4, i) : ldf(SP_N * SP + i - 1)) * xN;
-      njc = fmaf(SG ? R.f(5, i) : ldf(SP_J * SP + i - 1), xJ, njc);
-      njc = fmaf(SG ? R.f(6, i) : ldf(SP_C * SP + i - 1), xC, njc);
+      const float s_p = ldexpf(invZ, (SG ? R.s(1, i) : ldi(at(SP_S, i, 1))) + eb - ef_L);
+      njc = (SG ? R.f(4, i) : ldf(at(SP_N, i, 1))) * xN;
+      njc = fmaf(SG ? R.f(5, i) : ldf(at(SP_J, i, 1)), xJ, njc);
+      njc = fmaf(SG ? R.f(6, i) : ldf(at(SP_C, i, 1)), xC, njc);
       njc = njc * cm.loop * s_p;
     }
     if (SG) {
       if (lane == R.top - i) { wE = pe; wB = pb; wN = njc; }
     } else {
       __builtin_amdgcn_wave_barrier();
-      if (lane == 0) { spec[SP_E * SP + i] = pe; spec[SP_B * SP + i] = pb; spec[SP_N * SP + i] = njc; }
+      if (lane == 0) { spec[at(SP_E, i)] = pe; spec[at(SP_B, i)] = pb; spec[at(SP_N, i)] = njc; }
       __builtin_amdgcn_wave_barrier();
     }
   }
@@ -168,6 +187,8 @@
   T.load(nullptr, (const float *)c.bwL, c.lane);
   const ScanC sc = scan_prepare(lane_product<Q, false>(T, BW_DD));
   const int lane = c.lane, SP = c.SP;
+  const SpecOf<SG> at{SP};
+  constexpr bool NOJ = kUni && !SG;
   const float *spec = SG ? (const float *)c.specg : (const float *)c.spec;
   auto ldf = [&](int idx) -> float { return SG ? __builtin_nontemporal_load(spec + idx) : spec[idx]; };
   auto ldi = [&](int idx) -> int { return SG ? __builtin_nontemporal_load(reinterpret_cast<const int *>(spec) + idx) : reinterpret_cast<const int *>(spec)[idx]; };
@@ -186,7 +207,7 @@
   for (int i = Ld; i >= 1; i--) {
     asm volatile("" ::: "memory");
     if (SG && R.spent(i)) R.load(spec, r_off, r_sh, i, lane);
-    auto mask_word = [&]() -> unsigned { return SG ? (src < 32 ? R.u(0, i) : R.u(1, i)) : (src < 32 ? ldu(kSpML * SP + i) : ldu(kSpMH * SP + i)); };
+    auto mask_word = [&]() -> unsigned { return SG ? (src < 32 ? R.u(0, i) : R.u(1, i)) : (src < 32 ? ldu(at(kSpML, i)) : ldu(at(kSpMH, i))); };
     float4 fm4[Q / 4], fi4[Q / 4];
     auto request_row = [&]() {
       const unsigned mword = mask_word();
@@ -204,8 +225,8 @@
       }
     };
     if (TH < 768) request_row();
-    const int S_i = SG ? R.s(2, i) : ldi(SP_S * SP + i);
-    const int dS = S_i - (SG ? R.s(3, i) : ldi(SP_S * SP + i - 1));
+    const int S_i = SG ? R.s(2, i) : ldi(at(SP_S, i));
+    const int dS = S_i - (SG ? R.s(3, i) : ldi(at(SP_S, i, 1)));
     if (i < Ld) {
       mirror_scale<Q>(S_next - S_i, Mb, Ib, xJ, xC, xN);
       xB = wave_sum(backward_emit<Q, false>(T, emL, (const float *)c.emG, eseq[i], ctxKlds(c), lane, Mb));
@@ -251,9 +272,9 @@
       }
       fIs = fmaf(idot, s_i, fIs);
     }
-    float nj = (SG ? R.f(4, i) : ldf(SP_N * SP + i - 1)) * xN;
-    nj = fmaf(SG ? R.f(5, i) : ldf(SP_J * SP + i - 1), xJ, nj);
-    nj = fmaf(SG ? R.f(6, i) : ldf(SP_C * SP + i - 1), xC, nj);
+    float nj = (SG ? R.f(4, i) : ldf(at(SP_N, i, 1))) * xN;
+    nj = fmaf(SG ? R.f(5, i) : NOJ ? 0.f : ldf(at(SP_J, i, 1)), xJ, nj);
+    nj = fmaf(SG ? R.f(6, i) : ldf(at(SP_C, i, 1)), xC, nj);
     S_next = S_i;
     xfac = fmaf(nj * cu.loop, s_p, xfac);
   }
@@ -303,6 +324,10 @@
   constexpr int Q4 = Q / 4, B4 = QB / 4;
   const uint8_t *eseq = (const uint8_t *)eseq3;
   const int lane = c.lane, SP = c.SP, Klds = ctxKlds(c);
+  const SpecOf<SG> at{SP};
+  constexpr bool UNI = kUni && !SG;
+  if (UNI) touch_len_config(cu);
+  constexpr bool CARRY = !SG && kLayout == SPEC_ROWS;
   const float *spec = SG ? (const float *)c.specg : (const float *)c.spec;
   auto ldf = [&](int idx) -> float { return SG ? __builtin_nontemporal_load(spec + idx) : spec[idx]; };
   auto ldi = [&](int idx) -> int { return SG ? __builtin_nontemporal_load(reinterpret_cast<const int *>(spec) + idx) : reinterpret_cast<const int *>(spec)[idx]; };
@@ -339,7 +364,7 @@
   if (SG) R.load(spec, r_off, r_sh, Ld, lane);
   auto request_row = [&](int r, bool first) {
     const unsigned mword = SG ? (first ? (lanef < 32 ? ldu(kSpML * SP + r) : ldu(kSpMH * SP + r)) : (lanef < 32 ? R.u(0, r + 1) : R.u(1, r + 1)))
-                              : (lanef < 32 ? ldu(kSpML * SP + r) : ldu(kSpMH * SP + r));
+                              : (lanef < 32 ? ldu(at(kSpML, r)) : ldu(at(kSpMH, r)));
     have_n = (mword >> (lanef & 31)) & 1u;
     if (have_n) {
       const float4 *row = reinterpret_cast<const float4 *>((const float *)c.Fs) + (size_t)r * (2 * Q4 * kWave);
@@ -348,6 +373,7 @@
     }
   };
   request_row(Ld, true);
+  int S_row = CARRY ? ldi(at(SP_S, Ld)) : 0;
 #pragma unroll 1
   for (int i = Ld; i >= 1; i--) {
     asm volatile("" ::: "memory");
@@ -357,10 +383,16 @@
     for (int p4 = 0; p4 < B4; p4++) { fm_c[p4] = fm_n[p4]; fi_c[p4] = fi_n[p4]; }
     const bool have = have_n;
     if (i > 1) request_row(i - 1, false);
-    const int S_i = SG ? R.s(2, i) : ldi(SP_S * SP + i);
-    const int dS = S_i - (SG ? R.s(3, i) : ldi(SP_S * SP + i - 1));
+    int S_p = 0;
+    float N_p = 0.f, J_p = 0.f, C_p = 0.f;
+    if (CARRY) {
+      S_p = ldi(at(SP_S, i, 1)); N_p = ldf(at(SP_N, i, 1)); C_p = ldf(at(SP_C, i, 1));
+      if (!UNI) J_p = ldf(at(SP_J, i, 1));
+    }
+    const int S_i = CARRY ? S_row : SG ? R.s(2, i) : ldi(at(SP_S, i));
+    const int dS = S_i - (CARRY ? S_p : SG ? R.s(3, i) : ldi(at(SP_S, i, 1)));
     if (i < Ld) {
-      mirror_scale<QB>(S_next - S_i, Mb, Ib, xJ, xC, xN);
+      if (UNI) mirror_scale<QB>(S_next - S_i, Mb, Ib, xC, xN); else mirror_scale<QB>(S_next - S_i, Mb, Ib, xJ, xC, xN);
       const int x = __builtin_amdgcn_readfirstlane((int)eseq[i]);
       float part = 0.f;
       auto emit = [&](auto em_ld) {
@@ -377,13 +409,13 @@
       if (x < Klds) emit([&](int p4) { return em4L[x * (Q * 16) + fwd[p4]]; });
       else emit([&](int p4) { return em4G[(size_t)x * (Q * 16) + fwd[p4]]; });
       xB = wave_sum(part);
-      xJ = fmaf(xJ, cu.loop, xB * cu.move);
+      if (!UNI) xJ = fmaf(xJ, cu.loop, xB * cu.move);
       xC = xC * cu.loop;
       xN = fmaf(xN, cu.loop, xB * cu.move);
     }
-    const float xE = fmaf(xC, cu.EC, xJ * cu.EJ);
+    const float xE = UNI ? xC : fmaf(xC, cu.EC, xJ * cu.EJ);
     backward_cells<QB, true, false>(T, sc, Mb, Ib, xE);
-    clamp_backward<QB>(Mb, Ib, xB, xJ, xC, xN);
+    if (UNI) clamp_backward<QB>(Mb, Ib, xB, xC, xN); else clamp_backward<QB>(Mb, Ib, xB, xJ, xC, xN);
     const float s_i = invZe;
     const float s_p = ldexpf(invZe, -dS);
     if (have) {
@@ -401,10 +433,11 @@
       }
       fIs = fmaf(idot, s_i, fIs);
     }
-    float nj = (SG ? R.f(4, i) : ldf(SP_N * SP + i - 1)) * xN;
-    nj = fmaf(SG ? R.f(5, i) : ldf(SP_J * SP + i - 1), xJ, nj);
-    nj = fmaf(SG ? R.f(6, i) : ldf(SP_C * SP + i - 1), xC, nj);
+    float nj = (CARRY ? N_p : SG ? R.f(4, i) : ldf(at(SP_N, i, 1))) * xN;
+    if (!UNI) nj = fmaf(CARRY ? J_p : SG ? R.f(5, i) : ldf(at(SP_J, i, 1)), xJ, nj);
+    nj = fmaf(CARRY ? C_p : SG ? R.f(6, i) : ldf(at(SP_C, i, 1)), xC, nj);
     S_next = S_i;
+    if (CARRY) S_row = S_p;
     xfac = fmaf(nj * cu.loop, s_p, xfac);
   }
   float sm = 0.f;
@@ -549,13 +582,13 @@
         if (x < Klds) emit([&](int p4) { return em4L[x * (Q * 16) + (3 - p4) * kWave + lanef]; });
         else emit([&](int p4) { return em4G[(size_t)x * (Q * 16) + (3 - p4) * kWave + lanef]; });
         xB = row_sum(part);
-        xJ = fmaf(xJ, cu.loop, xB * cu.move);
+        if (!kUni) xJ = fmaf(xJ, cu.loop, xB * cu.move);
         xC = xC * cu.loop;
         xN = fmaf(xN, cu.loop, xB * cu.move);
       }
-      const float xE = fmaf(xC, cu.EC, xJ * cu.EJ);
+      const float xE = kUni ? xC : fmaf(xC, cu.EC, xJ * cu.EJ);
       backward_cells_row(T, sc, Mb, Ib, xE);
-      clamp_backward<16>(Mb, Ib, xB, xJ, xC, xN);
+      if (kUni) clamp_backward<16>(Mb, Ib, xB, xC, xN); else clamp_backward<16>(Mb, Ib, xB, xJ, xC, xN);
       const float s_i = invZe;
       const float s_p = ldexpf(invZe, S_p - S_i);
       if ((w_i >> (lanef & 31)) & 1u) {
@@ -573,10 +606,10 @@
         fIs = fmaf(idot, s_i, fIs);
       }
       float nj = n_p * xN;
-      nj = fmaf(j_p, xJ, nj);
+      if (!kUni) nj = fmaf(j_p, xJ, nj);
       nj = fmaf(c_p, xC, nj);
       xfac = fmaf(nj * cu.loop, s_p, xfac);
-      mirror_scale<16>(S_i - S_p, Mb, Ib, xJ, xC, xN);
+      if (kUni) mirror_scale<16>(S_i - S_p, Mb, Ib, xC, xN); else mirror_scale<16>(S_i - S_p, Mb, Ib, xJ, xC, xN);
     }
     if (j + 1 < Lmax) {
       request_row(j + 1);
@@ -641,9 +674,11 @@
   constexpr int Q4 = Q / 4, B4 = QB / 4;
   const uint8_t *seq = (const uint8_t *)seq3;
   const int lane = c.lane, SP = c.SP, Klds = ctxKlds(c);
+  const SpecAt<kLayout> at{SP};
+  constexpr bool CARRY = kLayout == SPEC_ROWS;
   const float *spec = (const float *)c.spec;
   float *tmp = (float *)c.spec + kSpArr * SP;
-  float *tE = INPL ? (float *)c.spec + SP_E * SP : tmp, *tB = INPL ? (float *)c.spec + SP_B * SP : tmp + SP, *tN = INPL ? (float *)c.spec + SP_N * SP : tmp + 2 * SP;
+  float *specw = (float *)c.spec;
   glb_f *gE = c.specg, *gB = c.specg + SP, *gN = c.specg + 2 * SP;
   const int *speci = reinterpret_cast<const int *>(spec);
   int fwd[B4];
@@ -669,9 +704,22 @@
   float xC = cm.move, xJ = 0.f, xN = 0.f, xB = 0.f;
   int eb = 0;
   float ratio = 0.f;
+  int S_row = 0;
+  float E_row = 0.f, B_row = 0.f;
+  if (CARRY) { S_row = speci[at(SP_S, L)]; E_row = spec[at(SP_E, L)]; B_row = spec[at(SP_B, L)]; }
 #pragma unroll 1
   for (int i = L; i >= 0; i--) {
     asm volatile("" ::: "memory");
+    const int S_i = CARRY ? S_row : 0;
+    const float E_i = CARRY ? E_row : 0.f, B_i = CARRY ? B_row : 0.f;
+    int S_p = 0;
+    float N_p = 0.f, J_p = 0.f, C_p = 0.f;
+    if (CARRY) {
+      const int ip = i >= 1 ? i - 1 : 0;
+      S_p = speci[at(SP_S, ip)]; N_p = spec[at(SP_N, ip)]; J_p = spec[at(SP_J, ip)]; C_p = spec[at(SP_C, ip)];
+      E_row = spec[at(SP_E, ip)]; B_row = spec[at(SP_B, ip)];
+      S_row = S_p;
+    }
     if (i < L) {
       const int x = __builtin_amdgcn_readfirstlane((int)seq[i]);
       float part = 0.f;
@@ -704,22 +752,25 @@
       xB *= r; xJ *= r; xC *= r; xN *= r; xE *= r;
       eb += e;
     }
-    const float s_i = ldexpf(invZ, speci[SP_S * SP + i] + eb - ef_L);
-    const float pe = spec[SP_E * SP + i] * xE * s_i;
-    const float pb = spec[SP_B * SP + i] * xB * s_i;
+    const float s_i = ldexpf(invZ, (CARRY ? S_i : speci[at(SP_S, i)]) + eb - ef_L);
+    const float pe = (CARRY ? E_i : spec[at(SP_E, i)]) * xE * s_i;
+    const float pb = (CARRY ? B_i : spec[at(SP_B, i)]) * xB * s_i;
     float njc = 0.f;
     if (i >= 1) {
-      const float s_p = ldexpf(invZ, speci[SP_S * SP + i - 1] + eb - ef_L);
-      njc = spec[SP_N * SP + i - 1] * xN;
-      njc = fmaf(spec[SP_J * SP + i - 1], xJ, njc);
-      njc = fmaf(spec[SP_C * SP + i - 1], xC, njc);
+      const float s_p = ldexpf(invZ, (CARRY ? S_p : speci[at(SP_S, i, 1)]) + eb - ef_L);
+      njc = (CARRY ? N_p : spec[at(SP_N, i, 1)]) * xN;
+      njc = fmaf(CARRY ? J_p : spec[at(SP_J, i, 1)], xJ, njc);
+      njc = fmaf(CARRY ? C_p : spec[at(SP_C, i, 1)], xC, njc);
       njc = njc * cm.loop * s_p;
     } else {
-      ratio = spec[SP_N * SP] * xN * s_i;
+      ratio = (CARRY ? N_p : spec[at(SP_N, 0)]) * xN * s_i;
     }
     __builtin_amdgcn_wave_barrier();
     if (TMPG) { if (lane == 0) { gE[i] = pe; gB[i] = pb; gN[i] = njc; } }
-    else if (lane == 0) { tE[i] = pe; tB[i] = pb; tN[i] = njc; }
+    else if (lane == 0) {
+      if (INPL) { specw[at(SP_E, i)] = pe; specw[at(SP_B, i)] = pb; specw[at(SP_N, i)] = njc; }
+      else { tmp[i] = pe; tmp[SP + i] = pb; tmp[2 * SP + i] = njc; }
+    }
     __builtin_amdgcn_wave_barrier();
   }
   WinDec o;
@@ -730,7 +781,13 @@
 template <int TH, bool INPL = false, bool TMPG = false>
 __device__ __noinline__ RegOut region_scan_cert(lds_f *spec3, int SP, int L, lds_i *regs3, int lane, float eps, glb_f *tmpg = nullptr) {
   float *tmp = TMPG ? (float *)tmpg : (float *)spec3 + kSpArr * SP;
-  float *tE = INPL ? (float *)spec3 + SP_E * SP : tmp, *tB = INPL ? (float *)spec3 + SP_B * SP : tmp + SP, *tN = INPL ? (float *)spec3 + SP_N * SP : tmp + 2 * SP;
+  const SpecAt<kLayout> at{SP};
+  struct Col {
+    float *base; int field; SpecAt<kLayout> at;
+    __device__ __forceinline__ float *operator+(int row) const { return INPL ? base + at(field, row) : base + row; }
+    __device__ __forceinline__ operator float *() const { return *this + 0; }
+  };
+  const Col tE{INPL ? (float *)spec3 : tmp, SP_E, at}, tB{INPL ? (float *)spec3 : tmp + SP, SP_B, at}, tN{INPL ? (float *)spec3 : tmp + 2 * SP, SP_N, at};
   if (TMPG) __builtin_amdgcn_fence(__ATOMIC_SEQ_CST, "workgroup");
   int *regs = (int *)regs3;
   const float rt1 = 0.25f, rt2 = 0.10f, rt3 = 0.20f;
@@ -749,7 +806,7 @@
     const int jj = j0 + lane;
     const bool valid = jj <= L;
     const float nv = valid ? ldt(tN + jj) : 0.f;
-    const float bv = valid ? (jj - 1 == 0 ? pb0 : ldt(tB + jj - 1)) : 0.f;
+    const float bv = valid ? (jj - 1 == 0 ? pb0 : ldt(tB + (jj - 1))) : 0.f;
     const float ev = valid ? ldt(tE + jj) : 0.f;
     float jout = 0.f, cout = 0.f;
     const int cnt = L - j0 + 1 < kWave ? L - j0 + 1 : kWave;
@@ -789,9 +846,9 @@
   for (int e = 0; e < nenv; e++) {
     const int ri = regs[2 * e], rj = regs[2 * e + 1];
     float mx = -1.0f;
-    const float e0 = ldt(tE + ri - 1), bj = ldt(tN + rj);
+    const float e0 = ldt(tE + (ri - 1)), bj = ldt(tN + rj);
     for (int z = ri + lane; z <= rj; z += kWave) {
-      const float u = ldt(tE + z) - e0, v = bj - ldt(tN + z - 1);
+      const float u = ldt(tE + z) - e0, v = bj - ldt(tN + (z - 1));
       mx = fmaxf(mx, fminf(u, v));
     }
     mx = wave_max(mx);
@@ -811,16 +868,17 @@
   int *regs = (int *)regs3;
   const float rt3 = 0.20f;
   int nenv = 0, nreg = 0, flags = 0;
-  region_scan_global(spec, SP, L, regs, lane, nenv, nreg, flags);
+  const SpecOf<SG> at{SP};
+  region_scan_global<(SG ? (int)SPEC_SOA : kLayout)>(spec, SP, L, regs, lane, nenv, nreg, flags);
   __builtin_amdgcn_wave_barrier();
   if (SG) __builtin_amdgcn_fence(__ATOMIC_SEQ_CST, "workgroup");
   int multi_mask = 0;
   for (int e = 0; e < nenv; e++) {
     const int ri = regs[2 * e], rj = regs[2 * e + 1];
     float mx = -1.0f;
-    const float e0 = ldf(SP_C * SP + ri - 1), bj = ldf(SP_J * SP + rj);
+    const float e0 = ldf(at(SP_C, ri, 1)), bj = ldf(at(SP_J, rj));
     for (int z = ri + lane; z <= rj; z += kWave) {
-      const float u = ldf(SP_C * SP + z) - e0, v = bj - ldf(SP_J * SP + z - 1);
+      const float u = ldf(at(SP_C, z)) - e0, v = bj - ldf(at(SP_J, z, 1));
       mx = fmaxf(mx, fminf(u, v));
     }
     mx = wave_max(mx);
@@ -858,7 +916,8 @@
   if constexpr (Q >= 8) {
     if (!dense && !a.no_window && !skip_window) {
       const unsigned *su = reinterpret_cast<const unsigned *>(SG ? (const float *)c.specg : (const float *)c.spec);
-      unsigned long long um = ((unsigned long long)su[kSpMH * SP] << 32) | su[kSpML * SP];
+      const SpecOf<SG> at{SP};
+      unsigned long long um = ((unsigned long long)su[at.row0(kSpMH)] << 32) | su[at.row0(kSpML)];
       um = mask_in_band(um, band);
       if (um != 0) {
         int lo = __builtin_ctzll(um), hi = 63 - __builtin_clzll(um);
@@ -1023,8 +1082,12 @@
         wd.eps = 1.0f;
         if (TMPG && nodes <= (Q % 8 == 0 && Q > 8 ? 8 : 4) * kWave) {
           const float *spec = (const float *)c.spec;
-          for (int arr = 0; arr < kSpArr; arr++)
-            for (int u = lane; u <= L; u += kWave) __builtin_nontemporal_store(spec[arr * SP + u], tmpg + arr * SP + u);
+          if (kLayout == SPEC_ROWS) {
+            for (int u = lane; u < kSpArr * (L + 1); u += kWave) __builtin_nontemporal_store(spec[u], tmpg + u);
+          } else {
+            for (int arr = 0; arr < kSpArr; arr++)
+              for (int u = lane; u <= L; u += kWave) __builtin_nontemporal_store(spec[arr * SP + u], tmpg + arr * SP + u);
+          }
           saved = true;
         }
         if (nodes <= 4 * kWave) wd = sweep_backward_decode_win<4, Q, TH, TMPG, false, false>(c, (lds_u8 *)seq, L, cm, 1.0f / (f1.xC * cm.move), f1.ef, min((63 - hi) * Q, kWave * (Q - 4)));
@@ -1050,8 +1113,12 @@
       __builtin_amdgcn_fence(__ATOMIC_SEQ_CST, "workgroup");
       float *spec = (float *)c.spec;
       __builtin_amdgcn_wave_barrier();
-      for (int arr = 0; arr < kSpArr; arr++)
-        for (int u = lane; u <= L; u += kWave) spec[arr * SP + u] = __builtin_nontemporal_load(tmpg + arr * SP + u);
+      if (kLayout == SPEC_ROWS) {
+        for (int u = lane; u < kSpArr * (L + 1); u += kWave) spec[u] = __builtin_nontemporal_load(tmpg + u);
+      } else {
+        for (int arr = 0; arr < kSpArr; arr++)
+          for (int u = lane; u <= L; u += kWave) spec[arr * SP + u] = __builtin_nontemporal_load(tmpg + arr * SP + u);
+      }
       __builtin_amdgcn_wave_barrier();
     }
     sweep_backward_decode<Q, TH, SG>(c, (lds_u8 *)seq, L, cm, 1.0f / (f1.xC * cm.move), f1.ef);
@@ -1331,7 +1398,8 @@
               bool done = !(f3.xC > 0.f);
               if (!done) {
                 const unsigned *su = reinterpret_cast<const unsigned *>((const float *)c.spec);
-                const unsigned long long um = mask_in_band(((unsigned long long)su[kSpMH * SP] << 32) | su[kSpML * SP], band);
+                const SpecAt<kLayout> at{SP};
+                const unsigned long long um = mask_in_band(((unsigned long long)su[at.row0(kSpMH)] << 32) | su[at.row0(kSpML)], band);
                 int m0 = -1;
                 if (um != 0) {
                   int lo = __builtin_ctzll(um), hi = 63 - __builtin_clzll(um);
@@ -1342,7 +1410,7 @@
                   glb_f *dst = specg0 + (size_t)t * spec_stride1;
                   const float *spec = (const float *)c.spec;
                   for (int arr = 0; arr < kSpArr; arr++)
-                    for (int u = lane; u <= Ld; u += kWave) __builtin_nontemporal_store(spec[arr * SP + u], dst + arr * SP + u);
+                    for (int u = lane; u <= Ld; u += kWave) __builtin_nontemporal_store(spec[at(arr, u)], dst + arr * SP + u);
                   if (lane == 0) {
                     int *sl = qslots + t * QS_INTS;
                     sl[QS_ACTIVE] = 1; sl[QS_LD] = Ld; sl[QS_M0] = m0;
@@ -1422,8 +1490,9 @@
             float *spec = (float *)c.spec;
             const glb_f *src = specg0 + (size_t)t * spec_stride1;
             __builtin_amdgcn_wave_barrier();
+            const SpecAt<kLayout> at{SP};
             for (int arr = 0; arr < kSpArr; arr++)
-              for (int u = lane; u <= Ld; u += kWave) spec[arr * SP + u] = __builtin_nontemporal_load(src + arr * SP + u);
+              for (int u = lane; u <= Ld; u += kWave) spec[at(arr, u)] = __builtin_nontemporal_load(src + arr * SP + u);
             __builtin_amdgcn_wave_barrier();
             c.Fs = Fs0 + (size_t)t * slab1;
             FwdOut f3; f3.xC = __builtin_bit_cast(float, qr[QR_XC3]); f3.ef = qr[QR_EF3];
@@ -1502,7 +1571,7 @@
 #if !defined(WH_SWEEPS_ONLY) && !defined(WH_K7B)
 hipError_t launch_score7q(int Q, const ScoreArgs &a, int blocks, int threads, size_t lds, hipStream_t s) {
   using namespace WH_K7NS;
-  if (a.spec_arrays != kSpArr || !a.spec_scratch || threads > 768) return hipErrorInvalidValue;
+  if (a.spec_arrays != kSpecTag || !a.spec_scratch || threads > 768) return hipErrorInvalidValue;
   if (Q == 16) return launch7q<16, 768>(a, blocks, threads, lds, s);
   return hipErrorInvalidValue;
 }
@@ -1510,7 +1579,7 @@
 #ifndef WH_SWEEPS_ONLY
 hipError_t WH_K7LAUNCH(int Q, const ScoreArgs &a, int blocks, int threads, size_t lds, hipStream_t s) {
   using namespace WH_K7NS;
-  if (!a.spec_scratch && a.spec_arrays != kSpArr) return hipErrorInvalidValue;
+  if (!a.spec_scratch && a.spec_arrays != kSpecTag) return hipErrorInvalidValue;
   if (threads <= 512) return launch7_q<512>(Q, a, blocks, threads, lds, s);
   if (threads <= 768) return launch7_q<768>(Q, a, blocks, threads, lds, s);
   return hipErrorInvalidValue;
```

Measured after the change: 23550 queries/s (median of 6 runs). +2.6%, better.
